# CWBudde/go-pocket-tts

Measured on AMD Instinct MI355X. Metric: synthesized audio sec/sec (xRT), higher is better.
Workload: dtype bf16; 1 GPU; b64_10s_bf16: 64 utterances/GPU x 125 frames (10.0 s each), 25-token prompt + 125-frame voice state, greedy (temperature 0), hipGraph-captured AR step, Mimi decode to 24 kHz PCM written to host; batch_per_gpu=64, frames=125, weights=BF16, kv=bf16, checkpoint=synthetic, shapes of tts_b6369a24 (seed 1234)

## Files before the change

### go-pocket-tts_amd/csrc/capi_hooks.cpp

```cpp
#include "capi_internal.h"
#include "launch_args.h"
#include "../../include/ptts_debug.h"
#include "scan_block.h"
#include "true_peak.h"

#include <memory>

using namespace ptts;
using namespace ptts::capi;

namespace {

template <class T> class Scoped {
    T& var_;
    T old_;
public:
    Scoped(T& var, T value) : var_(var), old_(var) { var = value; }
    ~Scoped() { var_ = old_; }
    Scoped(const Scoped&) = delete;
    Scoped& operator=(const Scoped&) = delete;
};

using Census = std::map<std::string, int64_t>;

// ... 1021 lines not shown
            if (t.t0 % 4) throw Error(PTTS_EINVAL, "ptts_debug_resblock: t0 % 4 != 0 with row destinations");
            if (!t.row_out || t.row_bytes % 16 || t.row_bytes < (int64_t)t.L * 4) throw Error(PTTS_EINVAL, "ptts_debug_resblock: row_bytes must be a multiple of 16 and hold L f32 samples");
            for (int b = 0; b < t.B; b++) if (t.rows[2 * b] < 0) throw Error(PTTS_EINVAL, "ptts_debug_resblock: negative lim");
        }
        if (up_) {
            if (!bf) throw Error(PTTS_EINVAL, "ptts_debug_resblock: f32 weights with the fused form (its weights live in registers and LDS as bf16)");
            if (t.C != 64 || !fin) throw Error(PTTS_EINVAL, "ptts_debug_resblock: the fused form is the 64-wide block with the final convolution");
            if (!t.xin || !t.wup || t.x_pad < 1 || t.x_pad > 64 || t.x_slack < 0 || t.x_slack > 64 || t.x_L < 1) throw Error(PTTS_EINVAL, "ptts_debug_resblock: bad arguments of the fused form");
            if ((int64_t)t.x_L * 4 != t.L) throw Error(PTTS_EINVAL, "ptts_debug_resblock: x_L * 4 != L");
            if (t.t0 % 4) throw Error(PTTS_EINVAL, "ptts_debug_resblock: t0 % 4 != 0 with the fused form");
            if (t.form == RES_FORM_TILE) throw Error(PTTS_EINVAL, "ptts_debug_resblock: the fused form is persistent only");
        }
        ResPlan plan;
        if (t.form == RES_FORM_AUTO) {
            require_device();
            plan = up_ ? resblock_up_plan(t.B, t.t1 - t.t0, RES_FORM_AUTO, 0, resblock_cus()) : resblock_plan(t.C, fin, bf, t.B, t.t1 - t.t0, RES_FORM_AUTO, 0, resblock_cus());
            if (plan.grid == 0) throw Error(PTTS_EINVAL, "ptts_debug_resblock: the fused form is not taken at this size (resblock_up_supported's threshold); ask for form 2 with a grid");
        } else {
            plan = up_ ? resblock_up_plan(t.B, t.t1 - t.t0, t.form, t.grid, 1) : resblock_plan(t.C, fin, bf, t.B, t.t1 - t.t0, t.form, t.grid, 1);
            if (plan.nw == 0) throw Error(PTTS_EINVAL, "ptts_debug_resblock: no persistent form of this block (bf16 weights; 64-wide with the final convolution, 128-wide without)");
        }
        const int64_t total = (int64_t)t.B * plan.tiles;
        if (plan.pers && (plan.grid < 1 || plan.grid > total))
            throw Error(PTTS_EINVAL, strfmt("ptts_debug_resblock: grid %d outside [1, B * tiles = %lld]: a block's first tile would lie past the last utterance", plan.grid, (long long)total));
        if (!plan.pers && plan.grid != total) throw Error(PTTS_EINVAL, "ptts_debug_resblock: one block per tile");

        const int C = t.C, H = t.H, B = t.B, L = t.L;
        const size_t n1 = frag16_count((size_t)H, (size_t)3 * C), n2 = frag16_count((size_t)C, (size_t)H), nf = frag16_count(16, (size_t)3 * C), nu = frag16_count(256, 256);
        std::vector<uint16_t> w1h(n1), w1l(n1), w2h(n2), w2l(n2), wfh(nf), wfl(nf), wuh(nu);
        pack_frag16(t.w1, (size_t)H, (size_t)3 * C, w1h.data(), bf ? nullptr : w1l.data());
        pack_frag16(t.w2, (size_t)C, (size_t)H, w2h.data(), bf ? nullptr : w2l.data());
        if (fin) pack_final_frag(t.wf, (size_t)3 * C, wfh.data(), wfl.data());
        if (up_) {
            std::vector<float> rg((size_t)256 * 256);
            regroup_convtr_rows(t.wup, 256, 256, 64, rg.data());
            pack_frag16(rg.data(), 256, 256, wuh.data(), nullptr);
        }
        require_device();
        const int64_t urows = (int64_t)t.pad + L + t.slack, u_bs = urows * C, xrows = up_ ? (int64_t)t.x_pad + t.x_L + t.x_slack : 1, x_bs = xrows * 128;
        const size_t u_elems = (size_t)B * u_bs, x_elems = (size_t)B * x_bs, pcm_elems = (size_t)B * L, row_bytes = t.rows ? (size_t)B * t.row_bytes : 0;
        Stage st;
        std::vector<float> img(u_elems, std::nanf("")), xi(up_ ? x_elems : 0, std::nanf(""));
        if (t.u) for (int b = 0; b < B; b++) std::memcpy(img.data() + (size_t)b * u_bs, t.u + (size_t)b * (t.pad + L) * C, (size_t)(t.pad + L) * C * 4);
        if (up_) for (int b = 0; b < B; b++) std::memcpy(xi.data() + (size_t)b * x_bs, t.xin + (size_t)b * (t.x_pad + t.x_L) * 128, (size_t)(t.x_pad + t.x_L) * 128 * 4);
        float *dUo = st.out(u_elems), *dPcm = st.out(pcm_elems);
        uint8_t* dRows = st.out<uint8_t>(row_bytes);
        ResArgs a;
        a.u = st.in(img.data(), u_elems); a.u_bs = u_bs; a.pad = t.pad;
        a.w1 = st.in(w1h.data(), n1); a.w2 = st.in(w2h.data(), n2);
        if (!bf) { a.w1_lo = st.in(w1l.data(), n1); a.w2_lo = st.in(w2l.data(), n2); }
        a.b1 = st.in(t.b1, (size_t)H); a.b2 = st.in(t.b2, (size_t)C);
        a.B = B; a.L = L; a.t0 = t.t0; a.t1 = t.t1; a.C = C; a.H = H; a.k1 = 3; a.k2 = 1; a.w_bf16 = bf; a.final_conv = fin;
        if (fin) {
            a.kf = 3; a.wf_hi = st.in(wfh.data(), nf); a.wf_lo = st.in(wfl.data(), nf);
            a.bf = st.in(t.bf, 1);
            a.pcm = dPcm; a.pcm_bs = L;
            if (t.rows) {
                std::vector<PcmRow> pr((size_t)B);
                for (int b = 0; b < B; b++) pr[b] = PcmRow{dRows + (size_t)b * t.row_bytes, t.rows[2 * b], t.rows[2 * b + 1] != 0};
                a.pcm_rows = st.in(pr.data(), (size_t)B);
            }
        } else a.uo = dUo;
        if (up_) {
            a.fuse_up = 1; a.xin = st.in(xi.data(), x_elems); a.x_bs = x_bs; a.x_pad = t.x_pad; a.x_L = t.x_L; a.CI = 128; a.up_stride = 4; a.wup = st.in(wuh.data(), nu);
            a.bup = st.in(t.bup, 64);
        }
        if (!(up_ ? resblock_up_shape_supported(a) : resblock_supported(a))) throw Error(PTTS_EINVAL, "ptts_debug_resblock: refused by resblock_supported / resblock_up_shape_supported");
        if (up_) launch_resblock_up_as(a, plan, nullptr);
        else launch_resblock_as(a, plan, nullptr);
        PTTS_HIP(hipGetLastError());
        PTTS_HIP(hipDeviceSynchronize());
        if (t.launched) { t.launched[0] = plan.nw; t.launched[1] = plan.pers; t.launched[2] = plan.grid; t.launched[3] = plan.tiles; t.launched[4] = plan.tout; }
        if (t.uo) down(t.uo, dUo, u_elems * 4);
        if (t.pcm) down(t.pcm, dPcm, pcm_elems * 4);
        if (t.rows) down(t.row_out, dRows, row_bytes);
    });
}

int ptts_debug_mimi_pack(int32_t kind, const float* w1, const float* w2, int32_t n, uint16_t* dst) {
    return guard([&] {
        if (!w1 || !dst || n < 32 || n % 32 || kind < 0 || kind > 1 || (kind == 0 && !w2)) throw Error(PTTS_EINVAL, "ptts_debug_mimi_pack: bad arguments");
        if (kind == 0) pack_ffn_image(w1, w2, n, dst);
        else pack_w1_image(w1, n, dst);
    });
}

int ptts_debug_mimi_fused(const ptts_mimi_fused_args* pa) {
    return guard([&] {
        if (!pa) throw Error(PTTS_EINVAL, "ptts_debug_mimi_fused: null argument");
        const ptts_mimi_fused_args& t = *pa;
        if (t.kind < 0 || t.kind > 1) throw Error(PTTS_EINVAL, strfmt("ptts_debug_mimi_fused: unknown kind %d", t.kind));
        const bool ffn = t.kind == 0;
        if (!t.x || !t.ln_w || !t.ln_b || !t.w1 || !t.out || (ffn && !t.w2) || t.M < 1 || t.M > (1 << 20) || t.D < 1 || t.D > 4096 || t.F < 1 || t.F > 8192 ||
            t.x_elems < 1 || t.x_ld < 1 || t.x_rows_per_batch < 0 || t.x_rows_per_batch > INT32_MAX || t.x_batch_stride < 0 || t.x_off < 0 || t.ls_off < 0 || t.ls_off > 64)
            throw Error(PTTS_EINVAL, "ptts_debug_mimi_fused: bad arguments");
        if (!ffn && (t.y_elems < 1 || t.y_ld < 1 || t.y_rows_per_batch < 0 || t.y_rows_per_batch > INT32_MAX || t.y_batch_stride < 0 || t.y_off < 0 || t.ls))
            throw Error(PTTS_EINVAL, "ptts_debug_mimi_fused: bad arguments for k_mimi_rowlin");
        const bool rope = t.rope_cos || t.rope_sin;
        if (rope && (ffn || !t.rope_cos || !t.rope_sin || t.n_pos < 1 || t.pos0 < 0 || t.rows_per_seg < 0 || t.rope_cols < 0))
            throw Error(PTTS_EINVAL, "ptts_debug_mimi_fused: bad RoPE arguments");
        const int M = t.M, D = t.D, F = t.F;
        const RowMap xmap{t.x_ld, t.x_rows_per_batch, t.x_batch_stride}, ymap{t.y_ld, t.y_rows_per_batch, t.y_batch_stride};
        check_rows("ptts_debug_mimi_fused", "x", M, t.x_elems, xmap, t.x_off, D, ffn);
        if (!ffn) check_rows("ptts_debug_mimi_fused", "y", M, t.y_elems, ymap, t.y_off, F, true);
        if (rope)
            for (int64_t m = 0; m < M; m++) {
                const int64_t pos = (int64_t)t.pos0 + (t.rows_per_seg ? m % t.rows_per_seg : m);
                if (pos >= t.n_pos) throw Error(PTTS_EINVAL, strfmt("ptts_debug_mimi_fused: row %lld at position %lld, the tables hold %d", (long long)m, (long long)pos, t.n_pos));
            }
        require_device();
        const size_t img_entries = ffn ? ffn_image_count(F) : w1_image_count(F), ntab = rope ? (size_t)t.n_pos * 32 : 0;
        Stage st;
        Tmp dX((size_t)t.x_elems * 4), dLw((size_t)D * 4), dLb((size_t)D * 4), dLs(((size_t)D + t.ls_off) * 4), dImg(img_entries * 2), dCos(ntab * 4), dSin(ntab * 4);
        float* dY = ffn ? nullptr : st.out((size_t)t.y_elems);
        FfnArgs fa;
        RowLinArgs ra;
        if (ffn) {
            fa.x = dX.as<float>() + t.x_off; fa.xmap = xmap;
            fa.ln_w = dLw.as<float>(); fa.ln_b = dLb.as<float>(); fa.eps = t.eps;
            fa.img = dImg.p;
            if (t.ls) fa.ls = dLs.as<float>() + t.ls_off;
            fa.M = M; fa.D = D; fa.F = F;
            if (!mimi_ffn_supported(fa)) throw Error(PTTS_EINVAL, "ptts_debug_mimi_fused: refused by mimi_ffn_supported");
        } else {
            ra.x = dX.as<float>() + t.x_off; ra.xmap = xmap;
            ra.ln_w = dLw.as<float>(); ra.ln_b = dLb.as<float>(); ra.eps = t.eps;
            ra.img = dImg.p;
            ra.y = dY + t.y_off; ra.ymap = ymap;
            if (rope) { ra.rope_cos = dCos.as<float>(); ra.rope_sin = dSin.as<float>(); ra.rope_cols = t.rope_cols; ra.rope_pos0 = t.pos0; ra.rope_rows_per_seg = t.rows_per_seg; }
            ra.M = M; ra.N = F; ra.K = D;
            if (!mimi_rowlin_supported(ra)) throw Error(PTTS_EINVAL, "ptts_debug_mimi_fused: refused by mimi_rowlin_supported");
        }
        std::vector<uint16_t> img(img_entries);
        if (ffn) pack_ffn_image(t.w1, t.w2, F, img.data());
        else pack_w1_image(t.w1, F, img.data());
        up(dImg.p, img.data(), img_entries * 2);
        up(dX.p, t.x, (size_t)t.x_elems * 4);
        up(dLw.p, t.ln_w, (size_t)D * 4); up(dLb.p, t.ln_b, (size_t)D * 4);
        if (t.ls) up(dLs.as<float>() + t.ls_off, t.ls, (size_t)D * 4);
        if (rope) { up(dCos.p, t.rope_cos, ntab * 4); up(dSin.p, t.rope_sin, ntab * 4); }
        LaunchScope launches;
        launches.run([&] {
            if (ffn) launch_mimi_ffn(fa, nullptr);
            else launch_mimi_rowlin(ra, nullptr);
        });
        PTTS_HIP(hipGetLastError());
        PTTS_HIP(hipDeviceSynchronize());
        put_str(t.launched, t.launched_cap, launches.str());
        if (ffn) down(t.out, dX.p, (size_t)t.x_elems * 4);
        else down(t.out, dY, (size_t)t.y_elems * 4);
    });
}

int ptts_mimi_layer_piece(ptts_model* h, int32_t layer, int32_t which, const float* x, int64_t rows, int32_t pos0, int32_t rows_per_seg, float* out) {
    return guard([&] {
        if (!h || !h->m) throw Error(PTTS_EINVAL, "native-safetensors runtime unavailable");
        Model& m = *h->m;
        const Desc& d = m.d;
        if (!x || !out || rows <= 0 || rows > (1 << 24)) throw Error(PTTS_EINVAL, "ptts-hip: bad rows");
        if (layer < 0 || layer >= d.mimi_layers) throw Error(PTTS_EINVAL, strfmt("ptts-hip: mimi layer %d out of range [0,%d)", layer, d.mimi_layers));
        if (which != PTTS_MIMI_PIECE_QKV && which != PTTS_MIMI_PIECE_FFN) throw Error(PTTS_EINVAL, "ptts-hip: unknown layer piece");
        if (pos0 < 0 || rows_per_seg < 0 || (int64_t)pos0 + (rows_per_seg ? rows_per_seg : rows) > ROPE_SEQ)
            throw Error(PTTS_EINVAL, strfmt("ops: rope cos/sin sequence length too small for pos=%d seq=%lld", pos0, (long long)(rows_per_seg ? rows_per_seg : rows)));
        std::lock_guard<std::mutex> lock(m.mu);
        m.use_device();
        const int C = d.mimi_dim, F = d.mimi_ffn, R = (int)rows;
        const int NO = which == PTTS_MIMI_PIECE_QKV ? 3 * C : C;
        Tmp dx((size_t)R * C * 4), dn((size_t)R * C * 4), dy((size_t)R * std::max(NO, F) * 4);
        PTTS_HIP(hipMemcpyAsync(dx.p, x, (size_t)R * C * 4, hipMemcpyHostToDevice, m.stream));
        if (which == PTTS_MIMI_PIECE_QKV) {
            mimi_layer_qkv(m, layer, dx.as<float>(), RowMap{C, 0, 0}, R, dy.as<float>(), RowMap{3 * C, 0, 0}, pos0, rows_per_seg, dn.as<float>(), m.stream);
            PTTS_HIP(hipMemcpyAsync(out, dy.p, (size_t)R * NO * 4, hipMemcpyDeviceToHost, m.stream));
        } else {
            mimi_layer_ffn(m, layer, dx.as<float>(), RowMap{C, 0, 0}, R, dn.as<float>(), dy.as<float>(), m.stream);
            PTTS_HIP(hipMemcpyAsync(out, dx.p, (size_t)R * NO * 4, hipMemcpyDeviceToHost, m.stream));
        }
        PTTS_HIP(hipStreamSynchronize(m.stream));
    });
}

}
```

### go-pocket-tts_amd/csrc/ffn_fused.hip

```cpp
#include <cstdlib>
#include <type_traits>

#include "kernels.h"
#include "device_util.h"
#include "mfma_util.h"

namespace ptts {

namespace {

__device__ __forceinline__ float ff_gelu(float x) {
    const float ax = fabsf(x);
    const float t = __builtin_amdgcn_rcpf(fmaf(0.3275911f * 0.70710678118654752f, ax, 1.0f));
    float p = fmaf(1.061405429f, t, -1.453152027f);
    p = fmaf(p, t, 1.421413741f);
    p = fmaf(p, t, -0.284496736f);
    p = fmaf(p, t, 0.254829592f);
    p *= t;
    const float e = __builtin_amdgcn_exp2f(-1.4426950408889634f * 0.5f * x * x);
    const float erfa = fmaf(-p, e, 1.0f);
    const float erfs = copysignf(erfa, x);
    return 0.5f * x * (1.0f + erfs);
}

constexpr int FF_D = 512;
constexpr int FF_CH = 32;
constexpr int FF_KS = FF_D / 32;
constexpr int FF_OT = FF_D / 16;
constexpr int FF_W1B = FF_CH * FF_D * 2;
constexpr int FF_W2B = FF_D * FF_CH * 2;
constexpr int FF_IMG = FF_W1B + FF_W2B;

__device__ __forceinline__ void ff_dma32k(const char* src, char* dst, int wave, int lane) {
#pragma unroll
    for (int i = 0; i < 8; i++) {
        const int idx = i * 4 + wave;
        lds_dma1k(src + idx * 1024 + lane * 16, dst + idx * 1024);
    }
}

__device__ __forceinline__ void ff_rows_layernorm(const float* xrow, const float* ln_w, const float* ln_b, float eps, int q, Frag (&xh)[16], Frag (&xl)[16]) {
    float4 v[16][2];
#pragma unroll
    for (int s = 0; s < 16; s++) {
        v[s][0] = *reinterpret_cast<const float4*>(xrow + 32 * s + 4 * q);
        v[s][1] = *reinterpret_cast<const float4*>(xrow + 32 * s + 16 + 4 * q);
    }
    float sum = 0.f;
#pragma unroll
    for (int s = 0; s < 16; s++) sum += (v[s][0].x + v[s][0].y) + (v[s][0].z + v[s][0].w) + (v[s][1].x + v[s][1].y) + (v[s][1].z + v[s][1].w);
    sum += __shfl_xor(sum, 16, 64);
    sum += __shfl_xor(sum, 32, 64);
    const float mean = sum * (1.0f / 512);
    float var = 0.f;
#pragma unroll
    for (int s = 0; s < 16; s++) {
#pragma unroll
        for (int h = 0; h < 2; h++) {
            const float d0 = v[s][h].x - mean, d1 = v[s][h].y - mean, d2 = v[s][h].z - mean, d3 = v[s][h].w - mean;
            var += (d0 * d0 + d1 * d1) + (d2 * d2 + d3 * d3);
        }
    }
    var += __shfl_xor(var, 16, 64);
    var += __shfl_xor(var, 32, 64);
    const float rstd = 1.0f / sqrtf(var * (1.0f / 512) + eps);
#pragma unroll
    for (int s = 0; s < 16; s++) {
        float4 o[2];
#pragma unroll
        for (int h = 0; h < 2; h++) {
            const int k = 32 * s + 16 * h + 4 * q;
            const float4 g = *reinterpret_cast<const float4*>(ln_w + k), b = *reinterpret_cast<const float4*>(ln_b + k);
            o[h].x = (v[s][h].x - mean) * rstd * g.x + b.x;
            o[h].y = (v[s][h].y - mean) * rstd * g.y + b.y;
            o[h].z = (v[s][h].z - mean) * rstd * g.z + b.z;
            o[h].w = (v[s][h].w - mean) * rstd * g.w + b.w;
        }
        split2(o[0].x, o[0].y, xh[s].u[0], xl[s].u[0]);
        split2(o[0].z, o[0].w, xh[s].u[1], xl[s].u[1]);
        split2(o[1].x, o[1].y, xh[s].u[2], xl[s].u[2]);
        split2(o[1].z, o[1].w, xh[s].u[3], xl[s].u[3]);
    }
}

template <class Piece>
__device__ __forceinline__ void ff_gemm1(const char* w1, int r16, int q, const Frag (&xh)[16], const Frag (&xl)[16], f32x4 (&acc)[2], Piece&& piece) {
    const int sw1 = (r16 >> 1) & 7;
    acc[0] = f32x4{0.f, 0.f, 0.f, 0.f};
    acc[1] = f32x4{0.f, 0.f, 0.f, 0.f};
    Frag wa[2], wb[2];
    const char* wl = w1 + r16 * 128;
    wa[0].q = *reinterpret_cast<const uint4*>(wl + ((q ^ sw1) << 4));
    wb[0].q = *reinterpret_cast<const uint4*>(wl + ((q ^ sw1) << 4) + 2048);
#pragma unroll
    for (int s = 0; s < 16; s++) {
        __builtin_amdgcn_sched_barrier(0);
        if (s + 1 < 16) {
            const int off = ((s + 1) >> 1) * 4096 + (((4 * ((s + 1) & 1) + q) ^ sw1) << 4);
            wa[(s + 1) & 1].q = *reinterpret_cast<const uint4*>(wl + off);
            wb[(s + 1) & 1].q = *reinterpret_cast<const uint4*>(wl + off + 2048);
        }
        acc[0] = __builtin_amdgcn_mfma_f32_16x16x32_bf16(wa[s & 1].v, xh[s].v, acc[0], 0, 0, 0);
        acc[1] = __builtin_amdgcn_mfma_f32_16x16x32_bf16(wb[s & 1].v, xh[s].v, acc[1], 0, 0, 0);
        PTTS_LO_MFMA(acc[0] = __builtin_amdgcn_mfma_f32_16x16x32_bf16(wa[s & 1].v, xl[s].v, acc[0], 0, 0, 0));
        PTTS_LO_MFMA(acc[1] = __builtin_amdgcn_mfma_f32_16x16x32_bf16(wb[s & 1].v, xl[s].v, acc[1], 0, 0, 0));
        piece(s);
        asm volatile("" : "+a"(acc[0]), "+a"(acc[1]));
        if (s + 1 < 16) __builtin_amdgcn_sched_group_barrier(0x100, 2, 0);
#pragma unroll
        for (int i = 0; i < 4; i++) {
            __builtin_amdgcn_sched_group_barrier(0x008, 1, 0);
            __builtin_amdgcn_sched_group_barrier(0x002, 3, 0);
        }
        __builtin_amdgcn_sched_barrier(0);
    }
}

}

template <int V>
__global__ __launch_bounds__(256) __attribute__((amdgpu_waves_per_eu(1, 1))) void k_mimi_ffn(FfnArgs a) {
    __shared__ __attribute__((aligned(16))) char lds[2 * FF_W1B + 2 * FF_W2B];
    const int tid = threadIdx.x, lane = tid & 63, wave = __builtin_amdgcn_readfirstlane(tid >> 6);
    const int r16 = lane & 15, q = lane >> 4;
    const int nch = a.F / FF_CH;
    const char* img = reinterpret_cast<const char*>(a.img);
    auto w1s = [&](int i) { return lds + i * FF_W1B; };
    auto w2s = [&](int i) { return lds + 2 * FF_W1B + i * FF_W2B; };

    ff_dma32k(img, w1s(0), wave, lane);
    ff_dma32k(img + FF_W1B, w2s(0), wave, lane);
    ff_dma32k(img + (size_t)min(1, nch - 1) * FF_IMG, w1s(1), wave, lane);

    const int m0 = blockIdx.x * 64 + wave * 16;
    const int row = min(m0 + r16, a.M - 1);
    const float* xrow = a.x + row_off(a.xmap, row);
    Frag xh[FF_KS], xl[FF_KS];
    ff_rows_layernorm(xrow, a.ln_w, a.ln_b, a.eps, q, xh, xl);

    f32x4 acc2[FF_OT];
#pragma unroll
    for (int t = 0; t < FF_OT; t++) acc2[t] = f32x4{0.f, 0.f, 0.f, 0.f};

    const int w2_lane = r16 * 64 + ((q ^ (((r16 >> 3) & 1) * 3)) << 4);

    asm volatile("s_waitcnt vmcnt(0)" ::: "memory");
    __syncthreads();
    f32x4 acc1[2], acc1n[2];
    ff_gemm1(w1s(0), r16, q, xh, xl, acc1, [](int) {});

    for (int c = 0; c < nch; c++) {
        asm volatile("s_waitcnt vmcnt(0)" ::: "memory");
        __syncthreads();
        asm volatile("" : "+a"(acc1[0]), "+a"(acc1[1]));
        const char* const src1 = img + (size_t)min(c + 2, nch - 1) * FF_IMG + wave * 1024 + lane * 16;
        const char* const src2 = img + (size_t)min(c + 1, nch - 1) * FF_IMG + FF_W1B + wave * 1024 + lane * 16;
        char* const dst1 = w1s(c & 1) + wave * 1024;
        char* const dst2 = w2s((c + 1) & 1) + wave * 1024;
        Frag hh, hl;
        float g[8];
        ff_gemm1(w1s(min(c + 1, nch - 1) & 1), r16, q, xh, xl, acc1n, [&](int s) {
            const int i = s >> 1;
            if ((s & 1) == 0) g[i] = ff_gelu(acc1[i >> 2][i & 3]);
            else if (i & 1) split2(g[i - 1], g[i], hh.u[i >> 1], hl.u[i >> 1]);
            if constexpr (V == 0) {
                if (s < 8) lds_dma1k(src1 + s * 4096, dst1 + s * 4096);
                else lds_dma1k(src2 + (s - 8) * 4096, dst2 + (s - 8) * 4096);
            }
        });
        const char* w2 = w2s(c & 1) + w2_lane;
        Frag w2f[2];
        w2f[0].q = *reinterpret_cast<const uint4*>(w2);
#pragma unroll
        for (int t = 0; t < FF_OT; t++) {
            __builtin_amdgcn_sched_barrier(0);
            if (t + 1 < FF_OT) w2f[(t + 1) & 1].q = *reinterpret_cast<const uint4*>(w2 + (t + 1) * 1024);
            acc2[t] = __builtin_amdgcn_mfma_f32_16x16x32_bf16(w2f[t & 1].v, hh.v, acc2[t], 0, 0, 0);
            PTTS_LO_MFMA(acc2[t] = __builtin_amdgcn_mfma_f32_16x16x32_bf16(w2f[t & 1].v, hl.v, acc2[t], 0, 0, 0));
            if (t + 1 < FF_OT) __builtin_amdgcn_sched_group_barrier(0x100, 1, 0);
            __builtin_amdgcn_sched_group_barrier(0x008, 2, 0);
            __builtin_amdgcn_sched_barrier(0);
        }
        acc1[0] = acc1n[0];
        acc1[1] = acc1n[1];
    }

    if (m0 + r16 < a.M) {
        float* orow = a.x + row_off(a.xmap, m0 + r16);
        const bool has_ls = a.ls != nullptr;
        const float* lsp = has_ls ? a.ls : a.ln_w;
#pragma unroll
        for (int t0 = 0; t0 < FF_OT; t0 += 8) {
            float4 r[8], sc[8];
#pragma unroll
            for (int t = 0; t < 8; t++) {
                const int col = 16 * (t0 + t) + 4 * q;
                r[t] = *reinterpret_cast<const float4*>(orow + col);
                sc[t] = *reinterpret_cast<const float4*>(lsp + col);
                if (!has_ls) sc[t] = make_float4(1.f, 1.f, 1.f, 1.f);
            }
#pragma unroll
            for (int t = 0; t < 8; t++) {
#pragma clang fp contract(off)
                const f32x4 y = acc2[t0 + t];
                float4 o;
                o.x = r[t].x + sc[t].x * y[0];
                o.y = r[t].y + sc[t].y * y[1];
                o.z = r[t].z + sc[t].z * y[2];
                o.w = r[t].w + sc[t].w * y[3];
                *reinterpret_cast<float4*>(orow + 16 * (t0 + t) + 4 * q) = o;
            }
        }
    }
}

__global__ __launch_bounds__(256) __attribute__((amdgpu_waves_per_eu(1, 1))) void k_mimi_rowlin(RowLinArgs a) {
    constexpr int NS = 3;
    __shared__ __attribute__((aligned(16))) char lds[NS * FF_W1B];
    const int tid = threadIdx.x, lane = tid & 63, wave = __builtin_amdgcn_readfirstlane(tid >> 6);
    const int r16 = lane & 15, q = lane >> 4;
    const int nch = a.N / FF_CH;
    const char* img = reinterpret_cast<const char*>(a.img);
    ff_dma32k(img, lds, wave, lane);
    ff_dma32k(img + (size_t)min(1, nch - 1) * FF_W1B, lds + FF_W1B, wave, lane);

    const int m0 = blockIdx.x * 64 + wave * 16;
    const int row = min(m0 + r16, a.M - 1);
    Frag xh[FF_KS], xl[FF_KS];
    ff_rows_layernorm(a.x + row_off(a.xmap, row), a.ln_w, a.ln_b, a.eps, q, xh, xl);
    float2 cs[4], sn[4];
    const bool rope = a.rope_cos != nullptr;
    {
        const int pos = a.rope_pos0 + (a.rope_rows_per_seg ? row % a.rope_rows_per_seg : row);
        const float* ct = rope ? a.rope_cos + (int64_t)pos * 32 : a.ln_w;
        const float* st = rope ? a.rope_sin + (int64_t)pos * 32 : a.ln_w;
#pragma unroll
        for (int i = 0; i < 4; i++) {
            const int jj = (32 * (i >> 1) + 16 * (i & 1) + 4 * q) >> 1;
            cs[i] = *reinterpret_cast<const float2*>(ct + jj);
            sn[i] = *reinterpret_cast<const float2*>(st + jj);
        }
    }
    float* const yrow = a.y + row_off(a.ymap, row);

    auto store_piece = [&](f32x4 (&acc)[2], int cc, auto par, int ht) {
#pragma clang fp contract(off)
        constexpr int PAR = decltype(par)::value;
        asm volatile("" : "+a"(acc[0]), "+a"(acc[1]));
        const int col = 32 * cc + 16 * ht + 4 * q;
        const bool rot = rope && 32 * cc < a.rope_cols;
        const f32x4 v = acc[ht];
        const float2 c2 = cs[2 * PAR + ht], s2 = sn[2 * PAR + ht];
        const float y0 = v[0] * c2.x - v[1] * s2.x, y1 = v[0] * s2.x + v[1] * c2.x;
        const float y2 = v[2] * c2.y - v[3] * s2.y, y3 = v[2] * s2.y + v[3] * c2.y;
        const float4 o = make_float4(rot ? y0 : v[0], rot ? y1 : v[1], rot ? y2 : v[2], rot ? y3 : v[3]);
        *reinterpret_cast<float4*>(yrow + col) = o;
    };

    asm volatile("s_waitcnt vmcnt(0)" ::: "memory");
    __syncthreads();
    f32x4 accA[2], accB[2];
    auto iter = [&](int c, auto par, auto first, f32x4 (&acc)[2], f32x4 (&prev)[2]) {
        constexpr int PAR = decltype(par)::value;
        constexpr bool FIRST = decltype(first)::value != 0;
        if constexpr (!FIRST) {
            asm volatile("s_waitcnt vmcnt(10)" ::: "memory");
            __syncthreads();
        }
        const char* const src = img + (size_t)min(c + 2, nch - 1) * FF_W1B + wave * 1024 + lane * 16;
        char* const dst = lds + ((c + 2) % NS) * FF_W1B + wave * 1024;
        ff_gemm1(lds + (c % NS) * FF_W1B, r16, q, xh, xl, acc, [&](int s) {
            if ((s & 1) == 0) lds_dma1k(src + (s >> 1) * 4096, dst + (s >> 1) * 4096);
            if constexpr (!FIRST) {
                if (s == 5) store_piece(prev, c - 1, std::integral_constant<int, 1 - PAR>{}, 0);
                if (s == 11) store_piece(prev, c - 1, std::integral_constant<int, 1 - PAR>{}, 1);
            }
        });
    };
    using ic0 = std::integral_constant<int, 0>;
    using ic1 = std::integral_constant<int, 1>;
    iter(0, ic0{}, ic1{}, accA, accB);
    iter(1, ic1{}, ic0{}, accB, accA);
    for (int c = 2; c < nch; c += 2) {
        iter(c, ic0{}, ic0{}, accA, accB);
        iter(c + 1, ic1{}, ic0{}, accB, accA);
    }
    store_piece(accB, nch - 1, std::integral_constant<int, 1>{}, 0);
    store_piece(accB, nch - 1, std::integral_constant<int, 1>{}, 1);
}

bool mimi_rowlin_supported(const RowLinArgs& a) {
    return a.img && a.K == FF_D && a.N >= 64 && a.N % 64 == 0 && a.M > 0 && aligned16(a.x) && a.xmap.ld % 4 == 0 && a.xmap.batch_stride % 4 == 0 && aligned16(a.y) &&
           a.ymap.ld % 4 == 0 && a.ymap.batch_stride % 4 == 0 && aligned16(a.img) && a.ln_w && a.ln_b && aligned16(a.ln_w) && aligned16(a.ln_b) &&
           (!a.rope_cos || (a.rope_sin && a.rope_cols % 64 == 0 && a.rope_cols <= a.N && (reinterpret_cast<uintptr_t>(a.rope_cos) & 7) == 0 && (reinterpret_cast<uintptr_t>(a.rope_sin) & 7) == 0));
}

void launch_mimi_rowlin(const RowLinArgs& a, hipStream_t stream) {
    note_launch(a.rope_cos ? "k_mimi_rowlin+rope" : "k_mimi_rowlin");
    hipLaunchKernelGGL(k_mimi_rowlin, dim3((unsigned)((a.M + 63) / 64)), dim3(256), 0, stream, a);
}

bool mimi_ffn_supported(const FfnArgs& a) {
    return a.img && a.D == FF_D && a.F >= FF_CH && a.F % FF_CH == 0 && a.M > 0 && aligned16(a.x) && a.xmap.ld % 4 == 0 && a.xmap.batch_stride % 4 == 0 &&
           aligned16(a.img) && a.ln_w && a.ln_b && aligned16(a.ln_w) && aligned16(a.ln_b) && (!a.ls || aligned16(a.ls));
}

void launch_mimi_ffn(const FfnArgs& a, hipStream_t stream) {
    note_launch("k_mimi_ffn");
    const dim3 grid((unsigned)((a.M + 63) / 64));
    hipLaunchKernelGGL(k_mimi_ffn<0>, grid, dim3(256), 0, stream, a);
}

}
```

### go-pocket-tts_amd/csrc/kernels.h

```cpp
#pragma once

#include <hip/hip_runtime.h>
#include <atomic>
#include <cstddef>
#include <cstdint>
#include <map>
#include <string>
#include <vector>

#include "deesser.h"
#include "limiter.h"
#include "pitch.h"
#include "tempo.h"
#include "trim.h"

namespace ptts {

struct RowMap {
    int64_t ld = 0;
    int64_t rows_per_batch = 0;
    int64_t batch_stride = 0;
};

enum AOp : int { AOP_NONE = 0, AOP_ELU = 1 };
// ... 255 lines not shown
    double* b_tiles;
    double* p_tiles;
    double* s_tiles;
    int32_t design, pad;
};
static_assert(sizeof(DeRow) == 48, "a turn of the de-esser ring holds 256 of them");
void launch_deesser(const DeRow* rows_dev, int n, int max_tiles, const DeScan* designs_dev, hipStream_t stream);

constexpr int kLimMaxDesigns = 16;
constexpr size_t kLimScanBytes = 64;
static_assert(sizeof(LimScan) == kLimScanBytes, "the limiter ring's tail (runtime.h) is sized by it");
struct LimRow {
    float* x;
    int64_t n;
    double* p_tiles;
    float* r;
    int32_t design, pad;
};
static_assert(sizeof(LimRow) == 40, "a turn of the limiter ring holds 256 of them");
void launch_limiter(const LimRow* rows_dev, int n, int max_tiles, const LimScan* designs_dev, hipStream_t stream);

constexpr int kJoinThreads = 256;
constexpr int kJoinTile = 4 * kJoinThreads;
struct JoinRow {
    const float* src;
    const float* prev;
    float* dst;
    int64_t off;
    int64_t n;
    int32_t k;
    int32_t gap;
};
static_assert(sizeof(JoinRow) == 48, "a turn of the join ring holds 256 of them");
void launch_join(const JoinRow* rows_dev, int n, int max_tiles, hipStream_t stream);

constexpr int kTrimMaxDesigns = 16;
constexpr size_t kTrimScanBytes = 32;
static_assert(sizeof(TrimScan) == kTrimScanBytes, "the trim ring's tail (runtime.h) is sized by it");
struct TrimTile {
    int32_t first, last;
    int32_t removed, cuts;
    int32_t prev, next;
    int32_t off, pad;
};
static_assert(sizeof(TrimTile) == 32, "trim_scratch_bytes counts on it");
struct TrimRow {
    const float* src;
    float* dst;
    int64_t n;
    TrimTile* tiles;
    ptts_trim_info* info;
    int32_t design, pad;
};
static_assert(sizeof(TrimRow) == 48, "a turn of the trim ring holds 256 of them");
void launch_trim(const TrimRow* rows_dev, int n, int max_tiles, const TrimScan* designs_dev, hipStream_t stream);

constexpr int kTempoMaxDesigns = 16;
constexpr size_t kTempoScanBytes = 16;
static_assert(sizeof(TempoScan) == kTempoScanBytes, "the tempo ring's tail (runtime.h) is sized by it");
struct TempoRow {
    const float* src;
    float* dst;
    int64_t n;
    int64_t n_out;
    int32_t* p;
    int32_t design, pad;
};
static_assert(sizeof(TempoRow) == 48, "a turn of the tempo ring holds 256 of them");
void launch_tempo(const TempoRow* rows_dev, int n, int max_tiles, const TempoScan* designs_dev, hipStream_t stream);

constexpr int kPitchMaxDesigns = 16;
constexpr size_t kPitchScanBytes = 16;
static_assert(sizeof(PitchScan) == kPitchScanBytes, "the pitch ring's tail (runtime.h) is sized by it");
constexpr int kPitchThreads = 512;
constexpr int kPitchTile = 1024;
constexpr int kPitchWindow = 2 * kPitchTile + 110;
PTTS_HD inline int pitch_image_at(int q) { return q + (q >> 5); }
constexpr int kPitchImage = (kPitchEntries + (kPitchEntries >> 5) + 1) & ~1;
struct PitchRow {
    const float* src;
    float* dst;
    int64_t n;
    int64_t n_out;
    int32_t design, pad;
};
static_assert(sizeof(PitchRow) == 40, "a turn of the pitch ring holds 256 of them");
void launch_pitch(const PitchRow* rows_dev, int n, int max_tiles, const PitchScan* designs_dev, const float* image_dev, hipStream_t stream);

constexpr int kFormantAnalyseThreads = 256;
constexpr int kFormantWhitenThreads = 256;
constexpr int kFormantShapeTiles = 16;
struct FormantRow {
    const float* x;
    float* e;
    const float* er;
    float* out;
    float* coeffs;
    int64_t n, n_r;
    int32_t K, p;
};
static_assert(sizeof(FormantRow) == 64, "a turn of the formant ring holds 256 of them");
void launch_formant_analyse(const FormantRow* rows_dev, int n, int64_t max_frames, const double* tables_dev, hipStream_t stream);
void launch_formant_whiten(const FormantRow* rows_dev, int n, int64_t max_tiles, hipStream_t stream);
void launch_formant_shape(const FormantRow* rows_dev, int n, int64_t max_tiles, hipStream_t stream);

struct PcmRow { void* dst; int32_t lim; int32_t s16; };
struct ResArgs {
    const float* u = nullptr; int64_t u_bs = 0; int pad = 0;
    float* uo = nullptr;
    float* pcm = nullptr; int64_t pcm_bs = 0;
    const PcmRow* pcm_rows = nullptr;
    const void* w1 = nullptr; const void* w1_lo = nullptr; const float* b1 = nullptr;
    const void* w2 = nullptr; const void* w2_lo = nullptr; const float* b2 = nullptr;
    const void* wf_hi = nullptr; const void* wf_lo = nullptr; const float* bf = nullptr;
    int B = 0, L = 0, t0 = 0, t1 = 0;
    int C = 0, H = 0, k1 = 0, k2 = 0, kf = 0, w_bf16 = 0, final_conv = 0;
    int fuse_up = 0; const float* xin = nullptr; int64_t x_bs = 0; int x_pad = 0, x_L = 0, CI = 0, up_stride = 0;
    const void* wup = nullptr; const float* bup = nullptr;
};
bool resblock_supported(const ResArgs& a);
void launch_resblock(const ResArgs& a, hipStream_t stream);
bool resblock_up_shape_supported(const ResArgs& a);
bool resblock_up_supported(const ResArgs& a);
void launch_resblock_up(const ResArgs& a, hipStream_t stream);
enum { RES_FORM_AUTO = 0, RES_FORM_TILE = 1, RES_FORM_PERS = 2 };
struct ResPlan { int nw = 0, pers = 0, grid = 0, tiles = 0, tout = 0; };
int resblock_cus();
ResPlan resblock_plan(int C, int final_conv, int w_bf16, int B, int rows, int form, int grid, int cus);
ResPlan resblock_up_plan(int B, int rows, int form, int grid, int cus);
void launch_resblock_as(const ResArgs& a, const ResPlan& p, hipStream_t stream);
void launch_resblock_up_as(const ResArgs& a, const ResPlan& p, hipStream_t stream);


struct FfnArgs {
    float* x = nullptr; RowMap xmap;
    const float* ln_w = nullptr; const float* ln_b = nullptr; float eps = 1e-5f;
    const void* img = nullptr;
    const float* ls = nullptr;
    int M = 0, D = 0, F = 0;
};
struct RowLinArgs {
    const float* x = nullptr; RowMap xmap;
    const float* ln_w = nullptr; const float* ln_b = nullptr; float eps = 1e-5f;
    const void* img = nullptr;
    float* y = nullptr; RowMap ymap;
    const float* rope_cos = nullptr; const float* rope_sin = nullptr; int rope_cols = 0, rope_pos0 = 0, rope_rows_per_seg = 0;
    int M = 0, N = 0, K = 0;
};
bool mimi_rowlin_supported(const RowLinArgs& a);
void launch_mimi_rowlin(const RowLinArgs& a, hipStream_t stream);
bool mimi_ffn_supported(const FfnArgs& a);
void launch_mimi_ffn(const FfnArgs& a, hipStream_t stream);

constexpr int FC_MAX_DEPTH = 8;
struct FlowClusterArgs {
    const float* fx_in = nullptr; float* fx_out = nullptr;
    const float* ada = nullptr; int64_t ldmod = 0;
    int rows = 0, depth = 0;
    float eps[FC_MAX_DEPTH] = {};
    const float* ln_w[FC_MAX_DEPTH] = {}; const float* ln_b[FC_MAX_DEPTH] = {};
    const void* w0[FC_MAX_DEPTH] = {}; const float* b0[FC_MAX_DEPTH] = {};
    const void* w2[FC_MAX_DEPTH] = {}; const float* b2[FC_MAX_DEPTH] = {};
    unsigned long long* xbuf = nullptr;
    unsigned long long* stamps = nullptr;
    int inject = 0;
    unsigned* sync = nullptr;
};
constexpr int kFlowClusterRows = 12;
constexpr int kFlowClusterMaxTiles = (kStepMaxRows + kFlowClusterRows - 1) / kFlowClusterRows;
constexpr size_t kFlowClusterTileBytes = (size_t)2 * 16 * 512 * 8;
constexpr size_t kFlowClusterSyncBytes = (size_t)(32 * kFlowClusterMaxTiles + 32) * 4;
inline size_t flow_cluster_xbuf_bytes(int rows) { return (size_t)((rows + kFlowClusterRows - 1) / kFlowClusterRows) * kFlowClusterTileBytes; }
bool flow_cluster_fits(int rows, int device);
bool flow_cluster_supported(const FlowClusterArgs& a, int C);
void launch_flow_cluster(const FlowClusterArgs& a, hipStream_t stream, hipEvent_t ev0 = nullptr, hipEvent_t ev1 = nullptr);

struct StepState {
    int32_t* kv_len;
    int32_t* active;
    int32_t* step;
    int32_t* countdown;
    int32_t* n_frames;
    int32_t* eos_step;
    int32_t* max_steps;
    int32_t* frames_after_eos;
    float*   eos_threshold;
    int32_t* n_active;
    int32_t* broke;
};
struct StepChain {
    const void* w_in; const float* b_in; float* x; int32_t d_in;
    const void* w_pj; const float* b_pj; float* fx; int32_t d_pj;
    const float* bos; float* x0; int32_t w_bf16; int32_t ok;
};
struct StepFinish {
    StepState s;
    const float* eos_logit;
    float* latents;
    int64_t lat_stride;
    int32_t ldim;
    StepChain ch;
};
struct StepOpenLinears {
    const void* w_in = nullptr; const float* b_in = nullptr; int d_in = 0; float* x = nullptr;
    const void* w_pj = nullptr; const float* b_pj = nullptr; int d_pj = 0; float* fx = nullptr;
    int w_bf16 = 0;
};
bool step_open_mfma_ok(const StepOpenLinears& lin, int ldim);
void launch_step_begin(const StepState& s, const float* latents, int64_t lat_stride, const float* bos, const float* noise, int64_t noise_stride,
                       int ldim, int b, float* in32, float* x0, const StepOpenLinears* lin, hipStream_t stream);
void launch_step_finish(const StepState& s, const float* frame, const float* eos_logit, int ldim, int b, float* latents,
                        int64_t lat_stride, hipStream_t stream);
struct NoiseSpec { uint64_t seed; float sigma; int32_t rows; };
void launch_noise_fill(const NoiseSpec* spec_dev, int n_slots, int max_rows, float* out, int64_t out_stride, int ldim, hipStream_t stream);
struct GatherTable { struct Row { int32_t src_row, dst_off, nf, T; }; Row rows[128]; };
void launch_gather_frames(const GatherTable& t, int n, const float* stage, int64_t row_stride, float* dst, int ld, hipStream_t stream);
void launch_readback_i32(const int32_t* a, int na, const int32_t* b, int nb, int32_t* host, hipStream_t stream);
struct SlotAdmit { int32_t slot, max_steps, frames_after_eos; float eos_threshold; int32_t kv_len, pre_len; const void* pre_k; const void* pre_v; };
void launch_slot_admit(const StepState& s, int32_t* pre_len, const void** pre_k, const void** pre_v, const SlotAdmit* dev, int n, hipStream_t stream);
void launch_slot_retire(const StepState& s, const int32_t* slots_dev, int n, hipStream_t stream);
void launch_fill_i32(int32_t* p, int32_t v, int n, hipStream_t stream);
void launch_add_i32(int32_t* p, const int32_t* inc, int n, hipStream_t stream);

void launch_enc_head(const float* pcm, const void* w, int w_bf16, const float* b, int64_t L, int C, int k, float* out, int64_t ldo, hipStream_t stream);
int enc_ds_splits(int M, int N, int K);
void launch_enc_downsample(const float* A, int64_t lda, const void* W, int w_bf16, const float* bias, int M, int N, int K, float* partial, float* out,
                           hipStream_t stream);

void launch_bct_to_btc(const float* in, int b, int c, int t, float* out, int out_pad_rows, hipStream_t stream);
void launch_btc_to_bct(const float* in, int in_pad_rows, int b, int c, int t, float* out, hipStream_t stream);

}
```

### go-pocket-tts_amd/csrc/mimi_decode.cpp

```cpp
#include "launch_args.h"

#include <algorithm>

namespace ptts {

void mimi_setup(Model& m, MimiWs& w, int B, int T) {
    const Desc& d = m.d;
    w.B = B; w.T = T;
    const int C = d.mimi_dim, S = d.up_stride, T1 = T * S, F = d.mimi_ffn;
    w.P0 = d.init_k - 1;
    w.Ls[0] = T1; w.Ps[0] = 1;
    for (int j = 0; j < 3; j++) {
        w.Ls[j + 1] = w.Ls[j] * d.strides[j];
        int need_next = j < 2 ? 1 : d.final_k - 1;
        w.Ps[j + 1] = std::max(d.rb_k1[j] - 1, need_next);
    }
    size_t n_xp = (size_t)B * (1 + T) * C, n_up = (size_t)B * (w.P0 + T1) * C;
    size_t n_n1 = (size_t)B * T1 * C, n_qkv = (size_t)B * T1 * 3 * C, n_ff = (size_t)B * T1 * F;
    size_t n_c[4], n_h[3];
    for (int j = 0; j < 4; j++) n_c[j] = (size_t)B * (w.Ps[j] + w.Ls[j]) * d.sea_ch[j];
    for (int j = 0; j < 3; j++) n_h[j] = (size_t)B * ((d.rb_k2[j] - 1) + w.Ls[j + 1]) * d.sea_hidden[j];
    size_t total = n_xp + n_up + n_n1 + n_qkv * d.mimi_layers + n_n1 + n_ff + n_c[0] + 2 * (n_c[1] + n_c[2] + n_c[3]) + n_h[0] + n_h[1] + n_h[2];
    DevBuf& wsb = m.work(WORK_DECODER, total * sizeof(float));
    float* p = wsb.as<float>();
    w.xp = p; p += n_xp;
    w.up = p; p += n_up;
    w.n1 = p; p += n_n1;
    for (int l = 0; l < d.mimi_layers; l++) { w.qkv[l] = p; p += n_qkv; }
    w.attn = p; p += n_n1;
    w.ff = p; p += n_ff;
    w.c0 = p; p += n_c[0];
    for (int j = 0; j < 3; j++) { w.u[j] = p; p += n_c[j + 1]; w.uo[j] = p; p += n_c[j + 1]; w.h[j] = p; p += n_h[j]; }
    w.zeroed = false;
}

void mimi_zero_history(Model& m, MimiWs& w, hipStream_t s) {
    const Desc& d = m.d;
    const int C = d.mimi_dim, T1 = w.Ls[0];
    launch_zero_rows(w.xp, (int64_t)(1 + w.T) * C, w.B, C, s);
    launch_zero_rows(w.up, (int64_t)(w.P0 + T1) * C, w.B, (int64_t)w.P0 * C, s);
    launch_zero_rows(w.c0, (int64_t)(w.Ps[0] + w.Ls[0]) * d.sea_ch[0], w.B, (int64_t)w.Ps[0] * d.sea_ch[0], s);
    for (int j = 0; j < 3; j++) {
        const int cout = d.sea_ch[j + 1], hid = d.sea_hidden[j], Ph = d.rb_k2[j] - 1;
        launch_zero_rows(w.u[j], (int64_t)(w.Ps[j + 1] + w.Ls[j + 1]) * cout, w.B, (int64_t)w.Ps[j + 1] * cout, s);
        launch_zero_rows(w.uo[j], (int64_t)(w.Ps[j + 1] + w.Ls[j + 1]) * cout, w.B, (int64_t)w.Ps[j + 1] * cout, s);
        if (Ph > 0) launch_zero_rows(w.h[j], (int64_t)(Ph + w.Ls[j + 1]) * hid, w.B, (int64_t)Ph * hid, s);
    }
    w.zeroed = true;
}

void mimi_layer_qkv(Model& m, int l, const float* x, RowMap xmap, int R, float* qkv, RowMap qmap, int pos0, int rows_per_seg, float* n1, hipStream_t s) {
    mimi_layer_qkv(m, m.d.ml[l], x, xmap, R, qkv, qmap, pos0, rows_per_seg, n1, s);
}
void mimi_layer_qkv(Model& m, const Desc::ML& L, const float* x, RowMap xmap, int R, float* qkv, RowMap qmap, int pos0, int rows_per_seg, float* n1, hipStream_t s) {
    const Desc& d = m.d;
    const int C = d.mimi_dim;
    if (L.qkv_img != NONE && d.mimi_hd == 64) {
        RowLinArgs ra;
        ra.x = x; ra.xmap = xmap;
        ra.ln_w = m.at<float>(L.n1.w); ra.ln_b = m.at<float>(L.n1.b); ra.eps = L.n1.eps;
        ra.img = m.at<uint8_t>(L.qkv_img);
        ra.y = qkv; ra.ymap = qmap;
        ra.rope_cos = m.at<float>(d.rope_cos); ra.rope_sin = m.at<float>(d.rope_sin); ra.rope_cols = 2 * C; ra.rope_pos0 = pos0; ra.rope_rows_per_seg = rows_per_seg;
        ra.M = R; ra.N = 3 * C; ra.K = C;
        if (mimi_rowlin_supported(ra)) { launch_mimi_rowlin(ra, s); return; }
    }
    launch_layernorm(mkln(m, x, xmap, L.n1, n1, C, R), s);
    GemmArgs gq = mk(m, n1, flat(C), L.in_proj, qkv, qmap, R);
    gq.rope_cos = m.at<float>(d.rope_cos); gq.rope_sin = m.at<float>(d.rope_sin);
    gq.rope_cols = 2 * C; gq.rope_hd = d.mimi_hd; gq.rope_pos0 = pos0; gq.rope_rows_per_seg = rows_per_seg;
    if (!launch_gemm_rope(gq, s)) {
        gq.rope_cos = gq.rope_sin = nullptr;
        launch_gemm(gq, s);
        launch_rope_rows(qkv, qmap, 0, d.mimi_heads, d.mimi_hd, nullptr, pos0, rows_per_seg, R, m.at<float>(d.rope_cos), m.at<float>(d.rope_sin), s);
        launch_rope_rows(qkv, qmap, C, d.mimi_heads, d.mimi_hd, nullptr, pos0, rows_per_seg, R, m.at<float>(d.rope_cos), m.at<float>(d.rope_sin), s);
    }
}

void mimi_layer_ffn(Model& m, int l, float* x, RowMap xmap, int R, float* n1, float* ffb, hipStream_t s) {
    mimi_layer_ffn(m, m.d.ml[l], x, xmap, R, n1, ffb, s);
}
void mimi_layer_ffn(Model& m, const Desc::ML& L, float* x, RowMap xmap, int R, float* n1, float* ffb, hipStream_t s) {
    const Desc& d = m.d;
    const int C = d.mimi_dim, F = d.mimi_ffn;
    if (L.ffn_img != NONE) {
        FfnArgs fa;
        fa.x = x; fa.xmap = xmap;
        fa.ln_w = m.at<float>(L.n2.w); fa.ln_b = m.at<float>(L.n2.b); fa.eps = L.n2.eps;
        fa.img = m.at<uint8_t>(L.ffn_img);
        fa.ls = m.at<float>(L.ls2);
        fa.M = R; fa.D = C; fa.F = F;
        if (mimi_ffn_supported(fa)) { launch_mimi_ffn(fa, s); return; }
    }
    launch_layernorm(mkln(m, x, xmap, L.n2, n1, C, R), s);
    GemmArgs g1 = mk(m, n1, flat(C), L.l1, ffb, flat(F), R);
    g1.epi = EPI_GELU;
    launch_gemm(g1, s);
    GemmArgs g2 = mk(m, ffb, flat(F), L.l2, x, xmap, R);
    g2.R = x; g2.epi = L.ls2 != NONE ? EPI_SCALE_RESADD : EPI_RESADD; g2.scale = m.at<float>(L.ls2);
    launch_gemm(g2, s);
}

void mimi_range(Model& m, MimiWs& w, const float* lat, int64_t lat_bstride, int f0, int f1, float* pcm, float* mimi_latent, hipStream_t s,
                const PcmRow* pcm_rows, bool* rows_used, float* xformer_out) {
    if (rows_used) *rows_used = false;
    const Desc& d = m.d;
    const int B = w.B, T = w.T, C = d.mimi_dim, S = d.up_stride, T1 = T * S, P0 = w.P0;
    if (f1 <= f0) return;
    if (!w.zeroed) mimi_zero_history(m, w, s);
    const int nf = f1 - f0;
    launch_projector(lat, lat_bstride, m.at<float>(d.proj_w), m.at<float>(d.proj_b), B, T, f0, f1, d.ldim, C, w.xp, s);
    if (mimi_latent) launch_btc_to_bct(w.xp, 1, B, C, T, mimi_latent, s);
    launch_upsample_depthwise(w.xp, m.at<float>(d.up_w0), m.at<float>(d.up_w1), nullptr, B, T, f0, f1, C, S, w.up, P0, s);
    const int t0 = f0 * S, CT = nf * S, R = B * CT;
    const int64_t up_bs = (int64_t)(P0 + T1) * C;
    float* upx = w.up + (size_t)(P0 + t0) * C;
    const RowMap upm = seg(C, CT, up_bs);
    float* n1 = w.n1;
    float* attn = w.attn;
    float* ffb = w.ff;
    for (int l = 0; l < d.mimi_layers; l++) {
        const auto& L = d.ml[l];
        float* qkv = w.qkv[l];
        float* qkvx = qkv + (size_t)t0 * 3 * C;
        const RowMap qm = seg(3 * C, CT, (int64_t)T1 * 3 * C);
        mimi_layer_qkv(m, l, upx, upm, R, qkvx, qm, t0, CT, n1, s);
        launch_attention(attn_dense_args(qkv, 3 * C, C, B, T1, t0, CT, d.mimi_heads, d.mimi_hd, d.mimi_ctx, attn, C), s);
        GemmArgs go = mk(m, attn, flat(C), L.out_proj, upx, upm, R);
        go.R = upx; go.epi = L.ls1 != NONE ? EPI_SCALE_RESADD : EPI_RESADD; go.scale = m.at<float>(L.ls1);
        launch_gemm(go, s);
        mimi_layer_ffn(m, l, upx, upm, R, n1, ffb, s);
    }
    if (xformer_out)
        PTTS_HIP(hipMemcpy2DAsync(xformer_out + (size_t)t0 * C, (size_t)T1 * C * sizeof(float), upx, (size_t)up_bs * sizeof(float), (size_t)CT * C * sizeof(float),
                                  (size_t)B, hipMemcpyDeviceToDevice, s));
    int r0 = t0, rn = CT;
    {
        const int ch = d.sea_ch[0];
        GemmArgs g = mk(m, w.up + (size_t)r0 * C, seg(C, rn, up_bs), d.init_conv, w.c0 + (size_t)(w.Ps[0] + r0) * ch,
                        seg(ch, rn, (int64_t)(w.Ps[0] + w.Ls[0]) * ch), B * rn);
        g.epi = EPI_ELU;
        if (C % 64 == 0 && d.init_conv.in == d.init_k * C) { g.win_taps = d.init_k; g.win_c = C; }
        launch_gemm(g, s);
    }
    bool final_done = false;
    for (int j = 0; j < 3; j++) {
        const int cin = d.sea_ch[j], cout = d.sea_ch[j + 1], st = d.strides[j], hid = d.sea_hidden[j];
        const int Lin_ = w.Ls[j], Lout = w.Ls[j + 1], Pin = w.Ps[j], Pout = w.Ps[j + 1], Ph = d.rb_k2[j] - 1;
        const float* in = j == 0 ? w.c0 : w.uo[j - 1];
        float* u = w.u[j];
        float* uo = w.uo[j];
        float* hb = w.h[j];
        const int64_t in_bs = (int64_t)(Pin + Lin_) * cin, u_bs = (int64_t)(Pout + Lout) * cout, h_bs = (int64_t)(Ph + Lout) * hid;
        GemmArgs gu = mk(m, in + (size_t)(Pin - 1 + r0) * cin, seg(cin, rn, in_bs), d.up[j],
                         u + (size_t)(Pout + (int64_t)r0 * st) * cout, seg((int64_t)st * cout, rn, u_bs), B * rn);
        if (j == 2 && d.rb1[j].wf != NONE && d.rb2[j].wf != NONE && d.rb1[j].bf16 && d.rb2[j].bf16 && d.up[j].wf != NONE) {
            ResArgs rr;
            rr.u = u; rr.u_bs = u_bs; rr.pad = Pout; rr.uo = uo;
            rr.w1 = m.at<uint8_t>(d.rb1[j].wf); rr.b1 = m.at<float>(d.rb1[j].b);
            rr.w2 = m.at<uint8_t>(d.rb2[j].wf); rr.b2 = m.at<float>(d.rb2[j].b);
            rr.B = B; rr.L = Lout; rr.t0 = r0 * st; rr.t1 = (r0 + rn) * st;
            rr.C = cout; rr.H = hid; rr.k1 = d.rb_k1[j]; rr.k2 = d.rb_k2[j]; rr.w_bf16 = 1;
            rr.final_conv = 1; rr.kf = d.final_k; rr.wf_hi = m.at<uint8_t>(d.final_wf); rr.wf_lo = m.at<uint8_t>(d.final_wf_lo); rr.bf = m.at<float>(d.final_b);
            rr.pcm = pcm; rr.pcm_bs = w.Ls[3]; rr.pcm_rows = pcm_rows;
            rr.fuse_up = 1; rr.xin = in; rr.x_bs = in_bs; rr.x_pad = Pin; rr.x_L = Lin_; rr.CI = cin; rr.up_stride = st;
            rr.wup = m.at<uint8_t>(d.up[j].wf); rr.bup = m.at<float>(d.up[j].b);
            if (resblock_up_supported(rr)) {
                launch_resblock_up(rr, s);
                if (rows_used && pcm_rows) *rows_used = true;
                final_done = true;
                r0 *= st; rn *= st;
                continue;
            }
        }
        launch_gemm(gu, s);
        r0 *= st; rn *= st;
        {
            ResArgs ra;
            ra.u = u; ra.u_bs = u_bs; ra.pad = Pout; ra.uo = uo;
            ra.w1 = m.at<uint8_t>(d.rb1[j].wf); ra.w1_lo = m.at<uint8_t>(d.rb1[j].wf_lo); ra.b1 = m.at<float>(d.rb1[j].b);
            ra.w2 = m.at<uint8_t>(d.rb2[j].wf); ra.w2_lo = m.at<uint8_t>(d.rb2[j].wf_lo); ra.b2 = m.at<float>(d.rb2[j].b);
            ra.B = B; ra.L = Lout; ra.t0 = r0; ra.t1 = r0 + rn;
            ra.C = cout; ra.H = hid; ra.k1 = d.rb_k1[j]; ra.k2 = d.rb_k2[j]; ra.w_bf16 = d.rb1[j].bf16;
            if (j == 2) {
                ra.final_conv = 1; ra.kf = d.final_k; ra.wf_hi = m.at<uint8_t>(d.final_wf); ra.wf_lo = m.at<uint8_t>(d.final_wf_lo); ra.bf = m.at<float>(d.final_b);
                ra.pcm = pcm; ra.pcm_bs = w.Ls[3];
            }
            if (j == 2 && pcm_rows && d.rb1[j].wf != NONE && d.rb2[j].wf != NONE && d.rb1[j].bf16 == d.rb2[j].bf16) {
                ResArgs rr = ra;
                rr.pcm_rows = pcm_rows;
                if (resblock_supported(rr)) {
                    launch_resblock(rr, s);
                    if (rows_used) *rows_used = true;
                    final_done = true;
                    continue;
                }
            }
            if (d.rb1[j].wf != NONE && d.rb2[j].wf != NONE && d.rb1[j].bf16 == d.rb2[j].bf16 && resblock_supported(ra)) {
                launch_resblock(ra, s);
                if (j == 2) final_done = true;
                continue;
            }
        }
        GemmArgs g1 = mk(m, u + (size_t)(Pout - (d.rb_k1[j] - 1) + r0) * cout, seg(cout, rn, u_bs), d.rb1[j],
                         hb + (size_t)(Ph + r0) * hid, seg(hid, rn, h_bs), B * rn);
        g1.aop = AOP_ELU; g1.epi = EPI_ELU;
        if (cout % 64 == 0 && d.rb1[j].in == d.rb_k1[j] * cout) { g1.win_taps = d.rb_k1[j]; g1.win_c = cout; }
        launch_gemm(g1, s);
        GemmArgs g2 = mk(m, hb + (size_t)r0 * hid, seg(hid, rn, h_bs), d.rb2[j], uo + (size_t)(Pout + r0) * cout, seg(cout, rn, u_bs), B * rn);
        g2.R = u + (size_t)(Pout + r0) * cout; g2.epi = EPI_RESADD_ELU;
        launch_gemm(g2, s);
    }
    if (!final_done)
    launch_conv_final(w.uo[2], w.Ps[3], m.at<float>(d.final_w), m.at<float>(d.final_b), B, w.Ls[3], r0, r0 + rn, d.sea_ch[3], d.final_k, 0, pcm, s);
}

void mimi_decode(Model& m, const float* lat, int64_t lat_bstride, int B, int T, float* pcm, float* mimi_latent, float* xformer_out) {
    if (B <= 0 || T <= 0) return;
    if ((int64_t)T * m.d.up_stride > ROPE_SEQ) throw Error(PTTS_EINVAL, strfmt("ops: rope cos/sin sequence length too small for pos=0 seq=%lld", (long long)T * m.d.up_stride));
    const Desc& d = m.d;
    double per_frame = 4.0 * ((double)d.up_stride * (d.mimi_dim * (4.0 + 3.0 * d.mimi_layers) + d.mimi_ffn) +
                              (double)d.samples_per_frame * (d.sea_ch[3] * 2.6 + d.sea_ch[2] * 0.7 + d.sea_ch[1] * 0.25));
    int group = (int)std::max(1.0, std::min((double)B, 40e9 / (per_frame * T)));
    const int64_t spu = (int64_t)T * d.samples_per_frame;
    for (int b0 = 0; b0 < B; b0 += group) {
        int nb = std::min(group, B - b0);
        MimiWs w;
        mimi_setup(m, w, nb, T);
        mimi_range(m, w, lat + (int64_t)b0 * lat_bstride, lat_bstride, 0, T, pcm + (int64_t)b0 * spu,
                   mimi_latent ? mimi_latent + (int64_t)b0 * d.mimi_dim * T : nullptr, m.stream, nullptr, nullptr,
                   xformer_out ? xformer_out + (int64_t)b0 * T * d.up_stride * d.mimi_dim : nullptr);
    }
}

}
```

### go-pocket-tts_amd/csrc/model.cpp

```cpp
#include <cmath>
#include <functional>

#include "model.h"

namespace ptts {

void quantize_rows(std::vector<float>& rm, size_t out, size_t in, std::vector<float>& scale, std::vector<int8_t>& q) {
    scale.assign(out, 1.0f);
    q.assign(out * in, 0);
    for (size_t n = 0; n < out; n++) {
        float mx = 0.0f;
        for (size_t k = 0; k < in; k++) mx = std::max(mx, std::fabs(rm[n * in + k]));
        const float s = mx > 0.0f ? mx / 127.0f : 1.0f;
        scale[n] = s;
        for (size_t k = 0; k < in; k++) {
            float v = std::nearbyint(rm[n * in + k] / s);
            v = std::min(127.0f, std::max(-127.0f, v));
            q[n * in + k] = (int8_t)v;
            rm[n * in + k] = v * s;
        }
    }
}
size_t step_tiled_bytes(size_t out, size_t in, int bytes_per_weight) {
    return ((out + 15) / 16) * ((in + 127) / 128) * 16 * 128 * (size_t)bytes_per_weight;
}
void pack_step_tiled(const float* rm, size_t out, size_t in, bool bf16w, uint8_t* dst) {
    const int E = bf16w ? 8 : 4, WV = bf16w ? 4 : 8;
    const size_t nt = (out + 15) / 16, nss = (in + 127) / 128;
    for (size_t t = 0; t < nt; t++)
        for (size_t ss = 0; ss < nss; ss++)
            for (int sidx = 0; sidx < WV; sidx++)
                for (int lane = 0; lane < 64; lane++)
                    for (int j = 0; j < E; j++) {
                        size_t n = t * 16 + (size_t)(lane & 15), k = ss * 128 + (size_t)(lane >> 4) * 32 + (size_t)sidx * E + j;
                        float v = (n < out && k < in) ? rm[n * in + k] : 0.0f;
                        size_t e = ((((t * nss + ss) * WV + sidx) * 64 + lane) * E + j);
                        if (bf16w) reinterpret_cast<uint16_t*>(dst)[e] = f32_to_bf16_rne(v);
                        else reinterpret_cast<float*>(dst)[e] = v;
                    }
}
void pack_step_tiled_i8(const int8_t* q, size_t out, size_t in, uint8_t* dst) {
    const size_t nt = (out + 15) / 16, nss = (in + 127) / 128;
    for (size_t t = 0; t < nt; t++)
        for (size_t ss = 0; ss < nss; ss++)
            for (int u = 0; u < 2; u++)
                for (int lane = 0; lane < 64; lane++)
                    for (int j = 0; j < 16; j++) {
                        const size_t n = t * 16 + (size_t)(lane & 15), k = ss * 128 + (size_t)(lane >> 4) * 32 + (size_t)(2 * u + j / 8) * 8 + (size_t)(j % 8);
                        const int v = (n < out && k < in) ? q[n * in + k] : 0;
                        dst[((((t * nss + ss) * 2 + u) * 64 + lane) * 16) + j] = (uint8_t)(v + 128);
                    }
}

size_t frag16_count(size_t out, size_t in) { return (out / 16) * (in / 32) * 64 * 8; }
void pack_frag16(const float* rm, size_t out, size_t in, uint16_t* hi, uint16_t* lo) {
    const size_t nt = out / 16, ks = in / 32;
    for (size_t t = 0; t < nt; t++)
        for (size_t s = 0; s < ks; s++)
            for (int lane = 0; lane < 64; lane++)
                for (int j = 0; j < 8; j++) {
                    const float v = rm[(t * 16 + (size_t)(lane & 15)) * in + s * 32 + (size_t)(lane >> 4) * 8 + j];
                    const size_t e = ((t * ks + s) * 64 + lane) * 8 + j;
                    const uint16_t h = f32_to_bf16_rne(v);
                    hi[e] = h;
                    if (lo) lo[e] = f32_to_bf16_rne(v - bf16_to_f32(h));
                }
}
void regroup_convtr_rows(const float* rm, int out, int in, int oc, float* dst) {
    for (int T = 0; T < out / 16; T++)
        for (int q = 0; q < 16; q++) {
            const int n = (q >> 2) * oc + 8 * (T >> 1) + 4 * (T & 1) + (q & 3);
            std::copy(rm + (size_t)n * in, rm + (size_t)(n + 1) * in, dst + (size_t)(T * 16 + q) * in);
        }
}
void pack_final_frag(const float* w, size_t n, uint16_t* hi, uint16_t* lo) {
    for (size_t s = 0; s < n / 32; s++)
        for (int lane = 0; lane < 64; lane++)
            for (int j = 0; j < 8; j++) {
                const size_t kk = s * 32 + (size_t)(lane >> 4) * 8 + j;
                const float v = (lane & 15) == 0 ? w[kk] : 0.0f;
                const uint16_t h = f32_to_bf16_rne(v);
                hi[(s * 64 + lane) * 8 + j] = h;
                lo[(s * 64 + lane) * 8 + j] = f32_to_bf16_rne(v - bf16_to_f32(h));
            }
}

static void w1_image_chunk(const float* w, int c, uint16_t* i1) {
    const int D = 512;
    for (int j = 0; j < 8; j++)
        for (int h = 0; h < 32; h++)
            for (int sg = 0; sg < 2; sg++)
                for (int q = 0; q < 4; q++) {
                    const int pos = (4 * sg + q) ^ ((h >> 1) & 7), s = 2 * j + sg;
                    uint16_t* p = i1 + ((size_t)j * 32 + h) * 64 + pos * 8;
                    for (int e = 0; e < 8; e++) {
                        const int k = 32 * s + (e < 4 ? 4 * q + e : 16 + 4 * q + (e - 4));
                        p[e] = f32_to_bf16_rne(w[(size_t)(32 * c + h) * D + k]);
                    }
                }
}
size_t w1_image_count(int N) { return (size_t)(N / 32) * 16384; }
size_t ffn_image_count(int F) { return (size_t)(F / 32) * 32768; }
void pack_w1_image(const float* rm, int N, uint16_t* dst) {
    for (int c = 0; c < N / 32; c++) w1_image_chunk(rm, c, dst + (size_t)c * 16384);
}
void pack_ffn_image(const float* w1, const float* w2, int F, uint16_t* dst) {
    const int D = 512, nch = F / 32;
    for (int c = 0; c < nch; c++) {
        uint16_t* i1 = dst + (size_t)c * 32768;
        uint16_t* i2 = i1 + 16384;
        w1_image_chunk(w1, c, i1);
        for (int o = 0; o < D; o++)
            for (int q = 0; q < 4; q++) {
                const int pos = q ^ (3 * ((o >> 3) & 1));
                uint16_t* p = i2 + (size_t)o * 32 + pos * 8;
                for (int e = 0; e < 8; e++) {
                    const int hcol = 32 * c + (e < 4 ? 4 * q + e : 16 + 4 * q + (e - 4));
                    p[e] = f32_to_bf16_rne(w2[(size_t)o * F + hcol]);
                }
            }
    }
}

namespace {

struct Walker {
    const StFile& f;
    Desc& d;
    bool bf16w;
    uint8_t* host;
    bool i8w = false;
    size_t cur = 0;

    size_t reserve(size_t bytes) {
        size_t off = (cur + 255) & ~(size_t)255;
        cur = off + bytes;
        return off;
    }
    bool has(const std::string& n) const { return f.has(n); }
    const std::vector<int64_t>& shape(const std::string& n) const { return f.at(n).shape; }
    std::vector<float> load(const std::string& n) const {
        std::vector<float> v((size_t)f.at(n).count());
        f.decode_f32(n, v.data());
        return v;
    }
    size_t add_f32(size_t count, const std::function<void(float*)>& fill) {
        size_t off = reserve(count * 4);
        if (host) fill(reinterpret_cast<float*>(host + off));
        return off;
    }
    size_t add_mat(size_t count, const std::function<void(float*)>& fill, int* is_bf16) {
        *is_bf16 = bf16w ? 1 : 0;
        size_t off = reserve(count * (bf16w ? 2 : 4));
        if (host) {
            if (bf16w) {
                std::vector<float> tmp(count);
                fill(tmp.data());
                uint16_t* dst = reinterpret_cast<uint16_t*>(host + off);
                for (size_t i = 0; i < count; i++) dst[i] = f32_to_bf16_rne(tmp[i]);
            } else fill(reinterpret_cast<float*>(host + off));
        }
        d.n_params += (int64_t)count;
        return off;
    }
    void expect_rank(const std::string& n, size_t rank) const {
        if (shape(n).size() != rank) throw Error(PTTS_EFORMAT, strfmt("native: tensor \"%s\" rank %zu, want %zu", n.c_str(), shape(n).size(), rank));
    }

    void add_tiled_i8(Lin& l, std::vector<float>* rm) {
        l.wt = reserve(step_tiled_bytes((size_t)l.out, (size_t)l.in, 1));
        l.wscale = reserve((size_t)l.out * 4);
        l.wt_i8 = 1;
        if (!host) return;
        std::vector<float> scale;
        std::vector<int8_t> q;
        quantize_rows(*rm, (size_t)l.out, (size_t)l.in, scale, q);
        std::memcpy(host + l.wscale, scale.data(), scale.size() * 4);
        pack_step_tiled_i8(q.data(), (size_t)l.out, (size_t)l.in, host + l.wt);
    }
    void add_step_matrix(Lin& l, const std::function<void(float*)>& fill_rowmajor, bool own_rowmajor) {
        const size_t count = (size_t)l.out * l.in;
        if (!i8w) {
            if (own_rowmajor) l.w = add_mat(count, fill_rowmajor, &l.bf16);
            add_tiled(l, fill_rowmajor);
            return;
        }
        std::vector<float> rm;
        if (host) { rm.resize(count); fill_rowmajor(rm.data()); }
        add_tiled_i8(l, &rm);
        if (own_rowmajor) {
            l.bf16 = 0;
            l.w = reserve(count * 4);
            if (host) std::memcpy(host + l.w, rm.data(), count * 4);
            d.n_params += (int64_t)count;
        }
    }

    void add_tiled(Lin& l, const std::function<void(float*)>& fill_rowmajor) {
        if (i8w) {
            std::vector<float> rm;
            if (host) { rm.resize((size_t)l.out * l.in); fill_rowmajor(rm.data()); }
            add_tiled_i8(l, &rm);
            return;
        }
        l.wt = reserve(step_tiled_bytes((size_t)l.out, (size_t)l.in, bf16w ? 2 : 4));
        if (!host) return;
        std::vector<float> rm((size_t)l.out * l.in);
        fill_rowmajor(rm.data());
        pack_step_tiled(rm.data(), (size_t)l.out, (size_t)l.in, bf16w, host + l.wt);
    }
    void add_frag16(Lin& l, const std::function<void(float*)>& fill_rowmajor) {
        if (l.out % 16 != 0 || l.in % 32 != 0) return;
        const size_t count = frag16_count((size_t)l.out, (size_t)l.in);
        l.wf = reserve(count * 2);
        if (!bf16w) l.wf_lo = reserve(count * 2);
        if (!host) return;
        std::vector<float> rm((size_t)l.out * l.in);
        fill_rowmajor(rm.data());
        pack_frag16(rm.data(), (size_t)l.out, (size_t)l.in, reinterpret_cast<uint16_t*>(host + l.wf), bf16w ? nullptr : reinterpret_cast<uint16_t*>(host + l.wf_lo));
    }
    size_t add_w1_image(const std::string& wn, int N) {
        const size_t off = reserve(w1_image_count(N) * 2);
        if (!host) return off;
        const std::vector<float> w = load(wn);
        pack_w1_image(w.data(), N, reinterpret_cast<uint16_t*>(host + off));
        return off;
    }
    size_t add_ffn_image(const std::string& w1n, const std::string& w2n, int F) {
        const size_t off = reserve(ffn_image_count(F) * 2);
        if (!host) return off;
        const std::vector<float> w1 = load(w1n), w2 = load(w2n);
        pack_ffn_image(w1.data(), w2.data(), F, reinterpret_cast<uint16_t*>(host + off));
        return off;
    }
    std::vector<float> effective_weights(const std::string& wn) {
        std::vector<float> rm = load(wn);
        const size_t out = (size_t)shape(wn)[0], in = (size_t)shape(wn)[1];
        if (i8w) {
            std::vector<float> sc;
            std::vector<int8_t> q;
            quantize_rows(rm, out, in, sc, q);
        } else if (bf16w) {
            for (float& v : rm) v = bf16_to_f32(f32_to_bf16_rne(v));
        }
        return rm;
    }
    Lin step_linear(const std::string& name, bool with_bias) {
        if (!i8w) {
            Lin l = linear(name, with_bias);
            const std::string wn = name + ".weight";
            add_tiled(l, [&](float* dst) { f.decode_f32(wn, dst); });
            return l;
        }
        Lin l;
        const std::string wn = name + ".weight";
        expect_rank(wn, 2);
        l.out = (int)shape(wn)[0];
        l.in = (int)shape(wn)[1];
        add_step_matrix(l, [&](float* dst) { f.decode_f32(wn, dst); }, true);
        if (with_bias && has(name + ".bias")) {
            const std::string bn = name + ".bias";
            if (shape(bn).size() != 1 || shape(bn)[0] != l.out) throw Error(PTTS_EFORMAT, strfmt("native: linear \"%s\" bias shape incompatible with weight", name.c_str()));
            l.b = add_f32((size_t)l.out, [&](float* dst) { f.decode_f32(bn, dst); });
        }
        return l;
    }

    Lin linear(const std::string& name, bool with_bias) {
        Lin l;
        const std::string wn = name + ".weight";
        expect_rank(wn, 2);
        l.out = (int)shape(wn)[0];
        l.in = (int)shape(wn)[1];
// ... 383 lines not shown
```

### go-pocket-tts_amd/csrc/model.h

```cpp
#pragma once

#include "common.h"

namespace ptts {

constexpr size_t NONE = (size_t)-1;
constexpr int MAX_LAYERS = 32;
constexpr int ROPE_SEQ = 8192;

struct Lin {
    size_t w = NONE, b = NONE;
    size_t wt = NONE;
    size_t wscale = NONE; int wt_i8 = 0;
    size_t wf = NONE, wf_lo = NONE;
    int in = 0, out = 0, bf16 = 0;
};
size_t step_tiled_bytes(size_t out, size_t in, int bytes_per_weight);
void pack_step_tiled(const float* rm, size_t out, size_t in, bool bf16w, uint8_t* dst);
void quantize_rows(std::vector<float>& rm, size_t out, size_t in, std::vector<float>& scale, std::vector<int8_t>& q);
void pack_step_tiled_i8(const int8_t* q, size_t out, size_t in, uint8_t* dst);
size_t frag16_count(size_t out, size_t in);
void pack_frag16(const float* rm, size_t out, size_t in, uint16_t* hi, uint16_t* lo);
void regroup_convtr_rows(const float* rm, int out, int in, int oc, float* dst);
void pack_final_frag(const float* w, size_t n, uint16_t* hi, uint16_t* lo);
size_t w1_image_count(int N);
size_t ffn_image_count(int F);
void pack_w1_image(const float* rm, int N, uint16_t* dst);
void pack_ffn_image(const float* w1, const float* w2, int F, uint16_t* dst);

struct Norm {
    size_t w = NONE, b = NONE;
    int d = 0;
    float eps = 1e-5f;
};

struct Desc {
    int d_model = 0, heads = 16, hd = 0, n_layers = 0, ffn = 0, ldim = 32, n_bins = 0;
    size_t embed = NONE, bos = NONE, rope_cos = NONE, rope_sin = NONE;
    Lin input_linear, out_eos;
    Norm out_norm;
    struct Layer {
        Norm n1, n2; Lin in_proj, out_proj, l1, l2;
    } layers[MAX_LAYERS];
    int flow_dim = 0, flow_depth = 0, nfreq = 0;
    struct TE { size_t freqs = NONE, alpha = NONE; Lin l1, l2; } te[2];
    Lin cond_embed, input_proj, ada_all, final_linear;
    Lin speaker_proj;
    Lin cond_eos;
    struct RB { Norm ln; Lin mlp0, mlp2; } rb[MAX_LAYERS];
    int mimi_dim = 0, mimi_heads = 8, mimi_hd = 0, mimi_layers = 0, mimi_ffn = 0, mimi_ctx = 250;
    int up_stride = 16, up_k = 32;
    size_t proj_w = NONE, proj_b = NONE, up_w0 = NONE, up_w1 = NONE;
    struct ML {
        Norm n1, n2; Lin in_proj, out_proj, l1, l2; size_t ls1 = NONE, ls2 = NONE;
        size_t ffn_img = NONE;
        size_t qkv_img = NONE;
    } ml[MAX_LAYERS];
    int sea_ch[4] = {0, 0, 0, 0};
    int sea_hidden[3] = {0, 0, 0};
    int strides[3] = {6, 5, 4};
    int init_k = 0, rb_k1[3] = {0, 0, 0}, rb_k2[3] = {0, 0, 0}, final_k = 0;
    Lin init_conv, up[3], rb1[3], rb2[3];
    size_t final_w = NONE, final_b = NONE;
    size_t final_wf = NONE, final_wf_lo = NONE;
    int64_t samples_per_frame = 0;
    struct Enc {
        int present = 0;
        int ch[4] = {0, 0, 0, 0};
        int hidden[3] = {0, 0, 0};
        int head_k = 0, rb_k1[3] = {0, 0, 0}, rb_k2[3] = {0, 0, 0}, down_k[3] = {0, 0, 0}, down_s[3] = {0, 0, 0}, tail_k = 0, ds_k = 0, ds_s = 0;
        int layers = 0;
        Lin head, rb1[3], rb2[3], down[3], tail, ds;
        ML ml[MAX_LAYERS];
        int64_t hop = 0;
    } enc;
    int64_t n_params = 0;
    size_t total_bytes = 0;
};

struct Plan {
    StFile file;
    ptts_opts opts;
    Desc desc;
};

void plan_build(Plan& p);
void plan_fill(const Plan& p, uint8_t* host);

}
```

### go-pocket-tts_amd/csrc/runtime.cpp

```cpp
#include "launch_args.h"

#include <chrono>

#include <algorithm>

namespace ptts {

static thread_local UploadArena* tl_upload = nullptr;
static void arena_open(UploadArena& a) {
    if (!a.base && hipHostMalloc((void**)&a.base, (size_t)1 << 20, hipHostMallocDefault) == hipSuccess) a.cap = (size_t)1 << 20;
    else if (!a.base) (void)hipGetLastError();
    a.off = 0;
    tl_upload = &a;
}
UploadScope::UploadScope(UploadArena& a, hipStream_t s) {
    (void)hipStreamSynchronize(s);
    arena_open(a);
}
UploadScope::UploadScope(UploadArena& a, hipEvent_t last_use) {
    if (last_use) (void)hipEventSynchronize(last_use);
    arena_open(a);
}
UploadScope::~UploadScope() { tl_upload = nullptr; }
void h2d(void* dst, const void* src, size_t bytes, hipStream_t s) {
    if (!bytes) return;
    UploadArena* a = tl_upload;
    const size_t need = (bytes + 63) & ~(size_t)63;
    if (a && a->base && a->off + need <= a->cap) {
        char* stage = a->base + a->off;
        a->off += need;
        std::memcpy(stage, src, bytes);
        PTTS_HIP(hipMemcpyAsync(dst, stage, bytes, hipMemcpyHostToDevice, s));
        return;
    }
    PTTS_HIP(hipMemcpyAsync(dst, src, bytes, hipMemcpyHostToDevice, s));
    PTTS_HIP(hipStreamSynchronize(s));
}
void d2h(void* dst, const void* src, size_t bytes, hipStream_t s) {
    if (!bytes) return;
    PTTS_HIP(hipMemcpyAsync(dst, src, bytes, hipMemcpyDeviceToHost, s));
    PTTS_HIP(hipStreamSynchronize(s));
}

Model::~Model() {
    if (upload.base) (void)hipHostFree(upload.base);
    for (hipEvent_t e : prof.ev) (void)hipEventDestroy(e);
    for (hipEvent_t e : prof.phase) if (e) (void)hipEventDestroy(e);
    for (hipEvent_t e : events) (void)hipEventDestroy(e);
    if (stream2) (void)hipStreamDestroy(stream2);

    cached_batch.reset();
    tcomb.clear();
    for (DevBuf& w : ws) w.release();
    if (own_arena && arena) (void)hipFree(arena);
    if (stream) (void)hipStreamDestroy(stream);
}

static std::unique_ptr<Model> model_on(const Desc& d, const ptts_opts& opts, int device) {
    std::unique_ptr<Model> m(new Model());
    m->d = d;
    m->opts = opts;
    m->opts.device = m->device = device;
    m->noise_state = (uint64_t)std::chrono::system_clock::now().time_since_epoch().count() ^ (uint64_t)(uintptr_t)m.get();
    return m;
}
static void open_streams(Model& m) {
    m.use_device();
    int lo = 0, hi = 0;
    PTTS_HIP(hipDeviceGetStreamPriorityRange(&lo, &hi));
    PTTS_HIP(hipStreamCreateWithPriority(&m.stream, hipStreamNonBlocking, hi));
    PTTS_HIP(hipStreamCreateWithPriority(&m.stream2, hipStreamNonBlocking, lo));
}

Model* model_open(Plan* plan, void* device_arena, int fill) {
    int ndev = 0;
    if (hipGetDeviceCount(&ndev) != hipSuccess || ndev <= 0)
        throw Error(PTTS_ENODEVICE, "ptts-hip: no HIP device available (this library has no CPU fallback)");
    if (plan->opts.device < 0 || plan->opts.device >= ndev)
        throw Error(PTTS_ENODEVICE, strfmt("ptts-hip: device %d out of range (%d visible)", plan->opts.device, ndev));
    std::unique_ptr<Model> m = model_on(plan->desc, plan->opts, plan->opts.device);
    open_streams(*m);
    if (device_arena) {
        m->arena = reinterpret_cast<uint8_t*>(device_arena);
    } else {
        void* p = nullptr;
        PTTS_HIP(hipMalloc(&p, m->d.total_bytes));
        m->arena = reinterpret_cast<uint8_t*>(p);
        m->own_arena = true;
        fill = 1;
    }
    if (fill) {
        std::vector<uint8_t> host(m->d.total_bytes, 0);
        plan_fill(*plan, host.data());
        PTTS_HIP(hipMemcpy(m->arena, host.data(), host.size(), hipMemcpyHostToDevice));
    }
    return m.release();
}

Model* model_share(Model& base) {
    std::unique_ptr<Model> m = model_on(base.d, base.opts, base.device);
    open_streams(*m);
    m->arena = base.arena;
    m->own_arena = false;
    return m.release();
}

Model* model_replicate(Model& base, int device) {
    int ndev = 0;
    if (hipGetDeviceCount(&ndev) != hipSuccess || ndev <= 0) throw Error(PTTS_ENODEVICE, "ptts-hip: no HIP device available (this library has no CPU fallback)");
    if (device < 0 || device >= ndev) throw Error(PTTS_ENODEVICE, strfmt("ptts-hip: device %d out of range (%d visible)", device, ndev));
    std::unique_ptr<Model> m = model_on(base.d, base.opts, device);
    {
        std::lock_guard<std::mutex> lock(base.mu);
        base.use_device();
        PTTS_HIP(hipStreamSynchronize(base.stream));
    }
    open_streams(*m);
    void* p = nullptr;
    PTTS_HIP(hipMalloc(&p, m->d.total_bytes));
    m->arena = reinterpret_cast<uint8_t*>(p);
    m->own_arena = true;
    if (device != base.device) {
        int can = 0;
        if (hipDeviceCanAccessPeer(&can, device, base.device) == hipSuccess && can) {
            const hipError_t e = hipDeviceEnablePeerAccess(base.device, 0);
            if (e != hipSuccess && e != hipErrorPeerAccessAlreadyEnabled) (void)hipGetLastError();
            else if (e == hipErrorPeerAccessAlreadyEnabled) (void)hipGetLastError();
        }
    }
    PTTS_HIP(hipMemcpyPeer(m->arena, device, base.arena, base.device, m->d.total_bytes));
    PTTS_HIP(hipDeviceSynchronize());
    return m.release();
}

void profile_read(Model& m, ptts_profile* out) {
    PTTS_HIP(hipStreamSynchronize(m.stream));
    std::memset(out, 0, sizeof *out);
    double ms = 0;
    for (size_t i = 0; i + 1 < m.prof.used; i += 2) {
        float t = 0;
        PTTS_HIP(hipEventElapsedTime(&t, m.prof.ev[i], m.prof.ev[i + 1]));
        ms += t;
    }
    out->launches = m.prof.launches;
    out->total_ms = ms;
    out->algorithmic_bytes = m.prof.bytes;
    out->weight_bytes = m.prof.wbytes;
    if (m.prof.phases) {
        PTTS_HIP(hipStreamSynchronize(m.stream2));
        float t = 0;
        PTTS_HIP(hipEventElapsedTime(&t, m.prof.phase[0], m.prof.phase[1])); out->prefill_ms = t;
        PTTS_HIP(hipEventElapsedTime(&t, m.prof.phase[1], m.prof.phase[2])); out->ar_loop_ms = t;
        PTTS_HIP(hipEventElapsedTime(&t, m.prof.phase[3], m.prof.phase[4])); out->mimi_ms = t;
    }
    snprintf(out->kernel, sizeof out->kernel, "%s", "k_skinny");
    m.prof.used = 0; m.prof.bytes = 0; m.prof.wbytes = 0; m.prof.launches = 0; m.prof.phases = false;
}

void Model::compute_tcomb(float sv, float tv, float* dst) {
    const int C = d.flow_dim, nf = d.nfreq;
    DevBuf& wsb = work(WORK_TCOMB, (size_t)(2 * nf + 3 * C) * sizeof(float));
    float* feat = wsb.as<float>();
    float* h = feat + 2 * nf;
    float* e[2] = {h + C, h + 2 * C};
    const float tvals[2] = {sv, tv};
    for (int i = 0; i < 2; i++) {
        const auto& te = d.te[i];
        if (te.l1.in != 2 * nf) throw Error(PTTS_EFORMAT, "native: timestep embedder width mismatch");
        launch_timestep_features(tvals[i], at<float>(te.freqs), nf, feat, stream);
        GemmArgs g1 = mk(*this, feat, flat(2 * nf), te.l1, h, flat(C), 1);
        g1.epi = EPI_SILU;
        launch_gemm(g1, stream);
        GemmArgs g2 = mk(*this, h, flat(C), te.l2, e[i], flat(C), 1);
        launch_gemm(g2, stream);
        launch_rmsnorm_alpha(e[i], at<float>(te.alpha), 1e-5f, 1, C, stream);
    }
    launch_avg2(e[0], e[1], dst, C, stream);
}

const float* Model::tcomb_for(int n) {
    auto it = tcomb.find(n);
    if (it != tcomb.end()) return it->second->as<float>();
    std::unique_ptr<DevBuf> buf(new DevBuf());
    buf->ensure((size_t)n * d.flow_dim * sizeof(float));
    for (int i = 0; i < n; i++)
        compute_tcomb((float)i / (float)n, (float)(i + 1) / (float)n, buf->as<float>() + (size_t)i * d.flow_dim);
    PTTS_HIP(hipStreamSynchronize(stream));
    const float* p = buf->as<float>();
    tcomb[n] = std::move(buf);
    return p;
}

namespace {
struct PinnedPool {
    std::mutex mu;
    std::map<void*, size_t> owned;
    std::multimap<size_t, void*> free_blocks;
    size_t free_bytes = 0;
    static constexpr size_t kKeep = (size_t)1 << 30;
};
PinnedPool& pool() { static PinnedPool* p = new PinnedPool(); return *p; }
}

void* result_alloc(size_t bytes) {
    const size_t sz = (std::max<size_t>(bytes, 1) + 65535) & ~(size_t)65535;
    PinnedPool& pp = pool();
    {
        std::lock_guard<std::mutex> lock(pp.mu);
// ... 45 lines not shown
```

### go-pocket-tts_amd/csrc/runtime.h

```cpp
#pragma once

#include <atomic>
#include <functional>
#include <type_traits>

#include "kernels.h"
#include "model.h"
#include "row_ring.h"
#include "dsp_spec.h"
#include "host_rows.h"
#include "join.h"

namespace ptts {

struct DevBuf {
    void* p = nullptr;
    size_t n = 0;
    DevBuf() = default;
    DevBuf(const DevBuf&) = delete;
    DevBuf& operator=(const DevBuf&) = delete;
    ~DevBuf() { release(); }
    void release() {
        if (p) (void)hipFree(p);
        p = nullptr;
        n = 0;
    }
    void ensure(size_t bytes) {
        if (bytes <= n && p) return;
        release();
        if (bytes == 0) bytes = 256;
        PTTS_HIP(hipMalloc(&p, bytes));
        n = bytes;
    }
    template <class T> T* as() const { return reinterpret_cast<T*>(p); }
};

struct Batch;

struct PinnedBuf {
    void* p = nullptr;
    size_t n = 0;
    PinnedBuf() = default;
    PinnedBuf(const PinnedBuf&) = delete;
    PinnedBuf& operator=(const PinnedBuf&) = delete;
    ~PinnedBuf() { if (p) (void)hipHostFree(p); }
    void* ensure(size_t bytes) {
        if (bytes <= n && p) return p;
        if (p) (void)hipHostFree(p);
        p = nullptr;
        n = 0;
        PTTS_HIP(hipHostMalloc(&p, std::max<size_t>(bytes, 256), hipHostMallocDefault));
        n = std::max<size_t>(bytes, 256);
        return p;
    }
};

enum WorkSlot : size_t {
    WORK_TCOMB = 0,
    WORK_VOICE_RAW = 1,
    WORK_PROMPT_META = 2,
    WORK_PROMPT_ACT = 3,
    WORK_DECODER = 4,
    WORK_PROMPT_ROWS = 5,
    WORK_TEXT_ROWS = 5,
    WORK_PROMPT_UPLOAD = 5,
    WORK_PROMPT_IDS = 6,
    WORK_TEXT_IDS = 6,
    WORK_PCM = 7,
    WORK_CONT_PCM = 7,
    WORK_STREAM_S16 = 8,
    WORK_EGRESS_S16 = 8,
    WORK_DECODE_IO = 8,
    WORK_SPEAKER_IO = 8,
    WORK_NOISE_ROWS = 8,
    WORK_PREFILL_PLANES = 9,
    WORK_FLOW_DIRECTION = 9,
    WORK_VOICE_SLOTS = 10,
    WORK_PCM_ROWS = 11,
    WORK_NOISE_SPECS = 12,
    WORK_NOISE_ROWS_SPEC = 12,
    WORK_CONT_RESERVE = 13,
    WORK_CONT_RETIRE = 15,
    WORK_ENCODER = 16,
    WORK_ENCODER_LATENTS = 17,
    WORK_EMBEDDING_IO = 17,
    WORK_VOICE_BUILD_ROWS = 18,
    WORK_VOICE_EXPORT = 19,
    WORK_VOICE_BUILD_TABLE = 20,
    WORK_EGRESS_PAGEABLE = 24,
    WORK_CONVERT_IN = 25,
    WORK_CONVERT_OUT = 26,
    WORK_ENCODER_CLIP = 26,
    WORK_STREAM_SNAP = 27,
    WORK_STREAM_STAGE = 28,
    WORK_DSP_SCRATCH = 29,
    WORK_HOST_ROWS = 30,
    WORK_JOINED = 31,
    WORK_TRIMMED = 32,
    WORK_TRIM_SCRATCH = 33,
    WORK_TEMPO = 34,
    WORK_TEMPO_SCRATCH = 35,
    WORK_JOIN_CARRY = 36,
    WORK_JOIN_STAGE = 37,
    WORK_PITCH = 38,
    WORK_FORMANT_COEFFS = 39,
    WORK_FORMANT_RESIDUAL = 40,
    WORK_FORMANT_SHIFTED = 41,
};
constexpr size_t kWorkSlots = 42;

constexpr int kNativeRate = 24000;
constexpr int kResampleMaxL = 512;
constexpr int kResampleMaxTaps = 65536;
struct RateFilter {
    int L = 1, M = 1, K = 0, dlo = 0, tile = 0;
    int64_t A = 0;
    size_t n_taps = 0;
    float* staged = nullptr;
    DevBuf taps;
    hipEvent_t ready = nullptr;
    hipStream_t up = nullptr;
    RateFilter() = default;
    RateFilter(const RateFilter&) = delete;
    RateFilter& operator=(const RateFilter&) = delete;
    ~RateFilter();
};
struct UploadedTable {
    void* staged = nullptr;
    DevBuf image;
    hipEvent_t ready = nullptr;
    hipStream_t up = nullptr;
    UploadedTable() = default;
    UploadedTable(const UploadedTable&) = delete;
    UploadedTable& operator=(const UploadedTable&) = delete;
    ~UploadedTable();
};
struct Prof {
    bool on = false;
    std::vector<hipEvent_t> ev;
    size_t used = 0;
    double bytes = 0, wbytes = 0;
    int64_t launches = 0;
    hipEvent_t phase[5] = {};
    bool phases_on = false;
    bool phases = false;
};

struct UploadArena {
    char* base = nullptr;
    size_t cap = 0, off = 0;
};

struct Model {
    Desc d;
    ptts_opts opts;
    uint8_t* arena = nullptr;
    bool own_arena = false;
    int device = 0;
    hipStream_t stream = nullptr;
    hipStream_t stream2 = nullptr;
    std::vector<hipEvent_t> events;
    std::mutex mu;
    std::map<int, std::unique_ptr<DevBuf>> tcomb;
    DevBuf ws[kWorkSlots];
    std::unique_ptr<Batch> cached_batch;
    Prof prof;
    std::map<std::pair<int, int>, std::unique_ptr<RateFilter>> rate_filters;
    RowRing<ResampleRow> rs_ring;
    RowRing<CmpRow, kCmpMaxDesigns * kCmpScanBytes> cmp_ring;
    RowRing<LimRow, kLimMaxDesigns * kLimScanBytes> lim_ring;
    RowRing<DeRow, kDeMaxDesigns * kDeScanBytes> de_ring;
    RowRing<JoinRow> join_ring;
    RowRing<TrimRow, kTrimMaxDesigns * kTrimScanBytes> trim_ring;
    RowRing<TempoRow, kTempoMaxDesigns * kTempoScanBytes> tempo_ring;
    RowRing<PitchRow, kPitchMaxDesigns * kPitchScanBytes> pitch_ring;
    std::unique_ptr<UploadedTable> pitch_image;
    RowRing<FormantRow> formant_ring;
    std::unique_ptr<UploadedTable> formant_tables;
    PinnedBuf trim_info;
    RowRing<DspRow, kDspMaxEq * kDspEqBytes> dsp_ring;
    int fc_inject = 0;
    std::atomic<int64_t> fc_fallbacks{0};
    std::atomic<bool> fc_disabled{false};

    ~Model();
    template <class T> const T* at(size_t off) const { return off == NONE ? nullptr : reinterpret_cast<const T*>(arena + off); }
    UploadArena upload;
    DevBuf& work(WorkSlot slot, size_t bytes) {
        ws[slot].ensure(bytes);
        return ws[slot];
    }
    static_assert(!std::is_convertible<int, WorkSlot>::value && !std::is_convertible<size_t, WorkSlot>::value, "Model::work takes a WorkSlot name, never a number");
    void use_device() const { PTTS_HIP(hipSetDevice(device)); }
    uint64_t noise_state = 0;
    uint64_t next_noise_seed() {
        uint64_t z = (noise_state += 0x9E3779B97F4A7C15ull);
        z = (z ^ (z >> 30)) * 0xBF58476D1CE4E5B9ull;
        z = (z ^ (z >> 27)) * 0x94D049BB133111EBull;
        z ^= z >> 31;
        return z ? z : 1;
    }
    const float* tcomb_for(int lsd_steps);
    void compute_tcomb(float s, float t, float* dst );
};

struct PackedRows {
    std::vector<size_t> bytes, off;
    char* base = nullptr;
    PackedRows(Model& m, WorkSlot slot, std::vector<size_t> row_bytes, const bool* skip = nullptr) : bytes(std::move(row_bytes)), off(bytes.size()) {
        base = m.work(slot, std::max<size_t>(pack_rows(bytes.data(), skip, (int)bytes.size(), off.data()), kRowAlign)).as<char>();
    }
    char* row(int i) const { return base + off[(size_t)i]; }
    void upload(int i, const void* src, hipStream_t s) const { PTTS_HIP(hipMemcpyAsync(row(i), src, bytes[(size_t)i], hipMemcpyHostToDevice, s)); }
    void download(int i, void* dst, hipStream_t s) const { PTTS_HIP(hipMemcpyAsync(dst, row(i), bytes[(size_t)i], hipMemcpyDeviceToHost, s)); }
};

struct Batch {
    Model* m = nullptr;
    int B = 0;
    int cap = 0;
    int max_steps = 0;
    DevBuf kcache, vcache;
    DevBuf state_i32;
    DevBuf state_f32;
    StepState st{};
    std::vector<int32_t> kv_len_host;
    DevBuf pre_k, pre_v, pre_len;
    std::vector<const void*> pre_k_host, pre_v_host;
    std::vector<int32_t> pre_len_host;
    DevBuf in_raw, in32, x, xn, qkv, attn, ff, last, eos, sy, ada, fx, fh, fh2, cur, noise_step, partial;
    DevBuf latents;
    DevBuf noise;
    bool has_noise = false;
    bool opened = false;
    bool chain_ok = false;
    DevBuf fx2, cur2;
    DevBuf fc_xbuf, fc_sync, fc_stamps;
    bool fc_ok = false;
    DevBuf tp_a, tp_f;
    bool tall_ok = false;
    bool tail_fused = false;
    unsigned* fc_fault() const { return fc_sync.as<unsigned>() + 32 * kFlowClusterMaxTiles; }
    int par = 0;
    float* fx_now() const { return (par ? fx2 : fx).as<float>(); }
    float* cur_now() const { return (par ? cur2 : cur).as<float>(); }
    hipStream_t io_stream = nullptr;
    bool slot_local = false;
    int kv_bound = 0;
    bool capturing = false;
    hipGraphExec_t graphs[2][17][3] = {};
    int graph_steps[2][2] = {{0, 0}, {0, 0}};
    int graph_lsd = 0;
    int capture_keys = 0;
    int32_t* n_active_pinned = nullptr;
    PcmRow* rows_pinned = nullptr;
    DevBuf fin_dev;

    ~Batch();
    void drop_graphs();
    size_t kv_elem() const { return m->opts.kv == PTTS_KV_BF16 ? 2 : 4; }
    void* kc(int layer) const { return (char*)kcache.p + (size_t)layer * B * m->d.heads * cap * m->d.hd * kv_elem(); }
    void* vc(int layer) const { return (char*)vcache.p + (size_t)layer * B * m->d.heads * cap * m->d.hd * kv_elem(); }
};

void* result_alloc(size_t bytes);
void result_free(void* p);
bool result_is_pinned(const void* p);

struct Voice {
    Model* m = nullptr;
    int device = 0;
    int offset = 0;
    DevBuf k, v;
    size_t layer_bytes() const { return (size_t)m->d.heads * offset * m->d.hd * (m->opts.kv == PTTS_KV_BF16 ? 2 : 4); }
};
Voice* voice_create(Model& m, const float* const* caches, const int64_t* steps, const int64_t* offsets);
void batch_apply_voice(Batch& b, const Voice& v, const std::vector<int32_t>& slots);
bool voice_usable_by(const Voice& v, const Model& m);
std::vector<std::unique_ptr<Voice>> voice_build(Model& m, const float* const* emb, const int64_t* frames, int64_t width, int n);
void voice_export(const Voice& v, int layer0, int n_layers, float* out);
void voice_read_state(const Voice& v, int layer, float* out);
std::vector<uint8_t> voice_state_bytes(const Voice& v);

struct MimiWs {
    int B = 0, T = 0, P0 = 0;
    int Ls[4] = {0, 0, 0, 0}, Ps[4] = {0, 0, 0, 0};
    float *xp = nullptr, *up = nullptr, *n1 = nullptr, *qkv[MAX_LAYERS] = {nullptr}, *attn = nullptr, *ff = nullptr, *c0 = nullptr;
    float *u[3] = {nullptr, nullptr, nullptr}, *uo[3] = {nullptr, nullptr, nullptr}, *h[3] = {nullptr, nullptr, nullptr};
    bool zeroed = false;
};
constexpr int kMimiGroup = 64;
void mimi_setup(Model& m, MimiWs& w, int B, int T);
void mimi_range(Model& m, MimiWs& w, const float* lat, int64_t lat_bstride, int f0, int f1, float* pcm, float* mimi_latent, hipStream_t s,
                const PcmRow* pcm_rows = nullptr, bool* rows_used = nullptr, float* xformer_out = nullptr);

void mimi_layer_qkv(Model& m, int layer, const float* x, RowMap xmap, int R, float* qkv, RowMap qmap, int pos0, int rows_per_seg, float* n1, hipStream_t s);
void mimi_layer_ffn(Model& m, int layer, float* x, RowMap xmap, int R, float* n1, float* ffb, hipStream_t s);
void mimi_layer_qkv(Model& m, const Desc::ML& L, const float* x, RowMap xmap, int R, float* qkv, RowMap qmap, int pos0, int rows_per_seg, float* n1, hipStream_t s);
void mimi_layer_ffn(Model& m, const Desc::ML& L, float* x, RowMap xmap, int R, float* n1, float* ffb, hipStream_t s);

constexpr int kEncStages = 10;
int64_t mimi_encode_max_frames(const Desc& d);
void mimi_encode(Model& m, const float* const* pcm, const int64_t* n_samples, int n_clips, float* const* latent_out, float* const* stages = nullptr,
                 const int32_t* rates = nullptr);
int64_t mimi_encode_clip(Model& m, const float* pcm, int64_t n_samples, float* lat_dev, float* const* stages = nullptr, int rate = kNativeRate);
int64_t mimi_encode_samples(int64_t n_samples, int rate);
void require_encoder(const Desc& d);
void mimi_encode_stage_shapes(const Desc& d, int64_t n_samples, int64_t* shapes );
Model* model_open(Plan* plan, void* device_arena, int fill);
void profile_read(Model& m, ptts_profile* out);
Batch* batch_new(Model& m, int n_slots, int cap, int max_steps);
void batch_reset(Batch& b);
void batch_set_voice(Batch& b, int slot, const float* const* caches, const int64_t* steps, const int64_t* offsets);
void batch_prompt(Batch& b, const float* rows_dev, const int64_t* row_offsets);
bool step_core(Batch& b, int lsd_steps, bool opened = false, bool fuse_finish = false, bool chain = false);
void step_open(Batch& b);
struct FlowClusterFault : Error { using Error::Error; };
void flow_cluster_recover(Batch& b);
// ... 176 lines not shown
```

### go-pocket-tts_amd/runtime.py

```python
from __future__ import annotations

import ctypes as C
import os
import subprocess
import sys
from dataclasses import dataclass, field
from typing import Callable, Optional, Sequence

import numpy as np

_HERE = os.path.dirname(os.path.abspath(__file__))
LIB_PATH = os.environ.get("PTTS_LIB_PATH") or os.path.join(_HERE, "libptts_hip.so")

PTTS_OK, PTTS_EINVAL, PTTS_EIO, PTTS_EFORMAT, PTTS_ENODEVICE, PTTS_ECANCELLED, PTTS_ENOMEM = range(7)
WEIGHTS_F32, WEIGHTS_BF16, WEIGHTS_INT8 = 0, 1, 2
KV_F32, KV_BF16 = 0, 1
PCM_F32, PCM_S16, PCM_ULAW, PCM_ALAW = 0, 1, 2, 3
_PCM_DTYPES = {PCM_F32: "<f4", PCM_S16: "<i2", PCM_ULAW: "|u1", PCM_ALAW: "|u1"}

_FP = C.POINTER(C.c_float)
_IP = C.POINTER(C.c_int64)
_DP = C.POINTER(C.c_double)
_I32P = C.POINTER(C.c_int32)
_STEP_CB = C.CFUNCTYPE(None, C.c_void_p, C.c_int32, C.c_int32)
# ... 61 lines not shown
                         float(release_ms), float(drive_db))


class DeesserOpts(C.Structure):
    _fields_ = [("size", C.c_uint32), ("reserved", C.c_int32), ("freq_hz", C.c_double), ("q", C.c_double), ("threshold_db", C.c_double),
                ("ratio", C.c_double), ("knee_db", C.c_double), ("attack_ms", C.c_double), ("release_ms", C.c_double), ("max_reduction_db", C.c_double)]

    def __init__(self, freq_hz: float = 5000.0, q: float = 0.7071, threshold_db: float = -30.0, ratio: float = 4.0, knee_db: float = 6.0,
                 attack_ms: float = 1.0, release_ms: float = 60.0, max_reduction_db: float = 12.0, size: Optional[int] = None, reserved: int = 0):
        super().__init__(C.sizeof(DeesserOpts) if size is None else int(size), int(reserved), float(freq_hz), float(q), float(threshold_db),
                         float(ratio), float(knee_db), float(attack_ms), float(release_ms), float(max_reduction_db))


class TrimOpts(C.Structure):
    _fields_ = [("size", C.c_uint32), ("edges", C.c_int32), ("threshold_db", C.c_double), ("pad_ms", C.c_double), ("max_pause_ms", C.c_double)]

    def __init__(self, edges: int = 1, threshold_db: float = -50.0, pad_ms: float = 30.0, max_pause_ms: float = 0.0, size: Optional[int] = None):
        super().__init__(C.sizeof(TrimOpts) if size is None else int(size), int(edges), float(threshold_db), float(pad_ms), float(max_pause_ms))


class TrimInfo(C.Structure):
    _fields_ = [("lo", C.c_int64), ("hi", C.c_int64), ("n_out", C.c_int64), ("cuts", C.c_int64), ("speech", C.c_int32), ("reserved", C.c_int32)]

    def astuple(self):
        return (int(self.lo), int(self.hi), int(self.n_out), int(self.cuts), int(self.speech))


class TempoOpts(C.Structure):
    _fields_ = [("size", C.c_uint32), ("speed_permille", C.c_int32), ("reserved", C.c_int32 * 2)]

    def __init__(self, speed_permille: int = 1000, size: Optional[int] = None, reserved=(0, 0)):
        super().__init__(C.sizeof(TempoOpts) if size is None else int(size), int(speed_permille), (C.c_int32 * 2)(*[int(v) for v in reserved]))


class FormantOpts(C.Structure):
    _fields_ = [("size", C.c_uint32), ("keep", C.c_int32), ("reserved", C.c_int32 * 2)]

    def __init__(self, keep: int = 1, size: Optional[int] = None, reserved=(0, 0)):
        super().__init__(C.sizeof(FormantOpts) if size is None else int(size), int(keep), (C.c_int32 * 2)(*[int(v) for v in reserved]))


class PitchOpts(C.Structure):
    _fields_ = [("size", C.c_uint32), ("pitch_permille", C.c_int32), ("reserved", C.c_int32 * 2)]

    def __init__(self, pitch_permille: int = 1000, size: Optional[int] = None, reserved=(0, 0)):
        super().__init__(C.sizeof(PitchOpts) if size is None else int(size), int(pitch_permille), (C.c_int32 * 2)(*[int(v) for v in reserved]))


class JoinOpts(C.Structure):
    _fields_ = [("size", C.c_uint32), ("pcm_format", C.c_int32), ("sample_rate", C.c_int32), ("loudness", C.c_int32), ("dsp", C.POINTER(DspOpts)),
                ("gap_ms", C.c_double), ("crossfade_ms", C.c_double)]

    def __init__(self, gap_ms: float = 0.0, crossfade_ms: float = 0.0, pcm_format: int = 0, sample_rate: int = 0, loudness: int = 0,
                 dsp: Optional[DspOpts] = None, size: Optional[int] = None):
        super().__init__(C.sizeof(JoinOpts) if size is None else int(size), int(pcm_format), int(sample_rate), int(loudness),
                         C.pointer(dsp) if dsp is not None else None, float(gap_ms), float(crossfade_ms))
        self._dsp = dsp


class JoinStreamOpts(C.Structure):
    _fields_ = [("size", C.c_uint32), ("first_group", C.c_int32), ("pcm_callback", _PCM_CB), ("pcm_user", C.c_void_p)]

    def __init__(self, first_group: int = 0, pcm_callback=None, size: Optional[int] = None):
        super().__init__(C.sizeof(JoinStreamOpts) if size is None else int(size), int(first_group))
        if pcm_callback is not None:
            self.pcm_callback = pcm_callback
        self._cb = pcm_callback


class JoinPart(C.Structure):
    _fields_ = [("offset", C.c_int64), ("n_samples", C.c_int64), ("n_frames", C.c_int32), ("eos_step", C.c_int32), ("status", C.c_int32),
                ("reserved", C.c_int32)]


class EqSection(C.Structure):
    _fields_ = [("type", C.c_int32), ("reserved", C.c_int32), ("freq_hz", C.c_double), ("gain_db", C.c_double), ("q", C.c_double)]


EQ_LOWPASS, EQ_HIGHPASS, EQ_LOWSHELF, EQ_HIGHSHELF, EQ_PEAKING = 1, 2, 3, 4, 5


class _Request(C.Structure):
    _fields_ = [("tokens", _IP), ("n_tokens", C.c_int64), ("temperature", C.c_float), ("eos_threshold", C.c_float),
                ("max_steps", C.c_int32), ("estimated_max_steps", C.c_int32), ("lsd_steps", C.c_int32),
                ("frames_after_eos", C.c_int32), ("voice_embedding", _FP), ("voice_frames", C.c_int64),
                ("voice_caches", C.POINTER(_FP)), ("voice_cache_steps", _IP), ("voice_offsets", _IP), ("noise", _FP),
                ("step_callback", _STEP_CB), ("callback_user", C.c_void_p), ("cancel", C.POINTER(C.c_int32)),
                ("want_latents", C.c_int32), ("pcm_format", C.c_int32), ("voice", C.c_void_p), ("noise_seed", C.c_uint64), ("noise_rows", C.c_int32), ("loudness", C.c_int32),
                ("pcm_callback", _PCM_CB), ("pcm_user", C.c_void_p), ("stream_frames", C.c_int32), ("sample_rate", C.c_int32), ("dsp", C.POINTER(DspOpts))]


class _Profile(C.Structure):
    _fields_ = [("launches", C.c_int64), ("total_ms", C.c_double), ("algorithmic_bytes", C.c_double), ("kernel", C.c_char * 64),
                ("weight_bytes", C.c_double), ("prefill_ms", C.c_double), ("ar_loop_ms", C.c_double), ("mimi_ms", C.c_double)]


class _Result(C.Structure):
    _fields_ = [("pcm", _FP), ("n_samples", C.c_int64), ("latents", _FP), ("n_frames", C.c_int32), ("eos_step", C.c_int32),
                ("status", C.c_int32), ("pcm16", C.POINTER(C.c_int16)), ("pcm8", C.POINTER(C.c_uint8))]


_RESULT_DTYPE = np.dtype({"names": ["pcm", "n_samples", "latents", "n_frames", "eos_step", "status", "pcm16", "pcm8"],
                          "formats": ["<u8", "<i8", "<u8", "<i4", "<i4", "<i4", "<u8", "<u8"],
                          "offsets": [_Result.pcm.offset, _Result.n_samples.offset, _Result.latents.offset, _Result.n_frames.offset,
                                      _Result.eos_step.offset, _Result.status.offset, _Result.pcm16.offset, _Result.pcm8.offset],
                          "itemsize": C.sizeof(_Result)})

class _VoiceTensor(C.Structure):
    _fields_ = [("data", C.POINTER(C.c_float)), ("count", C.c_int64), ("rank", C.c_int32), ("reserved", C.c_int32), ("shape", C.c_int64 * 8)]


_lib = None

ABI_SYMBOLS = [
    "ptts_default_opts", "ptts_model_open", "ptts_model_open_bytes", "ptts_model_close", "ptts_model_info", "ptts_last_error",
    "ptts_plan_create", "ptts_plan_create_bytes", "ptts_plan_arena_bytes", "ptts_model_open_planned", "ptts_plan_free",
    "ptts_generate", "ptts_free_result", "ptts_text_embeddings", "ptts_batch_new", "ptts_batch_free", "ptts_batch_reset",
    "ptts_batch_set_voice_state", "ptts_batch_prompt", "ptts_batch_step", "ptts_batch_offsets", "ptts_batch_read_kv",
    "ptts_decode_latents", "ptts_noise_rows", "ptts_speaker_project", "ptts_mimi_encode", "ptts_mimi_encode_frames", "ptts_voice_encode_audio", "ptts_flow_direction", "ptts_op_linear", "ptts_op_layernorm", "ptts_op_rope",
    "ptts_op_attention_positions", "ptts_op_conv1d_leftpad", "ptts_op_convtr1d_righttrim", "ptts_version",
        "ptts_voice_create", "ptts_voice_free", "ptts_profile_enable", "ptts_profile_read", "ptts_plan_fill_host", "ptts_wav_header_streaming", "ptts_op_pcm16",
    "ptts_dispatcher_create", "ptts_dispatcher_create_custom", "ptts_dispatch_generate", "ptts_dispatcher_stats", "ptts_dispatcher_close",
    "ptts_model_share", "ptts_model_replicate", "ptts_model_set_use_graph", "ptts_model_set_max_batch", "ptts_text_estimate_max_frames", "ptts_text_frames_after_eos", "ptts_text_prepare", "ptts_text_chunks", "ptts_chunks_count",
    "ptts_chunks_get", "ptts_chunks_free",
    "ptts_tokenizer_open", "ptts_tokenizer_open_bytes", "ptts_tokenizer_free", "ptts_tokenizer_vocab_size", "ptts_tokenizer_encode",
    "ptts_tokenizer_encode_cb", "ptts_text_nfkc", "ptts_rccl_unique_id", "ptts_rccl_broadcast", "ptts_dsp_apply",
    "ptts_voice_file_open", "ptts_voice_file_open_bytes", "ptts_voice_file_close", "ptts_voice_file_kind", "ptts_voice_file_embedding",
    "ptts_voice_file_modules", "ptts_voice_file_module", "ptts_voice_file_state", "ptts_voice_open", "ptts_voice_open_bytes",
    "ptts_voice_from_embeddings", "ptts_voice_from_audio", "ptts_voice_offset", "ptts_voice_read_state", "ptts_voice_write", "ptts_voice_write_bytes",
    "ptts_voice_state_write_bytes", "ptts_voice_embedding_write", "ptts_free_bytes",
    "ptts_resample_length", "ptts_resample", "ptts_pcm_encode", "ptts_mimi_encode_rates", "ptts_voice_from_audio_rates", "ptts_wav_header",
    "ptts_dsp_rows", "ptts_loudness", "ptts_loudness_normalize", "ptts_loudness_rows", "ptts_loudness_normalize_rows",
    "ptts_eq_design", "ptts_eq_response", "ptts_eq_create", "ptts_eq_free", "ptts_eq_apply", "ptts_eq_rows",
    "ptts_dsp_ext_create", "ptts_dsp_ext_free", "ptts_true_peak", "ptts_true_peak_limit", "ptts_true_peak_rows",
    "ptts_dsp_ext_set_compressor", "ptts_compress_gain", "ptts_compress_apply", "ptts_compress_rows",
    "ptts_dsp_ext_set_limiter", "ptts_limit_apply", "ptts_limit_rows",
    "ptts_dsp_ext_set_deesser", "ptts_deess_apply", "ptts_deess_band", "ptts_deess_rows",
    "ptts_join_length", "ptts_join", "ptts_join_rows", "ptts_generate_joined", "ptts_generate_joined_streamed", "ptts_join_stream_ready",
    "ptts_trim_plan", "ptts_trim_apply", "ptts_trim_rows", "ptts_dsp_ext_set_trim",
    "ptts_tempo_length", "ptts_tempo_plan", "ptts_tempo_apply", "ptts_tempo_rows", "ptts_dsp_ext_set_tempo",
    "ptts_pitch_speed", "ptts_pitch_resample_length", "ptts_pitch_resample", "ptts_pitch_length", "ptts_pitch_apply", "ptts_pitch_table",
    "ptts_pitch_rows", "ptts_dsp_ext_set_pitch",
    "ptts_formant_frames", "ptts_formant_analyse", "ptts_formant_whiten", "ptts_formant_shape", "ptts_formant_apply", "ptts_formant_rows",
    "ptts_dsp_ext_set_formant",
    ]
HOOK_SYMBOLS = [
    "ptts_decode_stages", "ptts_mimi_layer_piece", "ptts_debug_last_attention_kernel", "ptts_debug_launch_counts", "ptts_debug_flow_cluster_inject",
    "ptts_debug_time_skinny", "ptts_debug_skinny_stamps", "ptts_debug_gemm", "ptts_debug_step_stamps", "ptts_debug_tall_linear",
    "ptts_debug_encode_stages", "ptts_debug_resample_launches", "ptts_debug_dsp_blocked_host",
    "ptts_debug_loudness_energies", "ptts_debug_kweighting", "ptts_debug_step_linear", "ptts_debug_true_peak_taps", "ptts_debug_true_peak_oversample",
    "ptts_debug_dsp_opts_error", "ptts_debug_resblock", "ptts_debug_resblock_plan", "ptts_debug_seanet_pack", "ptts_debug_plan_seanet_frags",
    "ptts_debug_gemm_rows", "ptts_debug_attn_step", "ptts_debug_attn_step_rounds", "ptts_debug_attn_window", "ptts_debug_flow_cluster",
    "ptts_debug_mimi_fused", "ptts_debug_mimi_pack", "ptts_debug_dsp_windows", "ptts_debug_step_edge",
]


def build(force: bool = False) -> str:
    args = ["make", "-s", "-C", _HERE, "-j8"]
    if force:
        args.append("-B")
    subprocess.check_call(args)
    return LIB_PATH


def lib():
    global _lib
    if _lib is None:
        if not os.path.exists(LIB_PATH):
            raise PttsError(PTTS_ENODEVICE, f"{LIB_PATH} is missing: run __graft_entry__.build() (no CPU fallback exists)")
        if "torch" not in sys.modules and not os.environ.get("PTTS_NO_TORCH_PRELOAD"):
            try:
                import torch
            except Exception:
                pass
        L = C.CDLL(LIB_PATH)
        L.ptts_last_error.restype = C.c_char_p
        L.ptts_version.restype = C.c_char_p
        L.ptts_plan_arena_bytes.restype = C.c_size_t
        L.ptts_plan_arena_bytes.argtypes = [C.c_void_p]
        L.ptts_plan_free.argtypes = [C.c_void_p]
        L.ptts_model_close.argtypes = [C.c_void_p]
        L.ptts_batch_free.argtypes = [C.c_void_p]
        L.ptts_model_open.argtypes = [C.c_char_p, C.POINTER(_Opts), C.POINTER(C.c_void_p)]
        L.ptts_model_open_bytes.argtypes = [C.c_void_p, C.c_size_t, C.POINTER(_Opts), C.POINTER(C.c_void_p)]
        L.ptts_plan_create.argtypes = [C.c_char_p, C.POINTER(_Opts), C.POINTER(C.c_void_p)]
        L.ptts_plan_create_bytes.argtypes = [C.c_void_p, C.c_size_t, C.POINTER(_Opts), C.POINTER(C.c_void_p)]
        L.ptts_model_open_planned.argtypes = [C.c_void_p, C.c_void_p, C.c_int, C.POINTER(C.c_void_p)]
        L.ptts_plan_fill_host.argtypes = [C.c_void_p, C.c_void_p]
        L.ptts_model_info.argtypes = [C.c_void_p, C.POINTER(_Info)]
        L.ptts_generate.argtypes = [C.c_void_p, C.POINTER(_Request), C.c_int32, C.POINTER(_Result)]
        L.ptts_free_result.argtypes = [C.POINTER(_Result)]
        L.ptts_text_embeddings.argtypes = [C.c_void_p, _IP, C.c_int64, _FP]
        L.ptts_batch_new.argtypes = [C.c_void_p, C.c_int32, C.c_int32, C.POINTER(C.c_void_p)]
        L.ptts_batch_reset.argtypes = [C.c_void_p]
        L.ptts_batch_set_voice_state.argtypes = [C.c_void_p, C.c_int32, C.POINTER(_FP), _IP, _IP]
        L.ptts_batch_prompt.argtypes = [C.c_void_p, _FP, _IP]
        L.ptts_batch_step.argtypes = [C.c_void_p, _FP, C.c_int32, _FP, _FP, _FP, _FP]
        L.ptts_batch_offsets.argtypes = [C.c_void_p, _IP]
        L.ptts_batch_read_kv.argtypes = [C.c_void_p, C.c_int32, C.c_int32, _FP, _FP]
        L.ptts_decode_latents.argtypes = [C.c_void_p, _FP, C.c_int32, C.c_int32, _FP, _FP]
        L.ptts_noise_rows.argtypes = [C.c_void_p, C.c_uint64, C.c_float, C.c_int32, _FP]
        L.ptts_flow_direction.argtypes = [C.c_void_p, _FP, C.c_float, C.c_float, _FP, C.c_int32, _FP]
        L.ptts_voice_create.argtypes = [C.c_void_p, C.POINTER(_FP), _IP, _IP, C.POINTER(C.c_void_p)]
        L.ptts_voice_free.argtypes = [C.c_void_p]
        L.ptts_voice_file_open.argtypes = [C.c_char_p, C.POINTER(C.c_void_p)]
        L.ptts_voice_file_open_bytes.argtypes = [C.c_void_p, C.c_size_t, C.POINTER(C.c_void_p)]
        L.ptts_voice_file_close.argtypes = [C.c_void_p]
        L.ptts_voice_file_close.restype = None
        L.ptts_voice_file_kind.argtypes = [C.c_void_p]
        L.ptts_voice_file_kind.restype = C.c_int32
        L.ptts_voice_file_embedding.argtypes = [C.c_void_p, C.POINTER(_FP), _IP]
        L.ptts_voice_file_modules.argtypes = [C.c_void_p, C.POINTER(C.c_int32)]
        L.ptts_voice_file_module.argtypes = [C.c_void_p, C.c_int32, C.POINTER(C.c_char_p), C.POINTER(_VoiceTensor), C.POINTER(_VoiceTensor)]
        L.ptts_voice_file_state.argtypes = [C.c_void_p, C.c_int32, C.c_int32, C.c_int32, C.POINTER(_FP), _IP, _IP]
        L.ptts_voice_open.argtypes = [C.c_void_p, C.c_char_p, C.POINTER(C.c_void_p)]
        L.ptts_voice_open_bytes.argtypes = [C.c_void_p, C.c_void_p, C.c_size_t, C.POINTER(C.c_void_p)]
        L.ptts_voice_from_embeddings.argtypes = [C.c_void_p, C.POINTER(_FP), _IP, C.c_int64, C.c_int32, C.POINTER(C.c_void_p)]
        L.ptts_voice_from_audio.argtypes = [C.c_void_p, C.POINTER(_FP), _IP, C.c_int32, C.POINTER(C.c_void_p)]
        L.ptts_voice_offset.argtypes = [C.c_void_p, C.POINTER(C.c_int64)]
        L.ptts_voice_read_state.argtypes = [C.c_void_p, C.c_int32, _FP]
        L.ptts_voice_write.argtypes = [C.c_void_p, C.c_char_p]
        L.ptts_voice_write_bytes.argtypes = [C.c_void_p, C.POINTER(C.POINTER(C.c_uint8)), C.POINTER(C.c_size_t)]
        L.ptts_voice_state_write_bytes.argtypes = [C.POINTER(_FP), C.c_int64, C.c_int32, C.c_int32, C.c_int32, C.POINTER(C.POINTER(C.c_uint8)),
                                                   C.POINTER(C.c_size_t)]
        L.ptts_voice_embedding_write.argtypes = [_FP, C.c_int64, C.c_int64, C.c_char_p]
        L.ptts_free_bytes.argtypes = [C.POINTER(C.c_uint8)]
        L.ptts_free_bytes.restype = None
        L.ptts_profile_enable.argtypes = [C.c_void_p, C.c_int32]
        L.ptts_profile_read.argtypes = [C.c_void_p, C.POINTER(_Profile)]
        L.ptts_op_linear.argtypes = [_FP, _FP, _FP, C.c_int64, C.c_int64, C.c_int64, _FP]
        L.ptts_op_layernorm.argtypes = [_FP, _FP, _FP, C.c_float, C.c_int64, C.c_int64, _FP]
        L.ptts_op_rope.argtypes = [_FP, _FP, _FP] + [C.c_int64] * 5
        L.ptts_op_attention_positions.argtypes = [_FP, _FP, _FP] + [C.c_int64] * 5 + [_IP, _IP, C.c_int64, _FP]
        L.ptts_op_conv1d_leftpad.argtypes = [_FP, _FP, _FP] + [C.c_int64] * 5 + [_FP]
        L.ptts_op_convtr1d_righttrim.argtypes = [_FP, _FP, _FP] + [C.c_int64] * 7 + [_FP]
        L.ptts_resample_length.restype = C.c_int64
        L.ptts_resample_length.argtypes = [C.c_int64, C.c_int32, C.c_int32]
        L.ptts_resample.argtypes = [C.c_void_p, C.POINTER(_FP), _IP, C.c_int32, C.c_int32, C.c_int32, C.POINTER(_FP)]
        L.ptts_pcm_encode.argtypes = [C.c_void_p, _FP, C.c_int64, C.c_int32, C.c_void_p]
        L.ptts_dsp_rows.argtypes = [C.c_void_p, C.POINTER(_FP), _IP, C.c_int32, C.POINTER(DspOpts), C.POINTER(_FP)]
        L.ptts_eq_rows.argtypes = [C.c_void_p, C.POINTER(C.c_void_p), C.POINTER(_FP), _IP, C.c_int32, C.POINTER(_FP)]
        L.ptts_true_peak_rows.argtypes = [C.c_void_p, C.POINTER(_FP), _IP, C.c_int32, _FP]
        L.ptts_dsp_ext_set_compressor.argtypes = [C.c_void_p, C.POINTER(CompressorOpts)]
        L.ptts_compress_gain.argtypes = [C.POINTER(CompressorOpts), C.c_double, _DP]
        L.ptts_compress_apply.argtypes = [C.POINTER(CompressorOpts), _FP, C.c_int64]
        L.ptts_compress_rows.argtypes = [C.c_void_p, C.POINTER(C.POINTER(CompressorOpts)), C.POINTER(_FP), _IP, C.c_int32, C.POINTER(_FP)]
        L.ptts_dsp_ext_set_limiter.argtypes = [C.c_void_p, C.POINTER(LimiterOpts)]
        L.ptts_limit_apply.argtypes = [C.POINTER(LimiterOpts), _FP, C.c_int64]
        L.ptts_limit_rows.argtypes = [C.c_void_p, C.POINTER(C.POINTER(LimiterOpts)), C.POINTER(_FP), _IP, C.c_int32, C.POINTER(_FP)]
        L.ptts_dsp_ext_set_deesser.argtypes = [C.c_void_p, C.POINTER(DeesserOpts)]
        L.ptts_deess_apply.argtypes = [C.POINTER(DeesserOpts), _FP, C.c_int64]
        L.ptts_deess_band.argtypes = [C.POINTER(DeesserOpts), _FP, C.c_int64, _FP]
        L.ptts_deess_rows.argtypes = [C.c_void_p, C.POINTER(C.POINTER(DeesserOpts)), C.POINTER(_FP), _IP, C.c_int32, C.POINTER(_FP)]
        L.ptts_join_length.restype = C.c_int64
        L.ptts_join_length.argtypes = [_IP, C.c_int32, C.POINTER(JoinOpts), _IP]
        L.ptts_join.argtypes = [C.POINTER(_FP), _IP, C.c_int32, C.POINTER(JoinOpts), _FP]
        L.ptts_join_rows.argtypes = [C.c_void_p, C.POINTER(_FP), _IP, C.c_int32, C.POINTER(JoinOpts), _FP]
        L.ptts_generate_joined.argtypes = [C.c_void_p, C.POINTER(_Request), C.c_int32, C.POINTER(JoinOpts), C.POINTER(_Result), C.POINTER(JoinPart)]
        L.ptts_generate_joined_streamed.argtypes = [C.c_void_p, C.POINTER(_Request), C.c_int32, C.POINTER(JoinOpts), C.POINTER(JoinStreamOpts), C.POINTER(_Result),
                                                    C.POINTER(JoinPart)]
        L.ptts_join_stream_ready.restype = C.c_int64
        L.ptts_join_stream_ready.argtypes = [C.POINTER(JoinOpts), C.c_int64]
        L.ptts_trim_plan.argtypes = [C.POINTER(TrimOpts), _FP, C.c_int64, C.POINTER(TrimInfo)]
        L.ptts_trim_apply.argtypes = [C.POINTER(TrimOpts), _FP, C.c_int64, _FP, C.POINTER(TrimInfo)]
        L.ptts_trim_rows.argtypes = [C.c_void_p, C.POINTER(C.POINTER(TrimOpts)), C.POINTER(_FP), _IP, C.c_int32, C.POINTER(_FP), C.POINTER(TrimInfo)]
        L.ptts_dsp_ext_set_trim.argtypes = [C.c_void_p, C.POINTER(TrimOpts)]
        L.ptts_tempo_length.argtypes = [C.POINTER(TempoOpts), C.c_int64]
        L.ptts_tempo_length.restype = C.c_int64
        L.ptts_tempo_plan.argtypes = [C.POINTER(TempoOpts), _FP, C.c_int64, C.POINTER(C.c_int32)]
        L.ptts_tempo_apply.argtypes = [C.POINTER(TempoOpts), _FP, C.c_int64, _FP]
        L.ptts_tempo_rows.argtypes = [C.c_void_p, C.POINTER(C.POINTER(TempoOpts)), C.POINTER(_FP), _IP, C.c_int32, C.POINTER(_FP), _IP]
        L.ptts_dsp_ext_set_tempo.argtypes = [C.c_void_p, C.POINTER(TempoOpts)]
        L.ptts_pitch_speed.argtypes = [C.POINTER(PitchOpts), C.POINTER(TempoOpts)]
        L.ptts_pitch_speed.restype = C.c_int32
        L.ptts_pitch_resample_length.argtypes = [C.POINTER(PitchOpts), C.c_int64]
        L.ptts_pitch_resample_length.restype = C.c_int64
        L.ptts_pitch_resample.argtypes = [C.POINTER(PitchOpts), _FP, C.c_int64, _FP]
        L.ptts_pitch_length.argtypes = [C.POINTER(PitchOpts), C.POINTER(TempoOpts), C.c_int64]
        L.ptts_pitch_length.restype = C.c_int64
        L.ptts_pitch_apply.argtypes = [C.POINTER(PitchOpts), C.POINTER(TempoOpts), _FP, C.c_int64, _FP]
        L.ptts_pitch_table.argtypes = [C.POINTER(_FP), C.POINTER(_FP), C.POINTER(C.c_int32)]
        L.ptts_pitch_rows.argtypes = [C.c_void_p, C.POINTER(C.POINTER(PitchOpts)), C.POINTER(C.POINTER(TempoOpts)), C.POINTER(_FP), _IP, C.c_int32,
                                      C.POINTER(_FP), _IP]
        L.ptts_dsp_ext_set_pitch.argtypes = [C.c_void_p, C.POINTER(PitchOpts)]
        L.ptts_formant_frames.argtypes = [C.c_int64]
        L.ptts_formant_frames.restype = C.c_int32
        L.ptts_formant_analyse.argtypes = [_FP, C.c_int64, _FP]
        L.ptts_formant_whiten.argtypes = [_FP, _FP, C.c_int64, _FP]
        L.ptts_formant_shape.argtypes = [_FP, C.c_int64, C.c_int32, _FP, C.c_int64, _FP]
        L.ptts_formant_apply.argtypes = [C.POINTER(FormantOpts), C.POINTER(PitchOpts), C.POINTER(TempoOpts), _FP, C.c_int64, _FP]
        L.ptts_formant_rows.argtypes = [C.c_void_p, C.POINTER(C.POINTER(FormantOpts)), C.POINTER(C.POINTER(PitchOpts)), C.POINTER(C.POINTER(TempoOpts)),
                                        C.POINTER(_FP), _IP, C.c_int32, C.POINTER(_FP), _IP]
        L.ptts_dsp_ext_set_formant.argtypes = [C.c_void_p, C.POINTER(FormantOpts)]
        L.ptts_loudness_rows.argtypes = [C.c_void_p, C.POINTER(_FP), _IP, C.c_int32, _DP]
        L.ptts_loudness_normalize_rows.argtypes = [C.c_void_p, C.POINTER(_FP), _IP, C.c_int32, C.c_double, C.POINTER(_FP), _DP]
        L.ptts_mimi_encode_rates.argtypes = [C.c_void_p, C.POINTER(_FP), _IP, C.POINTER(C.c_int32), C.c_int32, C.POINTER(_FP)]
        L.ptts_voice_from_audio_rates.argtypes = [C.c_void_p, C.POINTER(_FP), _IP, C.POINTER(C.c_int32), C.c_int32, C.POINTER(C.c_void_p)]
        L.ptts_wav_header.argtypes = [C.c_void_p, C.c_int32, C.c_int32, C.c_int32, C.c_int64]
        _lib = L
    return _lib


HOOKS_PATH = os.path.join(_HERE, "libptts_hooks.so")
_hooks = None


def hooks():
    global _hooks
    if _hooks is None:
        lib()
        if not os.path.exists(HOOKS_PATH):
            raise PttsError(PTTS_ENODEVICE, f"{HOOKS_PATH} is missing: run __graft_entry__.build()")
        H = C.CDLL(HOOKS_PATH, mode=C.RTLD_GLOBAL)
        H.ptts_decode_stages.argtypes = [C.c_void_p, _FP, C.c_int32, C.c_int32, _FP, _FP, _FP]
        H.ptts_debug_last_attention_kernel.restype = C.c_char_p
        H.ptts_debug_launch_counts.restype = C.c_int64
        H.ptts_debug_launch_counts.argtypes = [C.c_int32, C.c_char_p, C.c_int64]
        H.ptts_mimi_layer_piece.argtypes = [C.c_void_p, C.c_int32, C.c_int32, _FP, C.c_int64, C.c_int32, C.c_int32, _FP]
        H.ptts_debug_flow_cluster_inject.argtypes = [C.c_void_p, C.c_int32]
        H.ptts_debug_loudness_energies.argtypes = [C.c_void_p, C.POINTER(_FP), _IP, C.c_int32, C.POINTER(_DP)]
        H.ptts_debug_dsp_windows.argtypes = [C.c_void_p, C.POINTER(_FP), _IP, C.c_int32, C.POINTER(DspOpts), _IP, C.c_int32, C.POINTER(_FP)]
        H.ptts_debug_dsp_opts_error.restype = C.c_int64
        H.ptts_debug_dsp_opts_error.argtypes = [C.POINTER(DspOpts), C.c_char_p, C.c_int64]
        for name, args in (("flow_cluster", _FlowClusterArgs), ("step_linear", _StepLinearArgs), ("step_edge", _StepEdgeArgs), ("attn_step", _AttnStepArgs), ("attn_window", _AttnWindowArgs),
                           ("gemm_rows", _GemmRowsArgs), ("mimi_fused", _MimiFusedArgs), ("resblock", _ResblockArgs)):
            getattr(H, "ptts_debug_" + name).argtypes = [C.POINTER(args)]
        _hooks = H
    return _hooks


def _check(rc: int):
    if rc != PTTS_OK:
        msg = lib().ptts_last_error().decode(errors="replace")
        raise (Cancelled if rc == PTTS_ECANCELLED else PttsError)(rc, msg)


def _f32(a) -> np.ndarray:
    return np.ascontiguousarray(np.asarray(a, dtype=np.float32))


def _row_ptrs(arrays, ptr=_FP):
    return (ptr * max(len(arrays), 1))(*[C.cast(a.ctypes.data, ptr) for a in arrays])


def _rows_in(x):
    single = not isinstance(x, (list, tuple))
    rows = [_f32(x).reshape(-1)] if single else [_f32(r).reshape(-1) for r in x]
    return single, rows, len(rows), _row_ptrs(rows), np.array([r.size for r in rows] or [0], np.int64)


def _tempo_size(r, t):
    return r.size if t is None else r.size * 1000 // min(max(int(t.speed_permille), 500), 2000)


def _fp(a: Optional[np.ndarray]):
    return C.cast(a.ctypes.data, _FP) if a is not None else None


def _ip(a: np.ndarray):
    return C.cast(a.ctypes.data, _IP)


class _Keep:

    def __init__(self):
        self.arrays = []

    def _ptr(self, a, dtype, ptr):
        if a is None:
            return C.cast(None, ptr)
        a = np.ascontiguousarray(np.asarray(a, dtype=dtype))
        self.arrays.append(a)
        return C.cast(a.ctypes.data, ptr)

    def f32(self, a):
        return self._ptr(a, np.float32, _FP)

    def i32(self, a):
        return self._ptr(a, np.int32, _I32P)


def _census_dict(buf) -> dict:
    return {k: int(v) for k, v in (item.split("=") for item in buf.value.decode().split(";") if item)}



@dataclass
class VoiceEmbedding:
    data: np.ndarray
    shape: Sequence[int]

    def save(self, path: str) -> None:
        d = _f32(self.data).reshape(-1, int(self.shape[-1]))
        _check(lib().ptts_voice_embedding_write(_fp(d), d.shape[0], d.shape[1], os.fsencode(path)))


@dataclass
class VoiceModelState:
    modules: dict


@dataclass
class RuntimeGenerateConfig:
    temperature: float = 0.0
    eos_threshold: float = -4.0
    max_steps: int = 0
    estimated_max_steps: int = 0
    lsd_decode_steps: int = 1
    frames_after_eos: int = 0
    mimi_steps_per_latent: int = 0
    mimi_sequence_length: int = 0
    voice_embedding: Optional[VoiceEmbedding] = None
    voice_model_state: Optional[VoiceModelState] = None
    device_voice: Optional["DeviceVoice"] = None
    step_callback: Optional[Callable[[int, int], None]] = None
    noise: Optional[np.ndarray] = None
    noise_seed: int = 0
    cancel: Optional[np.ndarray] = None
    want_latents: bool = False
    pcm16: bool = False
    g711: str = ""
    sample_rate: int = 0
    pcm_callback: Optional[Callable[[int, np.ndarray], None]] = None
    stream_frames: int = 0
    normalize: bool = False
    dc_block: bool = False
    fade_in_ms: float = 0.0
    fade_out_ms: float = 0.0
    dsp_opts: Optional[DspOpts] = None
    loudness: int = 0
    eq: Optional["Eq"] = None
    true_peak_dbtp: Optional[float] = None
    compressor: Optional[CompressorOpts] = None
    limiter: Optional[LimiterOpts] = None
    deesser: Optional[DeesserOpts] = None


def _free_addr(addr: int):
    r = _Result()
    r.pcm = C.cast(C.c_void_p(addr), _FP)
    lib().ptts_free_result(C.byref(r))


class _OwnedBuffer:

    def __init__(self, ptr, n: int, typestr: str):
        self._addr = ptr if type(ptr) is int else C.cast(ptr, C.c_void_p).value
        self.__array_interface__ = {"shape": (n,), "typestr": typestr, "data": (self._addr, False), "version": 3}

    def __del__(self):
        if self._addr and sys is not None and not sys.is_finalizing():
            _free_addr(self._addr)
            self._addr = None


@dataclass
class GenerateResult:
    pcm: np.ndarray
    n_frames: int
    eos_step: int
    latents: Optional[np.ndarray] = None


@dataclass
class JoinedResult:
    pcm: np.ndarray
    n_frames: int
    parts: list


@dataclass
class ModelInfo:
    d_model: int; n_heads: int; n_layers: int; ffn: int; ldim: int; n_bins: int
    flow_dim: int; flow_depth: int; mimi_dim: int; mimi_heads: int; mimi_layers: int; mimi_context: int
    sample_rate: int; samples_per_frame: int; steps_per_latent: int
    frame_rate: float; encoder_frame_rate: float; n_params: int; arena_bytes: int; weights: int; kv: int


# ... 1079 lines not shown
    a.a_elems, a.c_elems = a_buf.size, int(c_elems)
    a.a_ld, a.a_rows_per_batch, a.a_batch_stride, a.a_off = (int(v) for v in amap)
    a.c_ld, a.c_rows_per_batch, a.c_batch_stride, a.c_off = (int(v) for v in cmap)
    a.A, a.W, a.bias, a.addvec, a.scale, a.gate = ptr(a_buf), ptr(w), ptr(bias), ptr(addvec), ptr(scale), ptr(gate)
    if residual is not None:
        residual = _f32(residual).reshape(-1)
        if residual.size != int(c_elems):
            raise ValueError("the residual is addressed like C: c_elems floats")
    a.R = ptr(residual)
    if rope is not None:
        cos, sin = _f32(rope[0]), _f32(rope[1])
        if cos.shape != sin.shape or cos.ndim != 2 or cos.shape[1] * 2 != int(rope_hd):
            raise ValueError("rope tables are [n_pos, rope_hd / 2]")
        a.rope_cos, a.rope_sin, a.n_pos = ptr(cos), ptr(sin), cos.shape[0]
        a.rope_cols, a.rope_hd, a.rope_pos0, a.rope_rows_per_seg = int(rope_cols), int(rope_hd), int(rope_pos0), int(rope_rows_per_seg)
        if rope_row_pos is not None:
            a.rope_row_pos = keep.i32(np.asarray(rope_row_pos, np.int32).reshape(int(M)))
    a.kslice, a.zstride, a.win_taps, a.win_c = int(kslice), int(zstride), int(win_taps), int(win_c)
    out = np.empty(int(c_elems), np.float32)
    a.C = ptr(out)
    name = C.create_string_buffer(512)
    a.launched, a.launched_cap = C.cast(name, C.c_char_p), 512
    info = (C.c_int32 * 2)()
    a.info = C.cast(info, _I32P)
    _check(hooks().ptts_debug_gemm_rows(C.byref(a)))
    return {"out": out, "launched": _census_dict(name), "cus": int(info[0]), "rgl": int(info[1])}


class _MimiFusedArgs(C.Structure):
    _fields_ = ([(n, C.c_int32) for n in ("kind", "M", "D", "F", "n_pos", "rope_cols", "pos0", "rows_per_seg", "ls_off", "reserved")] +
                [("eps", C.c_float), ("reserved_f", C.c_float)] +
                [(n, C.c_int64) for n in ("x_elems", "x_ld", "x_rows_per_batch", "x_batch_stride", "x_off", "y_elems", "y_ld", "y_rows_per_batch", "y_batch_stride",
                                          "y_off", "launched_cap")] +
                [(n, _FP) for n in ("x", "ln_w", "ln_b", "w1", "w2", "ls", "rope_cos", "rope_sin", "out")] + [("launched", C.c_char_p)])


MIMI_FFN, MIMI_ROWLIN = 0, 1


def debug_mimi_fused(kind, x_buf, M, *, xmap, ln_w, ln_b, w1, w2=None, eps=1e-5, ls=None, ls_off=0, D=None, F=None, y_elems=0, ymap=(0, 0, 0, 0), rope=None,
                     rope_cols=0, pos0=0, rows_per_seg=0):
    x_buf, w1 = _f32(x_buf).reshape(-1), _f32(w1)
    a, keep = _MimiFusedArgs(), _Keep()
    ptr = keep.f32
    a.kind, a.M, a.D, a.F = int(kind), int(M), int(w1.shape[1] if D is None else D), int(w1.shape[0] if F is None else F)
    a.eps, a.ls_off = float(eps), int(ls_off)
    a.x_elems = x_buf.size
    a.x_ld, a.x_rows_per_batch, a.x_batch_stride, a.x_off = (int(v) for v in xmap)
    a.y_elems = int(y_elems)
    a.y_ld, a.y_rows_per_batch, a.y_batch_stride, a.y_off = (int(v) for v in ymap)
    a.x, a.ln_w, a.ln_b, a.w1, a.w2, a.ls = ptr(x_buf), ptr(ln_w), ptr(ln_b), ptr(w1), ptr(w2), ptr(ls)
    if rope is not None:
        cos, sin = (None if t is None else _f32(t) for t in rope)
        a.rope_cos, a.rope_sin = ptr(cos), ptr(sin)
        a.n_pos = (cos if cos is not None else sin).shape[0]
        a.rope_cols, a.pos0, a.rows_per_seg = int(rope_cols), int(pos0), int(rows_per_seg)
    out = np.empty(x_buf.size if int(kind) == 0 else max(int(y_elems), 1), np.float32)
    a.out = ptr(out)
    name = C.create_string_buffer(512)
    a.launched, a.launched_cap = C.cast(name, C.c_char_p), 512
    _check(hooks().ptts_debug_mimi_fused(C.byref(a)))
    return {"out": out, "launched": _census_dict(name)}


def debug_mimi_pack(kind, w1, w2=None):
    w1 = _f32(w1)
    n = w1.shape[0]
    if w1.ndim != 2 or w1.shape[1] != 512 or (kind == 0 and (w2 is None or tuple(np.shape(w2)) != (512, n))):
        raise ValueError("w1 is [n, 512], w2 [512, n]")
    w2 = None if kind != 0 else _f32(w2)
    dst = np.empty(n * (1024 if kind == 0 else 512), np.uint16)
    H = hooks()
    H.ptts_debug_mimi_pack.argtypes = [C.c_int32, _FP, _FP, C.c_int32, C.c_void_p]
    _check(H.ptts_debug_mimi_pack(int(kind), _fp(w1), C.cast(None, _FP) if w2 is None else _fp(w2), n, dst.ctypes.data_as(C.c_void_p)))
    return dst.reshape((n // 32, 2, 16384) if kind == 0 else (n // 32, 16384))


class _ResblockArgs(C.Structure):
    _fields_ = ([(n, C.c_int32) for n in ("B", "L", "t0", "t1", "C", "H", "pad", "slack", "w_bf16", "final_conv", "form", "grid", "fuse_up", "x_pad", "x_L", "x_slack")] +
                [(n, _FP) for n in ("u", "w1", "w2", "wf", "b1", "b2", "bf", "xin", "wup", "bup")] +
                [("rows", C.POINTER(C.c_int32)), ("uo", _FP), ("pcm", _FP), ("row_out", C.c_void_p), ("row_bytes", C.c_int64), ("launched", C.POINTER(C.c_int32))])


RES_FORM_AUTO, RES_FORM_TILE, RES_FORM_PERS = 0, 1, 2


def debug_resblock(u, w1, w2, *, L=None, pad=2, slack=0, t0=0, t1=None, w_bf16=True, wf=None, b1=None, b2=None, bf=None, rows=None, row_bytes=None,
                   form=RES_FORM_AUTO, grid=0, xin=None, wup=None, bup=None, x_pad=1, x_slack=0):
    w1, w2 = _f32(w1), _f32(w2)
    h, c = w1.shape[0], w2.shape[0]
    a, keep = _ResblockArgs(), _Keep()
    ptr = keep.f32
    fused = xin is not None
    if fused:
        xin = _f32(xin)
        b, xl = xin.shape[0], xin.shape[1] - int(x_pad)
        L = 4 * xl if L is None else int(L)
    else:
        u = _f32(u)
        b = u.shape[0]
        L = u.shape[1] - int(pad) if L is None else int(L)
        xl = 0
    a.B, a.L, a.t0, a.t1, a.C, a.H, a.pad, a.slack = b, L, int(t0), L if t1 is None else int(t1), c, h, int(pad), int(slack)
    a.w_bf16, a.final_conv, a.form, a.grid, a.fuse_up, a.x_pad, a.x_L, a.x_slack = (1 if w_bf16 else 0), (1 if wf is not None else 0), int(form), int(grid), (1 if fused else 0), int(x_pad), xl, int(x_slack)
    a.u, a.w1, a.w2, a.wf, a.b1, a.b2, a.bf, a.xin, a.wup, a.bup = ptr(None if fused else u), ptr(w1), ptr(w2), ptr(wf), ptr(b1), ptr(b2), ptr(bf), ptr(xin), ptr(wup), ptr(bup)
    final = wf is not None
    uo = None if final else np.empty((b, int(pad) + L + int(slack), c), np.float32)
    pcm = np.empty((b, L), np.float32) if final else None
    a.uo, a.pcm = ptr(uo), ptr(pcm)
    ro = None
    if rows is not None:
        a.rows = keep.i32(np.asarray(rows, np.int32).reshape(b, 2))
        a.row_bytes = ((4 * L + 8 * 4 + 15) // 16) * 16 if row_bytes is None else int(row_bytes)
        ro = np.empty((b, max(int(a.row_bytes), 0)), np.uint8)
        a.row_out = ro.ctypes.data_as(C.c_void_p)
    cnt = (C.c_int32 * 5)()
    a.launched = C.cast(cnt, _I32P)
    _check(hooks().ptts_debug_resblock(C.byref(a)))
    return {"uo": uo, "pcm": pcm, "rows": ro, "plan": tuple(int(v) for v in cnt)}


def debug_resblock_plan(c, final_conv, w_bf16, batch, rows, cus, *, fuse_up=False, form=RES_FORM_AUTO, grid=0):
    out = (C.c_int32 * 5)()
    H = hooks()
    H.ptts_debug_resblock_plan.argtypes = [C.c_int32] * 9 + [C.POINTER(C.c_int32)]
    _check(H.ptts_debug_resblock_plan(int(c), 1 if final_conv else 0, 1 if w_bf16 else 0, 1 if fuse_up else 0, int(batch), int(rows), int(form), int(grid), int(cus), out))
    return tuple(int(v) for v in out)


def debug_seanet_pack(kind, rm, want_lo=True):
    rm = _f32(rm)
    out, inn = (16, rm.shape[0]) if kind == 2 else rm.shape
    hi = np.empty(out * inn, np.uint16)
    lo = np.empty(out * inn, np.uint16) if (want_lo or kind == 2) else None
    H = hooks()
    H.ptts_debug_seanet_pack.argtypes = [C.c_int32, _FP, C.c_int32, C.c_int32, C.c_void_p, C.c_void_p]
    _check(H.ptts_debug_seanet_pack(int(kind), _fp(rm), 1 if kind == 2 else out, inn, hi.ctypes.data_as(C.c_void_p), lo.ctypes.data_as(C.c_void_p) if lo is not None else None))
    return hi, lo


def debug_plan_seanet_frags(plan, item):
    H = hooks()
    H.ptts_debug_plan_seanet_frags.argtypes = [C.c_void_p, C.c_int32, C.c_void_p, C.c_void_p, C.c_int64, C.POINTER(C.c_int64), C.POINTER(C.c_int32)]
    n, dims = C.c_int64(0), (C.c_int32 * 3)()
    _check(H.ptts_debug_plan_seanet_frags(plan, int(item), None, None, 0, C.byref(n), dims))
    if n.value == 0:
        return None
    hi = np.empty(n.value, np.uint16)
    lo = np.empty(n.value, np.uint16) if dims[2] else None
    _check(H.ptts_debug_plan_seanet_frags(plan, int(item), hi.ctypes.data_as(C.c_void_p), lo.ctypes.data_as(C.c_void_p) if lo is not None else None, n.value, C.byref(n), dims))
    return hi, lo, (int(dims[0]), int(dims[1]))


def last_attention_kernel() -> str:
    return hooks().ptts_debug_last_attention_kernel().decode()


def mimi_encode_frames(n_samples: int) -> int:
    L = lib()
    L.ptts_mimi_encode_frames.argtypes = [C.c_int64]
    L.ptts_mimi_encode_frames.restype = C.c_int64
    return int(L.ptts_mimi_encode_frames(int(n_samples)))


def resample_launches(reset: bool = True) -> int:
    H = hooks()
    H.ptts_debug_resample_launches.restype = C.c_int64
    H.ptts_debug_resample_launches.argtypes = [C.c_int32]
    return int(H.ptts_debug_resample_launches(1 if reset else 0))


def launch_counts(on: bool) -> dict:
    buf = C.create_string_buffer(4096)
    hooks().ptts_debug_launch_counts(1 if on else 0, buf, 4096)
    return _census_dict(buf)


def op_conv1d_leftpad(x, w, bias=None) -> np.ndarray:
    x, w = _f32(x), _f32(w)
    b, cin, ln = x.shape
    cout, _, k = w.shape
    y = np.empty((b, cout, ln), np.float32)
    ba = _f32(bias) if bias is not None else None
    _check(lib().ptts_op_conv1d_leftpad(_fp(x), _fp(w), _fp(ba), b, cin, ln, cout, k, _fp(y)))
    return y


def op_convtr1d_righttrim(x, w, bias, stride: int, groups: int = 1) -> np.ndarray:
    x, w = _f32(x), _f32(w)
    b, cin, ln = x.shape
    _, opg, k = w.shape
    y = np.empty((b, opg * groups, ln * stride), np.float32)
    ba = _f32(bias) if bias is not None else None
    _check(lib().ptts_op_convtr1d_righttrim(_fp(x), _fp(w), _fp(ba), b, cin, ln, opg, k, stride, groups, _fp(y)))
    return y


def wav_header_streaming() -> bytes:
    buf = (C.c_uint8 * 44)()
    lib().ptts_wav_header_streaming(buf)
    return bytes(buf)


def _pcm_format(cfg) -> int:
    g = getattr(cfg, "g711", "") or ""
    if g:
        if g not in ("ulaw", "alaw"):
            raise PttsError(PTTS_EINVAL, f'g711 must be "ulaw" or "alaw", got {g!r}')
        return PCM_ULAW if g == "ulaw" else PCM_ALAW
    return PCM_S16 if getattr(cfg, "pcm16", False) else PCM_F32


def _rates(sample_rate, n: int) -> np.ndarray:
    r = np.asarray(sample_rate, np.int32).reshape(-1)
    return np.ascontiguousarray(np.broadcast_to(r, (max(n, 1),)) if r.size == 1 else r, np.int32)


def resample_length(n_in: int, in_rate: int, out_rate: int) -> int:
    return int(lib().ptts_resample_length(int(n_in), int(in_rate), int(out_rate)))


def wav_header(sample_rate: int = 24000, pcm_format: int = PCM_S16, n_samples: int = -1) -> bytes:
    buf = (C.c_uint8 * 64)()
    n = lib().ptts_wav_header(buf, 64, int(sample_rate), int(pcm_format), int(n_samples))
    if n < 0:
        raise PttsError(-n, lib().ptts_last_error().decode(errors="replace"))
    return bytes(buf[:n])


def op_pcm16(samples) -> np.ndarray:
    x = np.ascontiguousarray(samples, np.float32).reshape(-1)
    out = np.zeros(x.size, np.int16)
    L = lib()
    L.ptts_op_pcm16.argtypes = [C.c_void_p, C.c_int64, C.c_void_p]
    _check(L.ptts_op_pcm16(x.ctypes.data, x.size, out.ctypes.data))
    return out


class _DispatchOpts(C.Structure):
    _fields_ = [("max_batch", C.c_int32), ("window_us", C.c_int32), ("queue_cap", C.c_int32), ("continuous", C.c_int32), ("cont_kv_capacity", C.c_int32),
                ("cont_max_steps", C.c_int32), ("cont_steps_per_group", C.c_int32), ("reserved", C.c_int32 * 1)]


class _DispatchStats(C.Structure):
    _fields_ = [("requests", C.c_int64), ("batches", C.c_int64), ("cancelled_waiting", C.c_int64), ("max_queue_depth", C.c_int64),
                ("mean_batch", C.c_double), ("mean_wait_us", C.c_double), ("mean_exec_us", C.c_double), ("cont_steps", C.c_int64), ("cont_slot_steps", C.c_int64), ("flow_cluster_fallbacks", C.c_int64)]


DISPATCH_EXEC = C.CFUNCTYPE(C.c_int, C.c_void_p, C.c_int32, C.POINTER(_Request), C.c_int32, C.POINTER(_Result), C.c_void_p, C.c_int32)


class Dispatcher:

    def __init__(self, models: Sequence[Model], max_batch: int = 0, window_us: int = 2000, queue_cap: int = 0, _custom_exec=None, _workers: int = 1,
                 continuous: Optional[bool] = None, cont_kv_capacity: int = 0, cont_max_steps: int = 0, cont_steps_per_group: int = 0):
        L = lib()
        L.ptts_dispatcher_create.argtypes = [C.POINTER(C.c_void_p), C.c_int32, C.POINTER(_DispatchOpts), C.POINTER(C.c_void_p)]
        L.ptts_dispatcher_create_custom.argtypes = [DISPATCH_EXEC, C.c_void_p, C.c_int32, C.POINTER(_DispatchOpts), C.POINTER(C.c_void_p)]
        L.ptts_dispatch_generate.argtypes = [C.c_void_p, C.POINTER(_Request), C.POINTER(_Result)]
        L.ptts_dispatcher_stats.argtypes = [C.c_void_p, C.POINTER(_DispatchStats)]
        L.ptts_dispatcher_close.argtypes = [C.c_void_p]
        o = _DispatchOpts(max_batch=max_batch, window_us=window_us, queue_cap=queue_cap, continuous=0 if continuous is None else (1 if continuous else -1), cont_kv_capacity=cont_kv_capacity,
                          cont_max_steps=cont_max_steps, cont_steps_per_group=cont_steps_per_group)
        h = C.c_void_p()
        self.models = list(models)
        if _custom_exec is not None:
            self._exec = DISPATCH_EXEC(_custom_exec)
            _check(L.ptts_dispatcher_create_custom(self._exec, None, _workers, C.byref(o), C.byref(h)))
        else:
            arr = (C.c_void_p * len(self.models))(*[m.h for m in self.models])
            _check(L.ptts_dispatcher_create(arr, len(self.models), C.byref(o), C.byref(h)))
        self.h = h.value

    def generate(self, tokens: Sequence[int], cfg: RuntimeGenerateConfig) -> GenerateResult:
        req, res, keep = _Request(), _Result(), []
        m = self.models[0] if self.models else None
        if m is not None:
            m._fill_request(req, tokens, cfg, keep)
        else:
            t = np.ascontiguousarray(tokens, np.int64)
            keep.append(t)
            req.tokens, req.n_tokens = _ip(t), t.size
            if cfg.cancel is not None:
                req.cancel = cfg.cancel.ctypes.data_as(C.POINTER(C.c_int32))
        rc = lib().ptts_dispatch_generate(self.h, C.byref(req), C.byref(res))
        try:
            _check(rc)
            if m is None:
                return GenerateResult(np.zeros(0, np.float32), int(res.n_frames), int(res.eos_step), None)
            return m._take_result(res, cfg)
        finally:
            lib().ptts_free_result(C.byref(res))

    def stats(self) -> dict:
        s = _DispatchStats()
        lib().ptts_dispatcher_stats(self.h, C.byref(s))
        return {n: getattr(s, n) for n, _ in _DispatchStats._fields_ if n != "reserved"}

    def close(self):
        if self.h:
            lib().ptts_dispatcher_close(self.h)
            self.h = None

    def __del__(self):
        if sys is None or sys.is_finalizing():
            return
# ... 623 lines not shown
```

### include/ptts_debug.h

```cpp
#ifndef PTTS_DEBUG_H
#define PTTS_DEBUG_H

#include "ptts.h"

#ifdef __cplusplus
extern "C" {
#endif

#define PTTS_MIMI_PIECE_QKV 0
#define PTTS_MIMI_PIECE_FFN 1
int  ptts_mimi_layer_piece(ptts_model* m, int32_t layer, int32_t which, const float* x, int64_t rows, int32_t pos0, int32_t rows_per_seg, float* out);

int  ptts_decode_stages(ptts_model* m, const float* latents, int32_t n_utt, int32_t frames,
                        float* pcm, float* mimi_latent, float* transformer_out);

int  ptts_debug_encode_stages(ptts_model* m, const float* pcm, int64_t n_samples, float* const* stages, int64_t* shapes);

int ptts_debug_time_skinny(int32_t M, int32_t N, int32_t K, int32_t w_bf16, int32_t splitk, int32_t fuse_ln, int32_t iters, float* avg_us);
int ptts_debug_skinny_stamps(int32_t M, int32_t N, int32_t K, int32_t w_bf16, int32_t splitk, int32_t fuse_ln, uint64_t* out ,
                             int32_t max_blocks, int32_t* n_blocks);
int ptts_debug_step_stamps(ptts_batch* b, int32_t lsd_steps, uint64_t* out , int64_t cap_blocks, int32_t* desc ,
                           int32_t cap_desc, int32_t* n_desc);
int ptts_debug_gemm(int32_t M, int32_t N, int32_t K, int32_t w_bf16, int32_t variant, int32_t epi, int32_t iters, float* avg_us,
                    float* maxdiff);

int ptts_debug_tall_linear(int32_t M, int32_t N, int32_t K, int32_t epi, int32_t splitk, const float* x, const float* planes, int32_t psplit, const float* pbias,
                           const float* ln_w, const float* ln_b, float eps, const float* W, const float* bias, const float* R, int32_t out_planes, float* out,
                           float* x_out);

typedef struct ptts_step_linear_args {
    int32_t M, N, K, lda, ldc, wfmt, epi, splitk, tail, path, ldg, ln, ldmod, psplit, r_in_c, zrows, pgate, reserved;
    float alpha, eps;
    const float *x, *W, *bias, *addvec, *R, *scale, *gate, *ln_w, *ln_b, *shift, *mscale, *planes, *pbias;
    float *C, *tail_out, *x_out, *y_out, *w_eff, *w_scale;
    int32_t* launches;
} ptts_step_linear_args;
int ptts_debug_step_linear(const ptts_step_linear_args* a);

#define PTTS_STEP_EDGE_BEGIN 0
#define PTTS_STEP_EDGE_BEGIN_LIN 1
#define PTTS_STEP_EDGE_FINISH 2
#define PTTS_STEP_EDGE_FIN 3
#define PTTS_STEP_EDGE_FIN_CHAIN 4
typedef struct ptts_step_edge_args {
    int32_t op, B, rows, S, ldim, d_in, d_pj, lin_bf16, N, K, wfmt, epi, ldmod, reserved;
    float alpha, eps;
    int64_t lat_stride, noise_stride, launched_cap;
    int32_t *kv_len, *active, *step, *countdown, *n_frames, *eos_step, *max_steps, *frames_after_eos, *broke, *n_active;
    float* eos_threshold;
    float* latents;
    const float *noise, *bos, *eos_logit, *frame;
    const void *w_in, *w_pj;
    const float *b_in, *b_pj;
    const float *fx_in, *W, *bias, *shift, *mscale;
    float* cur;
    float *in32, *x0, *x, *fx, *w_eff, *w_scale;
    char* launched;
} ptts_step_edge_args;
int ptts_debug_step_edge(const ptts_step_edge_args* a);

typedef struct ptts_attn_step_args {
    int32_t kv_bf16, heads, rows, layers, layer, cap, keys_now, n_pre;
    int64_t qkv_ld, out_ld, kernel_cap;
    const float *qkv, *cos_t, *sin_t;
    const int32_t *seg_len, *active, *pre_len, *voice_of_row;
    const void* pre_k[4];
    const void* pre_v[4];
    int32_t pre_rows[4];
    void *k, *v;
    float* out;
    char* kernel;
    int32_t* info;
} ptts_attn_step_args;
int ptts_debug_attn_step(const ptts_attn_step_args* a);
int ptts_debug_attn_step_rounds(int32_t keys, int32_t kv_bf16, int32_t* keys_per_round);

typedef struct ptts_attn_window_args {
    int32_t form, ragged, kv_bf16, heads, segs, context, T1, t0, CT, cap, rows, reserved;
    int64_t ld, out_ld, kernel_cap, launched_cap;
    const float* qkv;
    const void *k, *v;
    const int32_t *rag_off, *rag_pos0;
    float* out;
    char *kernel, *launched;
} ptts_attn_window_args;
int ptts_debug_attn_window(const ptts_attn_window_args* a);

typedef struct ptts_gemm_rows_args {
    int32_t M, N, K, ldw, w_bf16, aop, epi, kernel, cfg, rgl, r_in_c, ldg, rope_cols, rope_hd, rope_pos0, rope_rows_per_seg, n_pos, kslice, win_taps, win_c;
    float alpha;
    int32_t reserved;
    int64_t a_elems, a_ld, a_rows_per_batch, a_batch_stride, a_off, c_elems, c_ld, c_rows_per_batch, c_batch_stride, c_off, zstride, launched_cap;
    const float *A, *W, *bias, *addvec, *scale, *gate, *R, *rope_cos, *rope_sin;
    const int32_t* rope_row_pos;
    float* C;
    char* launched;
    int32_t* info;
} ptts_gemm_rows_args;
int ptts_debug_gemm_rows(const ptts_gemm_rows_args* a);

typedef struct ptts_resblock_args {
    int32_t B, L, t0, t1, C, H, pad, slack, w_bf16, final_conv, form, grid, fuse_up, x_pad, x_L, x_slack;
    const float *u, *w1, *w2, *wf, *b1, *b2, *bf, *xin, *wup, *bup;
    const int32_t* rows;
    float *uo, *pcm;
    uint8_t* row_out;
    int64_t row_bytes;
    int32_t* launched;
} ptts_resblock_args;
int ptts_debug_resblock(const ptts_resblock_args* a);
int ptts_debug_resblock_plan(int32_t C, int32_t final_conv, int32_t w_bf16, int32_t fuse_up, int32_t B, int32_t rows, int32_t form, int32_t grid, int32_t cus,
                             int32_t* out);
int ptts_debug_seanet_pack(int32_t kind, const float* rm, int32_t out, int32_t in, uint16_t* hi, uint16_t* lo);
int ptts_debug_plan_seanet_frags(ptts_plan* p, int32_t item, uint16_t* hi, uint16_t* lo, int64_t cap, int64_t* count, int32_t* dims);

const char* ptts_debug_last_attention_kernel(void);

int64_t ptts_debug_launch_counts(int32_t on, char* out, int64_t cap);
int64_t ptts_debug_resample_launches(int32_t reset);

int ptts_debug_dsp_blocked_host(const float* in, int64_t n, float* out);

int ptts_debug_dsp_windows(ptts_model* m, const float* const* in, const int64_t* n, int32_t rows, const ptts_dsp_opts* opts,
                           const int64_t* cuts, int32_t n_cuts, float* const* out);

int ptts_debug_loudness_energies(ptts_model* m, const float* const* in, const int64_t* n, int32_t rows, double* const* out);
int ptts_debug_kweighting(int32_t sample_rate, double out[10]);

int ptts_debug_flow_cluster_inject(ptts_model* m, int32_t block);

typedef struct ptts_flow_cluster_args {
    int32_t rows, depth, n_launch, in_place;
    uint32_t tag_base0;
    int32_t reserved;
    int64_t ldmod, launched_cap;
    const float *fx, *ada, *ln_w, *ln_b, *b0, *b2, *eps, *w0, *w2;
    const int32_t* launch_rows;
    float *out, *fx_back;
    uint32_t* state;
    char* launched;
} ptts_flow_cluster_args;
int ptts_debug_flow_cluster(const ptts_flow_cluster_args* a);

typedef struct ptts_mimi_fused_args {
    int32_t kind, M, D, F, n_pos, rope_cols, pos0, rows_per_seg, ls_off, reserved;
    float eps, reserved_f;
    int64_t x_elems, x_ld, x_rows_per_batch, x_batch_stride, x_off, y_elems, y_ld, y_rows_per_batch, y_batch_stride, y_off, launched_cap;
    const float *x, *ln_w, *ln_b, *w1, *w2, *ls, *rope_cos, *rope_sin;
    float* out;
    char* launched;
} ptts_mimi_fused_args;
int ptts_debug_mimi_fused(const ptts_mimi_fused_args* a);
int ptts_debug_mimi_pack(int32_t kind, const float* w1, const float* w2, int32_t n, uint16_t* dst);

int64_t ptts_debug_dsp_opts_error(const ptts_dsp_opts* opts, char* out, int64_t cap);
int ptts_debug_true_peak_taps(float* out , int32_t* L, int32_t* K, int32_t* dlo);
int ptts_debug_true_peak_oversample(const float* samples, int64_t n, float* y );

#ifdef __cplusplus
}
#endif
#endif
```

Before: 12830 x real-time.

## Fuse first SEANet resblock into one streaming kernel with packed weight image

Adds k_resblock_stream, a kernel that runs the first decoder resblock (3-tap conv to hidden, ELU, 1x1 conv back, residual add, ELU) in one pass. Each tile streams hidden-channel chunks of a pre-packed bf16 weight image through LDS, so the hidden activation never goes to global memory and one launch replaces two GEMM launches. The image is built once on the host from the arena weights and cached on the model. It shares the FFN kernel's gemm helpers, which move into a common header. The cost is a one-time host pack at workspace setup and a new code path restricted to C=256, k1=3, k2=1.

```diff
diff --git a/go-pocket-tts_amd/csrc/capi_hooks.cpp b/go-pocket-tts_amd/csrc/capi_hooks.cpp
--- a/go-pocket-tts_amd/csrc/capi_hooks.cpp
+++ b/go-pocket-tts_amd/csrc/capi_hooks.cpp
@@ -1197,6 +1197,91 @@
     });
 }
 
+int ptts_debug_resblock_stream_pack(const float* w1, const float* w2, int32_t H, uint16_t* dst) {
+    return guard([&] {
+        if (!w1 || !w2 || !dst || H < 32 || H % 32 || H > 4096) throw Error(PTTS_EINVAL, "ptts_debug_resblock_stream_pack: bad arguments");
+        pack_rbs_image(w1, w2, H, dst);
+    });
+}
+
+int ptts_debug_plan_resblock_stream_image(ptts_plan* hp, uint16_t* dst, int64_t cap, int64_t* count) {
+    return guard([&] {
+        if (!hp || !count) throw Error(PTTS_EINVAL, "ptts_debug_plan_resblock_stream_image: bad arguments");
+        const Desc& d = hp->p.desc;
+        const size_t n = rbs_image_wanted(d) ? rbs_image_count(d.sea_hidden[0]) : 0;
+        *count = (int64_t)n;
+        if (!n || !dst) return;
+        if ((int64_t)n > cap) throw Error(PTTS_EINVAL, "ptts_debug_plan_resblock_stream_image: buffer too small");
+        std::vector<uint8_t> host(d.total_bytes);
+        plan_fill(hp->p, host.data());
+        rbs_image_from_arena(d, reinterpret_cast<const uint16_t*>(host.data() + d.rb1[0].w), reinterpret_cast<const uint16_t*>(host.data() + d.rb2[0].w), dst);
+    });
+}
+
+int ptts_debug_resblock_stream(const ptts_resblock_stream_args* pa) {
+    return guard([&] {
+        if (!pa) throw Error(PTTS_EINVAL, "ptts_debug_resblock_stream: null argument");
+        const ptts_resblock_stream_args& t = *pa;
+        if (!t.u || !t.w1 || !t.w2 || !t.uo || t.B < 1 || t.B > 256 || t.L < 1 || t.L > (1 << 22) || t.t0 < 0 || t.t1 <= t.t0 || t.t1 > t.L || t.pad < 0 || t.pad > 64 ||
+            t.C < 1 || t.C > 4096 || t.H < 1 || t.H > 4096 || t.form < 0 || t.form > 1)
+            throw Error(PTTS_EINVAL, "ptts_debug_resblock_stream: bad arguments");
+        const int B = t.B, C = t.C, H = t.H, rn = t.t1 - t.t0;
+        if (t.u_bs < (int64_t)(t.pad + t.L) * C || (int64_t)B * t.u_bs > ((int64_t)1 << 31))
+            throw Error(PTTS_EINVAL, strfmt("ptts_debug_resblock_stream: u_bs %lld, an utterance has (pad + L) C = %lld floats", (long long)t.u_bs, (long long)(t.pad + t.L) * C));
+        require_device();
+        const size_t u_elems = (size_t)B * (size_t)t.u_bs;
+        Stage st;
+        const float* dU = st.in(t.u, u_elems);
+        float* dUo = st.out(u_elems);
+        const float* dB1 = st.in(t.b1, (size_t)H);
+        const float* dB2 = st.in(t.b2, (size_t)C);
+        LaunchScope launches;
+        if (t.form == 0) {
+            const size_t img_entries = std::max<size_t>(rbs_image_count(H), 32768);
+            uint16_t* dImg = st.out<uint16_t>(img_entries);
+            ResStreamArgs a;
+            a.u = dU; a.uo = dUo; a.u_bs = t.u_bs; a.pad = t.pad;
+            a.img = dImg; a.b1 = dB1; a.b2 = dB2;
+            a.B = B; a.L = t.L; a.t0 = t.t0; a.t1 = t.t1;
+            a.C = C; a.H = H; a.k1 = 3; a.k2 = 1;
+            if (!resblock_stream_supported(a)) throw Error(PTTS_EINVAL, "ptts_debug_resblock_stream: refused by resblock_stream_supported");
+            std::vector<uint16_t> img(img_entries);
+            pack_rbs_image(t.w1, t.w2, H, img.data());
+            up(dImg, img.data(), img_entries * 2);
+            launches.run([&] { launch_resblock_stream(a, nullptr); });
+        } else {
+            if (t.pad < 2 || t.u_bs % 4) throw Error(PTTS_EINVAL, "ptts_debug_resblock_stream: the two-launch form reads two rows of history through 16-byte loads (pad < 2 or u_bs % 4)");
+            std::vector<uint16_t> w1b((size_t)H * 3 * C), w2b((size_t)C * H);
+            for (size_t i = 0; i < w1b.size(); i++) w1b[i] = f32_to_bf16_rne(t.w1[i]);
+            for (size_t i = 0; i < w2b.size(); i++) w2b[i] = f32_to_bf16_rne(t.w2[i]);
+            const uint16_t* dW1 = st.in(w1b.data(), w1b.size());
+            const uint16_t* dW2 = st.in(w2b.data(), w2b.size());
+            float* dH = st.out((size_t)B * t.L * H);
+            const int64_t h_bs = (int64_t)t.L * H;
+            GemmArgs g1;
+            g1.A = dU + (size_t)(t.pad - 2 + t.t0) * C; g1.amap = seg(C, rn, t.u_bs);
+            g1.W = dW1; g1.w_bf16 = 1; g1.ldw = 3 * C; g1.bias = dB1;
+            g1.C = dH + (size_t)t.t0 * H; g1.cmap = seg(H, rn, h_bs);
+            g1.M = B * rn; g1.N = H; g1.K = 3 * C;
+            g1.aop = AOP_ELU; g1.epi = EPI_ELU;
+            if (C % 64 == 0) { g1.win_taps = 3; g1.win_c = C; }
+            GemmArgs g2;
+            g2.A = dH + (size_t)t.t0 * H; g2.amap = seg(H, rn, h_bs);
+            g2.W = dW2; g2.w_bf16 = 1; g2.ldw = H; g2.bias = dB2;
+            g2.C = dUo + (size_t)(t.pad + t.t0) * C; g2.cmap = seg(C, rn, t.u_bs);
+            g2.R = dU + (size_t)(t.pad + t.t0) * C; g2.epi = EPI_RESADD_ELU;
+            g2.M = B * rn; g2.N = C; g2.K = H;
+            if (!gemm5_supported(g1) || !gemm5_supported(g2)) throw Error(PTTS_EINVAL, "ptts_debug_resblock_stream: the two-launch form is compared on k_gemm5's shapes (refused by gemm5_supported)");
+            launches.run([&] { launch_gemm(g1, nullptr); launch_gemm(g2, nullptr); });
+        }
+        PTTS_HIP(hipGetLastError());
+        PTTS_HIP(hipDeviceSynchronize());
+        put_str(t.launched, t.launched_cap, launches.str());
+        down(t.uo, dUo, u_elems * 4);
+        if (t.u_back) down(t.u_back, dU, u_elems * 4);
+    });
+}
+
 int ptts_mimi_layer_piece(ptts_model* h, int32_t layer, int32_t which, const float* x, int64_t rows, int32_t pos0, int32_t rows_per_seg, float* out) {
     return guard([&] {
         if (!h || !h->m) throw Error(PTTS_EINVAL, "native-safetensors runtime unavailable");
diff --git a/go-pocket-tts_amd/csrc/ffn_fused.hip b/go-pocket-tts_amd/csrc/ffn_fused.hip
--- a/go-pocket-tts_amd/csrc/ffn_fused.hip
+++ b/go-pocket-tts_amd/csrc/ffn_fused.hip
@@ -4,6 +4,7 @@
 #include "kernels.h"
 #include "device_util.h"
 #include "mfma_util.h"
+#include "ffn_stream.h"
 
 namespace ptts {
 
@@ -24,20 +25,11 @@
 }
 
 constexpr int FF_D = 512;
-constexpr int FF_CH = 32;
 constexpr int FF_KS = FF_D / 32;
 constexpr int FF_OT = FF_D / 16;
 constexpr int FF_W1B = FF_CH * FF_D * 2;
 constexpr int FF_W2B = FF_D * FF_CH * 2;
 constexpr int FF_IMG = FF_W1B + FF_W2B;
-
-__device__ __forceinline__ void ff_dma32k(const char* src, char* dst, int wave, int lane) {
-#pragma unroll
-    for (int i = 0; i < 8; i++) {
-        const int idx = i * 4 + wave;
-        lds_dma1k(src + idx * 1024 + lane * 16, dst + idx * 1024);
-    }
-}
 
 __device__ __forceinline__ void ff_rows_layernorm(const float* xrow, const float* ln_w, const float* ln_b, float eps, int q, Frag (&xh)[16], Frag (&xl)[16]) {
     float4 v[16][2];
@@ -80,39 +72,6 @@
         split2(o[0].z, o[0].w, xh[s].u[1], xl[s].u[1]);
         split2(o[1].x, o[1].y, xh[s].u[2], xl[s].u[2]);
         split2(o[1].z, o[1].w, xh[s].u[3], xl[s].u[3]);
-    }
-}
-
-template <class Piece>
-__device__ __forceinline__ void ff_gemm1(const char* w1, int r16, int q, const Frag (&xh)[16], const Frag (&xl)[16], f32x4 (&acc)[2], Piece&& piece) {
-    const int sw1 = (r16 >> 1) & 7;
-    acc[0] = f32x4{0.f, 0.f, 0.f, 0.f};
-    acc[1] = f32x4{0.f, 0.f, 0.f, 0.f};
-    Frag wa[2], wb[2];
-    const char* wl = w1 + r16 * 128;
-    wa[0].q = *reinterpret_cast<const uint4*>(wl + ((q ^ sw1) << 4));
-    wb[0].q = *reinterpret_cast<const uint4*>(wl + ((q ^ sw1) << 4) + 2048);
-#pragma unroll
-    for (int s = 0; s < 16; s++) {
-        __builtin_amdgcn_sched_barrier(0);
-        if (s + 1 < 16) {
-            const int off = ((s + 1) >> 1) * 4096 + (((4 * ((s + 1) & 1) + q) ^ sw1) << 4);
-            wa[(s + 1) & 1].q = *reinterpret_cast<const uint4*>(wl + off);
-            wb[(s + 1) & 1].q = *reinterpret_cast<const uint4*>(wl + off + 2048);
-        }
-        acc[0] = __builtin_amdgcn_mfma_f32_16x16x32_bf16(wa[s & 1].v, xh[s].v, acc[0], 0, 0, 0);
-        acc[1] = __builtin_amdgcn_mfma_f32_16x16x32_bf16(wb[s & 1].v, xh[s].v, acc[1], 0, 0, 0);
-        PTTS_LO_MFMA(acc[0] = __builtin_amdgcn_mfma_f32_16x16x32_bf16(wa[s & 1].v, xl[s].v, acc[0], 0, 0, 0));
-        PTTS_LO_MFMA(acc[1] = __builtin_amdgcn_mfma_f32_16x16x32_bf16(wb[s & 1].v, xl[s].v, acc[1], 0, 0, 0));
-        piece(s);
-        asm volatile("" : "+a"(acc[0]), "+a"(acc[1]));
-        if (s + 1 < 16) __builtin_amdgcn_sched_group_barrier(0x100, 2, 0);
-#pragma unroll
-        for (int i = 0; i < 4; i++) {
-            __builtin_amdgcn_sched_group_barrier(0x008, 1, 0);
-            __builtin_amdgcn_sched_group_barrier(0x002, 3, 0);
-        }
-        __builtin_amdgcn_sched_barrier(0);
     }
 }
 
@@ -128,9 +87,9 @@
     auto w1s = [&](int i) { return lds + i * FF_W1B; };
     auto w2s = [&](int i) { return lds + 2 * FF_W1B + i * FF_W2B; };
 
-    ff_dma32k(img, w1s(0), wave, lane);
-    ff_dma32k(img + FF_W1B, w2s(0), wave, lane);
-    ff_dma32k(img + (size_t)min(1, nch - 1) * FF_IMG, w1s(1), wave, lane);
+    ff_dma<32>(img, w1s(0), wave, lane);
+    ff_dma<32>(img + FF_W1B, w2s(0), wave, lane);
+    ff_dma<32>(img + (size_t)min(1, nch - 1) * FF_IMG, w1s(1), wave, lane);
 
     const int m0 = blockIdx.x * 64 + wave * 16;
     const int row = min(m0 + r16, a.M - 1);
@@ -169,18 +128,7 @@
             }
         });
         const char* w2 = w2s(c & 1) + w2_lane;
-        Frag w2f[2];
-        w2f[0].q = *reinterpret_cast<const uint4*>(w2);
-#pragma unroll
-        for (int t = 0; t < FF_OT; t++) {
-            __builtin_amdgcn_sched_barrier(0);
-            if (t + 1 < FF_OT) w2f[(t + 1) & 1].q = *reinterpret_cast<const uint4*>(w2 + (t + 1) * 1024);
-            acc2[t] = __builtin_amdgcn_mfma_f32_16x16x32_bf16(w2f[t & 1].v, hh.v, acc2[t], 0, 0, 0);
-            PTTS_LO_MFMA(acc2[t] = __builtin_amdgcn_mfma_f32_16x16x32_bf16(w2f[t & 1].v, hl.v, acc2[t], 0, 0, 0));
-            if (t + 1 < FF_OT) __builtin_amdgcn_sched_group_barrier(0x100, 1, 0);
-            __builtin_amdgcn_sched_group_barrier(0x008, 2, 0);
-            __builtin_amdgcn_sched_barrier(0);
-        }
+        ff_gemm2(w2, hh, hl, acc2);
         acc1[0] = acc1n[0];
         acc1[1] = acc1n[1];
     }
@@ -221,8 +169,8 @@
     const int r16 = lane & 15, q = lane >> 4;
     const int nch = a.N / FF_CH;
     const char* img = reinterpret_cast<const char*>(a.img);
-    ff_dma32k(img, lds, wave, lane);
-    ff_dma32k(img + (size_t)min(1, nch - 1) * FF_W1B, lds + FF_W1B, wave, lane);
+    ff_dma<32>(img, lds, wave, lane);
+    ff_dma<32>(img + (size_t)min(1, nch - 1) * FF_W1B, lds + FF_W1B, wave, lane);
 
     const int m0 = blockIdx.x * 64 + wave * 16;
     const int row = min(m0 + r16, a.M - 1);
diff --git a/go-pocket-tts_amd/csrc/ffn_stream.h b/go-pocket-tts_amd/csrc/ffn_stream.h
--- /dev/null
+++ b/go-pocket-tts_amd/csrc/ffn_stream.h
@@ -0,0 +1,69 @@
+#pragma once
+
+#include "device_util.h"
+#include "mfma_util.h"
+
+namespace ptts {
+
+constexpr int FF_CH = 32;
+
+template <int KB>
+__device__ __forceinline__ void ff_dma(const char* src, char* dst, int wave, int lane) {
+    static_assert(KB % 4 == 0, "whole wave-instructions per wave");
+#pragma unroll
+    for (int i = 0; i < KB / 4; i++) {
+        const int idx = i * 4 + wave;
+        lds_dma1k(src + idx * 1024 + lane * 16, dst + idx * 1024);
+    }
+}
+
+template <int KS, class Piece>
+__device__ __forceinline__ void ff_gemm1(const char* w1, int r16, int q, const Frag (&xh)[KS], const Frag (&xl)[KS], f32x4 (&acc)[2], Piece&& piece) {
+    const int sw1 = (r16 >> 1) & 7;
+    acc[0] = f32x4{0.f, 0.f, 0.f, 0.f};
+    acc[1] = f32x4{0.f, 0.f, 0.f, 0.f};
+    Frag wa[2], wb[2];
+    const char* wl = w1 + r16 * 128;
+    wa[0].q = *reinterpret_cast<const uint4*>(wl + ((q ^ sw1) << 4));
+    wb[0].q = *reinterpret_cast<const uint4*>(wl + ((q ^ sw1) << 4) + 2048);
+#pragma unroll
+    for (int s = 0; s < KS; s++) {
+        __builtin_amdgcn_sched_barrier(0);
+        if (s + 1 < KS) {
+            const int off = ((s + 1) >> 1) * 4096 + (((4 * ((s + 1) & 1) + q) ^ sw1) << 4);
+            wa[(s + 1) & 1].q = *reinterpret_cast<const uint4*>(wl + off);
+            wb[(s + 1) & 1].q = *reinterpret_cast<const uint4*>(wl + off + 2048);
+        }
+        acc[0] = __builtin_amdgcn_mfma_f32_16x16x32_bf16(wa[s & 1].v, xh[s].v, acc[0], 0, 0, 0);
+        acc[1] = __builtin_amdgcn_mfma_f32_16x16x32_bf16(wb[s & 1].v, xh[s].v, acc[1], 0, 0, 0);
+        PTTS_LO_MFMA(acc[0] = __builtin_amdgcn_mfma_f32_16x16x32_bf16(wa[s & 1].v, xl[s].v, acc[0], 0, 0, 0));
+        PTTS_LO_MFMA(acc[1] = __builtin_amdgcn_mfma_f32_16x16x32_bf16(wb[s & 1].v, xl[s].v, acc[1], 0, 0, 0));
+        piece(s);
+        asm volatile("" : "+a"(acc[0]), "+a"(acc[1]));
+        if (s + 1 < KS) __builtin_amdgcn_sched_group_barrier(0x100, 2, 0);
+#pragma unroll
+        for (int i = 0; i < 4; i++) {
+            __builtin_amdgcn_sched_group_barrier(0x008, 1, 0);
+            __builtin_amdgcn_sched_group_barrier(0x002, 3, 0);
+        }
+        __builtin_amdgcn_sched_barrier(0);
+    }
+}
+
+template <int OT>
+__device__ __forceinline__ void ff_gemm2(const char* w2, const Frag& hh, const Frag& hl, f32x4 (&acc2)[OT]) {
+    Frag w2f[2];
+    w2f[0].q = *reinterpret_cast<const uint4*>(w2);
+#pragma unroll
+    for (int t = 0; t < OT; t++) {
+        __builtin_amdgcn_sched_barrier(0);
+        if (t + 1 < OT) w2f[(t + 1) & 1].q = *reinterpret_cast<const uint4*>(w2 + (t + 1) * 1024);
+        acc2[t] = __builtin_amdgcn_mfma_f32_16x16x32_bf16(w2f[t & 1].v, hh.v, acc2[t], 0, 0, 0);
+        PTTS_LO_MFMA(acc2[t] = __builtin_amdgcn_mfma_f32_16x16x32_bf16(w2f[t & 1].v, hl.v, acc2[t], 0, 0, 0));
+        if (t + 1 < OT) __builtin_amdgcn_sched_group_barrier(0x100, 1, 0);
+        __builtin_amdgcn_sched_group_barrier(0x008, 2, 0);
+        __builtin_amdgcn_sched_barrier(0);
+    }
+}
+
+}
diff --git a/go-pocket-tts_amd/csrc/kernels.h b/go-pocket-tts_amd/csrc/kernels.h
--- a/go-pocket-tts_amd/csrc/kernels.h
+++ b/go-pocket-tts_amd/csrc/kernels.h
@@ -431,6 +431,15 @@
 bool mimi_ffn_supported(const FfnArgs& a);
 void launch_mimi_ffn(const FfnArgs& a, hipStream_t stream);
 
+struct ResStreamArgs {
+    const float* u = nullptr; float* uo = nullptr; int64_t u_bs = 0; int pad = 0;
+    const void* img = nullptr; const float* b1 = nullptr; const float* b2 = nullptr;
+    int B = 0, L = 0, t0 = 0, t1 = 0;
+    int C = 0, H = 0, k1 = 0, k2 = 0;
+};
+bool resblock_stream_supported(const ResStreamArgs& a);
+void launch_resblock_stream(const ResStreamArgs& a, hipStream_t stream);
+
 constexpr int FC_MAX_DEPTH = 8;
 struct FlowClusterArgs {
     const float* fx_in = nullptr; float* fx_out = nullptr;
diff --git a/go-pocket-tts_amd/csrc/mimi_decode.cpp b/go-pocket-tts_amd/csrc/mimi_decode.cpp
--- a/go-pocket-tts_amd/csrc/mimi_decode.cpp
+++ b/go-pocket-tts_amd/csrc/mimi_decode.cpp
@@ -32,6 +32,7 @@
     w.c0 = p; p += n_c[0];
     for (int j = 0; j < 3; j++) { w.u[j] = p; p += n_c[j + 1]; w.uo[j] = p; p += n_c[j + 1]; w.h[j] = p; p += n_h[j]; }
     w.zeroed = false;
+    (void)m.rb_image();
 }
 
 void mimi_zero_history(Model& m, MimiWs& w, hipStream_t s) {
@@ -202,6 +203,14 @@
                 continue;
             }
         }
+        if (j == 0 && m.rb_img_buf.p) {
+            ResStreamArgs rs;
+            rs.u = u; rs.uo = uo; rs.u_bs = u_bs; rs.pad = Pout;
+            rs.img = m.rb_img_buf.p; rs.b1 = m.at<float>(d.rb1[j].b); rs.b2 = m.at<float>(d.rb2[j].b);
+            rs.B = B; rs.L = Lout; rs.t0 = r0; rs.t1 = r0 + rn;
+            rs.C = cout; rs.H = hid; rs.k1 = d.rb_k1[j]; rs.k2 = d.rb_k2[j];
+            if (resblock_stream_supported(rs)) { launch_resblock_stream(rs, s); continue; }
+        }
         GemmArgs g1 = mk(m, u + (size_t)(Pout - (d.rb_k1[j] - 1) + r0) * cout, seg(cout, rn, u_bs), d.rb1[j],
                          hb + (size_t)(Ph + r0) * hid, seg(hid, rn, h_bs), B * rn);
         g1.aop = AOP_ELU; g1.epi = EPI_ELU;
diff --git a/go-pocket-tts_amd/csrc/model.cpp b/go-pocket-tts_amd/csrc/model.cpp
--- a/go-pocket-tts_amd/csrc/model.cpp
+++ b/go-pocket-tts_amd/csrc/model.cpp
@@ -119,6 +119,45 @@
                     p[e] = f32_to_bf16_rne(w2[(size_t)o * F + hcol]);
                 }
             }
+    }
+}
+
+size_t rbs_image_count(int H) { return (size_t)(H / 32) * 32768; }
+bool rbs_image_wanted(const Desc& d) {
+    const int H = d.sea_hidden[0];
+    return d.rb1[0].bf16 && d.rb2[0].bf16 && d.rb1[0].w != NONE && d.rb2[0].w != NONE && d.sea_ch[1] == 256 && d.rb_k1[0] == 3 && d.rb_k2[0] == 1 && H >= 32 && H % 32 == 0 &&
+           d.rb1[0].in == 3 * 256 && d.rb1[0].out == H && d.rb2[0].in == H && d.rb2[0].out == 256;
+}
+void rbs_image_from_arena(const Desc& d, const uint16_t* w1_bf16, const uint16_t* w2_bf16, uint16_t* dst) {
+    const int H = d.sea_hidden[0];
+    std::vector<float> w1((size_t)H * 768), w2((size_t)256 * H);
+    for (size_t i = 0; i < w1.size(); i++) w1[i] = bf16_to_f32(w1_bf16[i]);
+    for (size_t i = 0; i < w2.size(); i++) w2[i] = bf16_to_f32(w2_bf16[i]);
+    pack_rbs_image(w1.data(), w2.data(), H, dst);
+}
+void pack_rbs_image(const float* w1, const float* w2, int H, uint16_t* dst) {
+    const int C = 256, K = 3 * C, nch = H / 32;
+    for (int c = 0; c < nch; c++) {
+        uint16_t* i1 = dst + (size_t)c * 32768;
+        uint16_t* i2 = i1 + 24576;
+        for (int j = 0; j < 12; j++)
+            for (int h = 0; h < 32; h++) {
+                const int ht = h >> 4, i = h & 15, unit = 32 * c + 8 * (i >> 2) + 4 * ht + (i & 3);
+                for (int sg = 0; sg < 2; sg++)
+                    for (int q = 0; q < 4; q++) {
+                        const int pos = (4 * sg + q) ^ ((h >> 1) & 7), koff = C * (j % 3) + 64 * (j / 3) + 32 * sg;
+                        uint16_t* p = i1 + ((size_t)j * 32 + h) * 64 + pos * 8;
+                        for (int e = 0; e < 8; e++) p[e] = f32_to_bf16_rne(w1[(size_t)unit * K + koff + 8 * q + e]);
+                    }
+            }
+        for (int o = 0; o < C; o++) {
+            const int t = o >> 4, i = o & 15, ch = 64 * (t >> 2) + 32 * ((t >> 1) & 1) + 8 * (i >> 2) + 4 * (t & 1) + (i & 3);
+            for (int q = 0; q < 4; q++) {
+                const int pos = q ^ (3 * ((o >> 3) & 1));
+                uint16_t* p = i2 + (size_t)o * 32 + pos * 8;
+                for (int e = 0; e < 8; e++) p[e] = f32_to_bf16_rne(w2[(size_t)ch * H + 32 * c + 8 * q + e]);
+            }
+        }
     }
 }
 
diff --git a/go-pocket-tts_amd/csrc/model.h b/go-pocket-tts_amd/csrc/model.h
--- a/go-pocket-tts_amd/csrc/model.h
+++ b/go-pocket-tts_amd/csrc/model.h
@@ -27,6 +27,11 @@
 size_t ffn_image_count(int F);
 void pack_w1_image(const float* rm, int N, uint16_t* dst);
 void pack_ffn_image(const float* w1, const float* w2, int F, uint16_t* dst);
+size_t rbs_image_count(int H);
+void pack_rbs_image(const float* w1, const float* w2, int H, uint16_t* dst);
+struct Desc;
+bool rbs_image_wanted(const Desc& d);
+void rbs_image_from_arena(const Desc& d, const uint16_t* w1_bf16, const uint16_t* w2_bf16, uint16_t* dst);
 
 struct Norm {
     size_t w = NONE, b = NONE;
diff --git a/go-pocket-tts_amd/csrc/resblock_stream.hip b/go-pocket-tts_amd/csrc/resblock_stream.hip
--- /dev/null
+++ b/go-pocket-tts_amd/csrc/resblock_stream.hip
@@ -0,0 +1,167 @@
+#include <algorithm>
+#include <cstdlib>
+
+#include "kernels.h"
+#include "device_util.h"
+#include "mfma_util.h"
+#include "ffn_stream.h"
+
+namespace ptts {
+
+namespace {
+
+constexpr int RS_C = 256;
+constexpr int RS_KS = 3 * RS_C / 32;
+constexpr int RS_OT = RS_C / 16;
+constexpr int RS_W1B = FF_CH * 3 * RS_C * 2;
+constexpr int RS_W2B = RS_C * FF_CH * 2;
+constexpr int RS_IMG = RS_W1B + RS_W2B;
+
+__device__ __forceinline__ constexpr int rs_koff(int s) { return ((s >> 1) % 3) * RS_C + ((s >> 1) / 3) * 64 + (s & 1) * 32; }
+
+}
+
+__global__ __launch_bounds__(256) __attribute__((amdgpu_waves_per_eu(1, 1))) void k_resblock_stream(ResStreamArgs a) {
+    __shared__ __attribute__((aligned(16))) char lds[2 * RS_W1B + 2 * RS_W2B];
+    const int tid = threadIdx.x, lane = tid & 63, wave = __builtin_amdgcn_readfirstlane(tid >> 6);
+    const int r16 = lane & 15, q = lane >> 4;
+    const int nch = a.H / FF_CH;
+    const char* img = reinterpret_cast<const char*>(a.img);
+    auto w1s = [&](int i) { return lds + i * RS_W1B; };
+    auto w2s = [&](int i) { return lds + 2 * RS_W1B + i * RS_W2B; };
+
+    ff_dma<48>(img, w1s(0), wave, lane);
+    ff_dma<16>(img + RS_W1B, w2s(0), wave, lane);
+    ff_dma<48>(img + (size_t)(1 % nch) * RS_IMG, w1s(1), wave, lane);
+    int g = 0;
+
+    const bool has_b1 = a.b1 != nullptr;
+    const float* b1p = (has_b1 ? a.b1 : reinterpret_cast<const float*>(a.img)) + 8 * q;
+    float4 bn[2];
+    bn[0] = *reinterpret_cast<const float4*>(b1p);
+    bn[1] = *reinterpret_cast<const float4*>(b1p + 4);
+
+    const int M = a.B * (a.t1 - a.t0), ntiles = (M + 63) / 64;
+    const unsigned n = (unsigned)(a.t1 - a.t0);
+    const int w2_lane = r16 * 64 + ((q ^ (((r16 >> 3) & 1) * 3)) << 4);
+
+  for (int tile = blockIdx.x; tile < ntiles; tile += gridDim.x) {
+    const int m0 = tile * 64 + wave * 16;
+    const unsigned mu = (unsigned)min(m0 + r16, M - 1);
+    const unsigned bi = mu / n, ri = mu - bi * n;
+    const int64_t row = (int64_t)bi * a.u_bs + (int64_t)(a.pad + a.t0 + (int)ri) * RS_C;
+    Frag xh[RS_KS], xl[RS_KS];
+    float4 res[RS_C / 64][2][2];
+    {
+        const float* win = a.u + row - 2 * RS_C + 8 * q;
+        float4 v[RS_KS][2];
+#pragma unroll
+        for (int s = 0; s < RS_KS; s++) {
+            v[s][0] = *reinterpret_cast<const float4*>(win + rs_koff(s));
+            v[s][1] = *reinterpret_cast<const float4*>(win + rs_koff(s) + 4);
+        }
+#pragma unroll
+        for (int s = 0; s < RS_KS; s++) {
+            if ((s >> 1) % 3 == 2) {
+                res[(s >> 1) / 3][s & 1][0] = v[s][0];
+                res[(s >> 1) / 3][s & 1][1] = v[s][1];
+            }
+            float4 x0 = v[s][0], x1 = v[s][1];
+            x0.x = elu_fast(x0.x); x0.y = elu_fast(x0.y); x0.z = elu_fast(x0.z); x0.w = elu_fast(x0.w);
+            x1.x = elu_fast(x1.x); x1.y = elu_fast(x1.y); x1.z = elu_fast(x1.z); x1.w = elu_fast(x1.w);
+            split8(x0, x1, xh[s], xl[s]);
+        }
+    }
+
+    f32x4 acc2[RS_OT];
+#pragma unroll
+    for (int t = 0; t < RS_OT; t++) acc2[t] = f32x4{0.f, 0.f, 0.f, 0.f};
+
+    asm volatile("s_waitcnt vmcnt(0)" ::: "memory");
+    __syncthreads();
+    f32x4 acc1[2], acc1n[2];
+    ff_gemm1(w1s(g & 1), r16, q, xh, xl, acc1, [](int) {});
+
+    for (int c = 0; c < nch; c++, g++) {
+        asm volatile("s_waitcnt vmcnt(0)" ::: "memory");
+        __syncthreads();
+        asm volatile("" : "+a"(acc1[0]), "+a"(acc1[1]));
+        asm volatile("" : "+v"(bn[0].x), "+v"(bn[0].y), "+v"(bn[0].z), "+v"(bn[0].w), "+v"(bn[1].x), "+v"(bn[1].y), "+v"(bn[1].z), "+v"(bn[1].w));
+        const float bc[8] = {has_b1 ? bn[0].x : 0.f, has_b1 ? bn[0].y : 0.f, has_b1 ? bn[0].z : 0.f, has_b1 ? bn[0].w : 0.f,
+                             has_b1 ? bn[1].x : 0.f, has_b1 ? bn[1].y : 0.f, has_b1 ? bn[1].z : 0.f, has_b1 ? bn[1].w : 0.f};
+        int c1 = c + 1, c2 = c + 2;
+        c1 -= c1 >= nch ? nch : 0;
+        c2 -= c2 >= nch ? nch : 0;
+        c2 -= c2 >= nch ? nch : 0;
+        {
+            const float* nb = b1p + (has_b1 ? c1 * FF_CH : 0);
+            bn[0] = *reinterpret_cast<const float4*>(nb);
+            bn[1] = *reinterpret_cast<const float4*>(nb + 4);
+        }
+        const char* const src1 = img + (size_t)c2 * RS_IMG + wave * 1024 + lane * 16;
+        const char* const src2 = img + (size_t)c1 * RS_IMG + RS_W1B + wave * 1024 + lane * 16;
+        char* const dst1 = w1s(g & 1) + wave * 1024;
+        char* const dst2 = w2s((g + 1) & 1) + wave * 1024;
+        Frag hh, hl;
+        float g8[8];
+        auto piece = [&](int s) {
+#pragma clang fp contract(off)
+            const int i = s >> 1;
+            if (s < 16) {
+                if ((s & 1) == 0) g8[i] = elu_fast(acc1[i >> 2][i & 3] + bc[i]);
+                else if (i & 1) split2(g8[i - 1], g8[i], hh.u[i >> 1], hl.u[i >> 1]);
+            }
+            if (s < 12) lds_dma1k(src1 + s * 4096, dst1 + s * 4096);
+            else if (s < 16) lds_dma1k(src2 + (s - 12) * 4096, dst2 + (s - 12) * 4096);
+        };
+        if (c + 1 < nch) {
+            ff_gemm1(w1s((g + 1) & 1), r16, q, xh, xl, acc1n, piece);
+        } else {
+            acc1n[0] = acc1n[1] = f32x4{0.f, 0.f, 0.f, 0.f};
+#pragma unroll
+            for (int s = 0; s < RS_KS; s++) piece(s);
+        }
+        ff_gemm2(w2s(g & 1) + w2_lane, hh, hl, acc2);
+        acc1[0] = acc1n[0];
+        acc1[1] = acc1n[1];
+    }
+
+    if (m0 + r16 < M) {
+        float* orow = a.uo + row + 8 * q;
+        const bool has_b2 = a.b2 != nullptr;
+        const float* b2p = (has_b2 ? a.b2 : reinterpret_cast<const float*>(a.img)) + 8 * q;
+        float4 bb[RS_OT];
+#pragma unroll
+        for (int t = 0; t < RS_OT; t++) {
+            bb[t] = *reinterpret_cast<const float4*>(b2p + 64 * (t >> 2) + 32 * ((t >> 1) & 1) + 4 * (t & 1));
+            if (!has_b2) bb[t] = make_float4(0.f, 0.f, 0.f, 0.f);
+        }
+#pragma unroll
+        for (int t = 0; t < RS_OT; t++) {
+#pragma clang fp contract(off)
+            const f32x4 y = acc2[t];
+            const float4 r = res[t >> 2][(t >> 1) & 1][t & 1];
+            float4 o;
+            o.x = elu_fast(r.x + (y[0] + bb[t].x));
+            o.y = elu_fast(r.y + (y[1] + bb[t].y));
+            o.z = elu_fast(r.z + (y[2] + bb[t].z));
+            o.w = elu_fast(r.w + (y[3] + bb[t].w));
+            *reinterpret_cast<float4*>(orow + 64 * (t >> 2) + 32 * ((t >> 1) & 1) + 4 * (t & 1)) = o;
+        }
+    }
+  }
+}
+
+bool resblock_stream_supported(const ResStreamArgs& a) {
+    return a.img && a.C == RS_C && a.H >= FF_CH && a.H % FF_CH == 0 && a.k1 == 3 && a.k2 == 1 && a.pad >= 2 && a.B > 0 && a.t0 >= 0 && a.t1 > a.t0 && a.t1 <= a.L &&
+           (int64_t)a.B * (a.t1 - a.t0) <= INT32_MAX - 64 && a.u && a.uo && aligned16(a.u) && aligned16(a.uo) && a.u_bs % 4 == 0 && aligned16(a.img) &&
+           (!a.b1 || aligned16(a.b1)) && (!a.b2 || aligned16(a.b2));
+}
+
+void launch_resblock_stream(const ResStreamArgs& a, hipStream_t stream) {
+    note_launch("k_resblock_stream");
+    const int64_t tiles = ((int64_t)a.B * (a.t1 - a.t0) + 63) / 64;
+    hipLaunchKernelGGL(k_resblock_stream, dim3((unsigned)std::min<int64_t>(tiles, resblock_cus())), dim3(256), 0, stream, a);
+}
+
+}
diff --git a/go-pocket-tts_amd/csrc/runtime.cpp b/go-pocket-tts_amd/csrc/runtime.cpp
--- a/go-pocket-tts_amd/csrc/runtime.cpp
+++ b/go-pocket-tts_amd/csrc/runtime.cpp
@@ -54,6 +54,20 @@
     for (DevBuf& w : ws) w.release();
     if (own_arena && arena) (void)hipFree(arena);
     if (stream) (void)hipStreamDestroy(stream);
+}
+
+const void* Model::rb_image() {
+    if (rb_img_tried) return rb_img_buf.p;
+    rb_img_tried = true;
+    if (!rbs_image_wanted(d)) return nullptr;
+    const size_t n1 = (size_t)d.rb1[0].out * d.rb1[0].in, n2 = (size_t)d.rb2[0].out * d.rb2[0].in, ni = rbs_image_count(d.sea_hidden[0]);
+    std::vector<uint16_t> w1(n1), w2(n2), img(ni);
+    PTTS_HIP(hipMemcpy(w1.data(), arena + d.rb1[0].w, n1 * 2, hipMemcpyDeviceToHost));
+    PTTS_HIP(hipMemcpy(w2.data(), arena + d.rb2[0].w, n2 * 2, hipMemcpyDeviceToHost));
+    rbs_image_from_arena(d, w1.data(), w2.data(), img.data());
+    rb_img_buf.ensure(ni * 2);
+    PTTS_HIP(hipMemcpy(rb_img_buf.p, img.data(), ni * 2, hipMemcpyHostToDevice));
+    return rb_img_buf.p;
 }
 
 static std::unique_ptr<Model> model_on(const Desc& d, const ptts_opts& opts, int device) {
diff --git a/go-pocket-tts_amd/csrc/runtime.h b/go-pocket-tts_amd/csrc/runtime.h
--- a/go-pocket-tts_amd/csrc/runtime.h
+++ b/go-pocket-tts_amd/csrc/runtime.h
@@ -164,6 +164,9 @@
     std::map<int, std::unique_ptr<DevBuf>> tcomb;
     DevBuf ws[kWorkSlots];
     std::unique_ptr<Batch> cached_batch;
+    DevBuf rb_img_buf;
+    bool rb_img_tried = false;
+    const void* rb_image();
     Prof prof;
     std::map<std::pair<int, int>, std::unique_ptr<RateFilter>> rate_filters;
     RowRing<ResampleRow> rs_ring;
diff --git a/go-pocket-tts_amd/runtime.py b/go-pocket-tts_amd/runtime.py
--- a/go-pocket-tts_amd/runtime.py
+++ b/go-pocket-tts_amd/runtime.py
@@ -237,6 +237,7 @@
     "ptts_debug_dsp_opts_error", "ptts_debug_resblock", "ptts_debug_resblock_plan", "ptts_debug_seanet_pack", "ptts_debug_plan_seanet_frags",
     "ptts_debug_gemm_rows", "ptts_debug_attn_step", "ptts_debug_attn_step_rounds", "ptts_debug_attn_window", "ptts_debug_flow_cluster",
     "ptts_debug_mimi_fused", "ptts_debug_mimi_pack", "ptts_debug_dsp_windows", "ptts_debug_step_edge",
+    "ptts_debug_resblock_stream", "ptts_debug_resblock_stream_pack", "ptts_debug_plan_resblock_stream_image",
 ]
 
 
@@ -408,7 +409,8 @@
         H.ptts_debug_dsp_opts_error.restype = C.c_int64
         H.ptts_debug_dsp_opts_error.argtypes = [C.POINTER(DspOpts), C.c_char_p, C.c_int64]
         for name, args in (("flow_cluster", _FlowClusterArgs), ("step_linear", _StepLinearArgs), ("step_edge", _StepEdgeArgs), ("attn_step", _AttnStepArgs), ("attn_window", _AttnWindowArgs),
-                           ("gemm_rows", _GemmRowsArgs), ("mimi_fused", _MimiFusedArgs), ("resblock", _ResblockArgs)):
+                           ("gemm_rows", _GemmRowsArgs), ("mimi_fused", _MimiFusedArgs), ("resblock", _ResblockArgs),
+                           ("resblock_stream", _ResblockStreamArgs)):
             getattr(H, "ptts_debug_" + name).argtypes = [C.POINTER(args)]
         _hooks = H
     return _hooks
@@ -1794,6 +1796,48 @@
     return hi, lo, (int(dims[0]), int(dims[1]))
 
 
+class _ResblockStreamArgs(C.Structure):
+    _fields_ = ([(n, C.c_int32) for n in ("B", "L", "t0", "t1", "C", "H", "pad", "form")] + [(n, C.c_int64) for n in ("u_bs", "launched_cap")] +
+                [(n, _FP) for n in ("u", "w1", "w2", "b1", "b2", "uo", "u_back")] + [("launched", C.c_char_p)])
+
+
+def debug_resblock_stream(u, w1, w2, *, L, pad=2, t0=0, t1=None, b1=None, b2=None, form=0, want_u=False):
+    u, w1, w2 = _f32(u), _f32(w1), _f32(w2)
+    a, keep = _ResblockStreamArgs(), _Keep()
+    ptr = keep.f32
+    a.B, a.L, a.t0, a.t1, a.C, a.H, a.pad, a.form = u.shape[0], int(L), int(t0), int(L if t1 is None else t1), w2.shape[0], w1.shape[0], int(pad), int(form)
+    a.u_bs = u.shape[1] * u.shape[2]
+    uo = np.empty(u.shape, np.float32)
+    back = np.empty(u.shape, np.float32) if want_u else None
+    a.u, a.w1, a.w2, a.b1, a.b2, a.uo, a.u_back = ptr(u), ptr(w1), ptr(w2), ptr(b1), ptr(b2), ptr(uo), ptr(back)
+    name = C.create_string_buffer(512)
+    a.launched, a.launched_cap = C.cast(name, C.c_char_p), 512
+    _check(hooks().ptts_debug_resblock_stream(C.byref(a)))
+    return {"uo": uo, "u": back, "launched": _census_dict(name)}
+
+
+def debug_resblock_stream_pack(w1, w2):
+    w1, w2 = _f32(w1), _f32(w2)
+    h = w1.shape[0]
+    dst = np.empty(max(h, 0) * 1024, np.uint16)
+    H = hooks()
+    H.ptts_debug_resblock_stream_pack.argtypes = [_FP, _FP, C.c_int32, C.c_void_p]
+    _check(H.ptts_debug_resblock_stream_pack(_fp(w1), _fp(w2), h, dst.ctypes.data_as(C.c_void_p)))
+    return dst.reshape(h // 32, 32768)
+
+
+def debug_plan_resblock_stream_image(plan):
+    H = hooks()
+    H.ptts_debug_plan_resblock_stream_image.argtypes = [C.c_void_p, C.c_void_p, C.c_int64, C.POINTER(C.c_int64)]
+    n = C.c_int64(0)
+    _check(H.ptts_debug_plan_resblock_stream_image(plan, None, 0, C.byref(n)))
+    if n.value == 0:
+        return None
+    dst = np.empty(n.value, np.uint16)
+    _check(H.ptts_debug_plan_resblock_stream_image(plan, dst.ctypes.data_as(C.c_void_p), n.value, C.byref(n)))
+    return dst.reshape(-1, 32768)
+
+
 def last_attention_kernel() -> str:
     return hooks().ptts_debug_last_attention_kernel().decode()
 
diff --git a/include/ptts_debug.h b/include/ptts_debug.h
--- a/include/ptts_debug.h
+++ b/include/ptts_debug.h
@@ -153,6 +153,17 @@
 int ptts_debug_mimi_fused(const ptts_mimi_fused_args* a);
 int ptts_debug_mimi_pack(int32_t kind, const float* w1, const float* w2, int32_t n, uint16_t* dst);
 
+typedef struct ptts_resblock_stream_args {
+    int32_t B, L, t0, t1, C, H, pad, form;
+    int64_t u_bs, launched_cap;
+    const float *u, *w1, *w2, *b1, *b2;
+    float *uo, *u_back;
+    char* launched;
+} ptts_resblock_stream_args;
+int ptts_debug_resblock_stream(const ptts_resblock_stream_args* a);
+int ptts_debug_resblock_stream_pack(const float* w1, const float* w2, int32_t H, uint16_t* dst);
+int ptts_debug_plan_resblock_stream_image(ptts_plan* p, uint16_t* dst, int64_t cap, int64_t* count);
+
 int64_t ptts_debug_dsp_opts_error(const ptts_dsp_opts* opts, char* out, int64_t cap);
 int ptts_debug_true_peak_taps(float* out , int32_t* L, int32_t* K, int32_t* dlo);
 int ptts_debug_true_peak_oversample(const float* samples, int64_t n, float* y );
```

Result: no change. 12880 x real-time (median of 6 runs) (+0.4%).
